# althonos/pyskani

Hardware: AMD Instinct MI355X
Metric: genome-pairs/sec (sketch+ANI) (higher is better)
Workload: dtype u64; 1 GPU; all-vs-all 10000 x 10000 synthetic ~5 Mb genomes on one GPU (100 families x 100; single-contig genomes, substitutions only), c=125 marker_c=1000 k=15; device-resident ASCII; hits=999867, genomes=10000, parallelism=references sharded over 1 GPU(s)

## Files before the change

include/pyskani_amd.h:

```cpp
#ifndef PYSKANI_AMD_H
#define PYSKANI_AMD_H
#include <stddef.h>
#include <stdint.h>
#ifdef __cplusplus
extern "C" {
#endif

typedef enum {
    PSK_OK = 0,
    PSK_EINVAL = 1,
    PSK_ENOMEM = 2,
    PSK_EHIP = 3,
    PSK_ENOMODEL = 4,
    PSK_EKEY = 5,
    PSK_ELIMIT = 6,
    PSK_ERCCL = 7
} psk_status;

typedef struct psk_ctx psk_ctx;
typedef struct psk_sketch psk_sketch;
typedef struct psk_db psk_db;
typedef struct psk_model psk_model;

typedef struct {
    int32_t c;
    int32_t marker_c;
    int32_t k;
} psk_params;

typedef struct {
    int32_t learned_ani;
    int32_t median;
    int32_t robust;
    int32_t faster_small;
    double cutoff;
    double min_aligned_frac;
    const psk_model* model;
} psk_query_opts;

typedef struct {
    float ani;
    float af_query;
    float af_ref;
    uint32_t ref_index;
    uint32_t n_chunks, n_intervals;
    uint64_t n_anchors, covered_query, covered_ref, sum_chain_anchors, sum_chunk_seeds;
    float ani_raw;
    float ani_std;
    uint32_t learned;
    uint32_t reserved;
} psk_hit;

typedef struct {
    float ani, af_query, af_ref;
    uint32_t ref_index;
    uint32_t query;
} psk_hit_min;

typedef struct { uint32_t kmer, pos, contig, canon; } psk_seed;

const char* psk_last_error(void);
const char* psk_version(void);
#define PSK_ABI_VERSION 7
int psk_abi_version(void);
void psk_free(void* p);

psk_status psk_ctx_create(int device, psk_ctx** out);
void psk_ctx_destroy(psk_ctx* ctx);
psk_status psk_ctx_synchronize(psk_ctx* ctx);
psk_status psk_ctx_set_timing(psk_ctx* ctx, int on);
psk_status psk_ctx_clock_probe(psk_ctx* ctx, double* mhz, double* ms);
psk_status psk_ctx_timing(psk_ctx* ctx, const char* kernel, double* total_ms, uint64_t* launches);
psk_status psk_ctx_work(psk_ctx* ctx, uint64_t* pairs, uint64_t* items, uint64_t* anchors, int reset);
psk_status psk_ctx_join_work(psk_ctx* ctx, uint64_t* lookups, uint64_t* visited, uint64_t* candidates, uint64_t* rows, int reset);
psk_status psk_ctx_small_query_stats(psk_ctx* ctx, uint64_t* taken, uint64_t* rerun, uint64_t* general);
psk_status psk_ctx_rerun_stats(psk_ctx* ctx, uint64_t* cap, uint64_t* wide, uint64_t* onepass, uint64_t* refit, int reset);
psk_status psk_ctx_tier_stats(psk_ctx* ctx, uint64_t* out, int n, int reset);
void psk_pack2bit_host(const uint8_t* src, uint64_t n, uint32_t* dst, int mode);
psk_status psk_device_alloc(psk_ctx* ctx, size_t bytes, void** dptr);
psk_status psk_device_free(psk_ctx* ctx, void* dptr);
psk_status psk_memcpy_h2d(psk_ctx* ctx, void* dst, const void* src, size_t bytes);

psk_status psk_sketch_host(psk_ctx* ctx, const psk_params* p, const uint8_t* const* contigs,
                           const uint64_t* lens, uint32_t n_contigs, int want_seeds,
                           psk_sketch** out);

psk_status psk_sketch_many_host(psk_ctx* ctx, const psk_params* p, const uint8_t* const* contigs, const uint64_t* lens,
                                const uint32_t* genome_first_contig, uint32_t n_genomes, int want_seeds,
                                psk_sketch** out);

psk_status psk_sketch_batch_device(psk_ctx* ctx, const psk_params* p, const uint8_t* d_bases,
                                   const uint64_t* contig_off, const uint64_t* contig_len,
                                   const uint32_t* genome_first_contig, uint32_t n_genomes,
                                   int want_seeds, psk_sketch** out);

void psk_sketch_free(psk_sketch* s);
void psk_sketch_free_many(psk_sketch* const* sketches, uint32_t n);
psk_status psk_sketch_info(const psk_sketch* s, psk_params* p, uint64_t* n_seeds,
                           uint64_t* n_markers, uint64_t* total_len, uint32_t* n_contigs);
psk_status psk_sketch_export(const psk_sketch* s, psk_seed* seeds, uint64_t* markers);

psk_status psk_sketch_contig_lens(const psk_sketch* s, uint32_t* lens);
psk_status psk_sketch_import(psk_ctx* ctx, const psk_params* p, const uint32_t* contig_lens, uint32_t n_contigs,
                             const psk_seed* seeds, uint64_t n_seeds, const uint64_t* markers, uint64_t n_markers,
                             int has_seeds, psk_sketch** out);

#define PSK_FEATURE_UNKNOWN (-3.402823466e+38F)
typedef struct {
    int32_t feature;
    float threshold;
    int32_t left, right;
    float value;
    int32_t missing;
    int32_t is_leaf;
    int32_t reserved;
} psk_tree_node;
typedef enum {
    PSK_F_ANI100 = 0,
    PSK_F_STD100 = 1,
    PSK_F_Q90_QUERY = 2, PSK_F_Q50_QUERY = 3, PSK_F_Q10_QUERY = 4,
    PSK_F_Q90_REF = 5, PSK_F_Q50_REF = 6, PSK_F_Q10_REF = 7,
    PSK_F_AVG_CHAIN_LEN = 8,
    PSK_F_AF_QUERY = 9, PSK_F_AF_REF = 10, PSK_F_N_CHUNKS = 11,
    PSK_F_TOTAL_LEN_QUERY = 12, PSK_F_TOTAL_LEN_REF = 13, PSK_F_N_CONTIGS_QUERY = 14, PSK_F_N_CONTIGS_REF = 15,
    PSK_F_COUNT = 16
} psk_feature;
psk_status psk_model_create(psk_ctx* ctx, const psk_tree_node* nodes, uint64_t n_nodes, const uint32_t* tree_first_node,
                            uint32_t n_trees, float bias, float shrinkage, const int32_t* features, uint32_t n_features,
                            psk_model** out);
psk_status psk_model_load_json(psk_ctx* ctx, const char* json, size_t len, psk_model** out);
psk_status psk_model_load_file(psk_ctx* ctx, const char* path, psk_model** out);
void psk_model_free(psk_model* m);
psk_status psk_model_info(const psk_model* m, uint32_t* n_trees, uint64_t* n_nodes, uint32_t* n_features);
psk_status psk_model_predict(const psk_model* m, const float* rows, uint32_t n_rows, float* out);

psk_status psk_sketch_pack_size(const psk_sketch* s, uint64_t* bytes);
psk_status psk_sketch_pack(const psk_sketch* s, void* d_dst, uint64_t capacity);
psk_status psk_sketch_unpack(psk_ctx* ctx, const void* d_src, uint64_t capacity, const uint64_t* offsets, uint32_t n, psk_sketch** out);
psk_status psk_sketch_pack_many(const psk_sketch* const* sketches, uint32_t n, void* d_dst, const uint64_t* offsets, uint64_t capacity);

typedef struct psk_comm psk_comm;
#define PSK_COMM_ID_BYTES 128
psk_status psk_comm_unique_id(void* id);
psk_status psk_comm_create(psk_ctx* ctx, int rank, int world, const void* id, psk_comm** out);
void psk_comm_destroy(psk_comm* comm);
psk_status psk_comm_info(const psk_comm* comm, int* rank, int* world, uint64_t* bytes_sent, uint64_t* collectives);
psk_status psk_gather_hits(psk_comm* comm, const psk_hit* local, uint64_t n_local, psk_hit** all, uint64_t* n_all, uint64_t* counts);
psk_status psk_gather_hits_min(psk_comm* comm, const psk_hit_min* local, uint64_t n_local, psk_hit_min** all, uint64_t* n_all, uint64_t* counts);
psk_status psk_gather_sketches(psk_comm* comm, const psk_sketch* const* mine, uint32_t n, psk_sketch*** all, uint32_t* counts);

psk_status psk_db_create(psk_ctx* ctx, const psk_params* p, psk_db** out);
void psk_db_destroy(psk_db* db);
psk_status psk_db_add(psk_db* db, const char* name, psk_sketch* s);
psk_status psk_db_add_batch(psk_db* db, const char* const* names, psk_sketch* const* sketches, uint32_t n);
uint32_t psk_db_size(const psk_db* db);
const char* psk_db_name(const psk_db* db, uint32_t index);
const psk_sketch* psk_db_sketch(const psk_db* db, uint32_t index);

psk_status psk_db_locality(psk_db* db, uint32_t* slot_of, uint32_t* n_groups, uint32_t* is_identity);

psk_status psk_screen(psk_db* db, const psk_sketch* query, double screen_val, int rescue_small,
                      uint8_t* pass, uint32_t* shared);

psk_status psk_chain(psk_ctx* ctx, const psk_sketch* const* refs, uint32_t n_refs,
                     const psk_sketch* query, const psk_query_opts* o, psk_hit* out);

psk_status psk_query(psk_db* db, const psk_sketch* query, const psk_query_opts* o,
                     psk_hit** hits, uint64_t* n_hits);

psk_status psk_query_host(psk_db* db, const uint8_t* const* contigs, const uint64_t* lens, uint32_t n_contigs, int seed,
                          const psk_query_opts* o, psk_hit** hits, uint64_t* n_hits);

psk_status psk_query_many(psk_db* db, const psk_sketch* const* queries, uint32_t n_queries,
                          const psk_query_opts* o, psk_hit** hits, uint64_t* offsets);
psk_status psk_query_many_min(psk_db* db, const psk_sketch* const* queries, uint32_t n_queries,
                              const psk_query_opts* opts, psk_hit_min** hits, uint64_t* offsets);

psk_status psk_query_many_tri(psk_db* db, const psk_sketch* const* queries, uint32_t n_queries, const int64_t* query_key, uint64_t ref_base,
                              const psk_query_opts* opts, psk_hit** hits, uint64_t* offsets);
psk_status psk_query_many_tri_min(psk_db* db, const psk_sketch* const* queries, uint32_t n_queries, const int64_t* query_key, uint64_t ref_base,
                                  const psk_query_opts* opts, psk_hit_min** hits, uint64_t* offsets);

typedef struct {
    double  min_ani;
    double  min_af;
    int32_t af_rule;
    int32_t linkage;
} psk_cluster_opts;
psk_status psk_cluster_records(psk_ctx* ctx, const psk_hit_min* recs, uint64_t n_recs, uint32_t n_genomes,
                               const uint64_t* priority , const psk_cluster_opts* opts,
                               uint32_t* rep_of, float* rep_ani , uint32_t* n_reps );
psk_status psk_ctx_cluster_stats(psk_ctx* ctx, uint64_t* edges, uint64_t* rounds, uint64_t* hook_passes);

#ifdef __cplusplus
}
#endif
#endif
```

pyskani_amd/_capi.py:

```python
import ctypes as C
import os

_HERE = os.path.dirname(os.path.abspath(__file__))
LIB_PATH = os.environ.get("PSK_LIB_PATH") or os.path.join(_HERE, "libpyskani_amd.so")

PSK_OK, PSK_EINVAL, PSK_ENOMEM, PSK_EHIP, PSK_ENOMODEL, PSK_EKEY, PSK_ELIMIT, PSK_ERCCL = range(8)
COMM_ID_BYTES = 128
ABI_VERSION = 7


class Params(C.Structure):
    _fields_ = [("c", C.c_int32), ("marker_c", C.c_int32), ("k", C.c_int32)]


class QueryOpts(C.Structure):
    _fields_ = [("learned_ani", C.c_int32), ("median", C.c_int32), ("robust", C.c_int32),
                ("faster_small", C.c_int32), ("cutoff", C.c_double), ("min_aligned_frac", C.c_double),
                ("model", C.c_void_p)]


class Hit(C.Structure):
    _fields_ = [("ani", C.c_float), ("af_query", C.c_float), ("af_ref", C.c_float),
                ("ref_index", C.c_uint32), ("n_chunks", C.c_uint32), ("n_intervals", C.c_uint32),
                ("n_anchors", C.c_uint64), ("covered_query", C.c_uint64), ("covered_ref", C.c_uint64),
                ("sum_chain_anchors", C.c_uint64), ("sum_chunk_seeds", C.c_uint64),
                ("ani_raw", C.c_float), ("ani_std", C.c_float), ("learned", C.c_uint32), ("reserved", C.c_uint32)]


class HitMin(C.Structure):
    _fields_ = [("ani", C.c_float), ("af_query", C.c_float), ("af_ref", C.c_float), ("ref_index", C.c_uint32), ("query", C.c_uint32)]


class ClusterOpts(C.Structure):
    _fields_ = [("min_ani", C.c_double), ("min_af", C.c_double), ("af_rule", C.c_int32), ("linkage", C.c_int32)]


class TreeNode(C.Structure):
    _fields_ = [("feature", C.c_int32), ("threshold", C.c_float), ("left", C.c_int32), ("right", C.c_int32),
                ("value", C.c_float), ("missing", C.c_int32), ("is_leaf", C.c_int32), ("reserved", C.c_int32)]


FEATURE_NAMES = ["ani100", "std100", "q90_query", "q50_query", "q10_query", "q90_ref", "q50_ref", "q10_ref", "avg_chain_len",
                 "af_query", "af_ref", "n_chunks", "total_len_query", "total_len_ref", "n_contigs_query", "n_contigs_ref"]
DEFAULT_FEATURES = FEATURE_NAMES[:9]


class Seed(C.Structure):
    _fields_ = [("kmer", C.c_uint32), ("pos", C.c_uint32), ("contig", C.c_uint32), ("canon", C.c_uint32)]


SYMBOLS = [
    "psk_last_error", "psk_version", "psk_abi_version", "psk_free", "psk_ctx_create", "psk_ctx_destroy",
    "psk_ctx_synchronize", "psk_pack2bit_host", "psk_ctx_small_query_stats", "psk_ctx_rerun_stats", "psk_ctx_tier_stats", "psk_ctx_set_timing", "psk_ctx_timing", "psk_db_add_batch", "psk_device_alloc", "psk_device_free", "psk_memcpy_h2d",
    "psk_sketch_host", "psk_sketch_many_host", "psk_sketch_batch_device", "psk_sketch_free", "psk_sketch_free_many", "psk_sketch_info",
    "psk_sketch_export", "psk_sketch_contig_lens", "psk_sketch_import", "psk_db_create", "psk_db_destroy", "psk_db_add", "psk_db_size",
    "psk_db_name", "psk_db_sketch", "psk_db_locality", "psk_screen", "psk_chain", "psk_query", "psk_query_host", "psk_query_many", "psk_query_many_min", "psk_query_many_tri", "psk_query_many_tri_min", "psk_cluster_records", "psk_ctx_cluster_stats", "psk_gather_hits_min",
    "psk_sketch_pack_size", "psk_sketch_pack", "psk_sketch_unpack", "psk_sketch_pack_many", "psk_ctx_clock_probe", "psk_ctx_work", "psk_ctx_join_work",
    "psk_comm_unique_id", "psk_comm_create", "psk_comm_destroy", "psk_comm_info", "psk_gather_hits", "psk_gather_sketches",
    "psk_model_create", "psk_model_load_json", "psk_model_load_file", "psk_model_free", "psk_model_info", "psk_model_predict",
]

_lib = None


def load():
    global _lib
    if _lib is not None:
        return _lib
    if not os.path.exists(LIB_PATH):
        raise ImportError(
            f"{LIB_PATH} not found: build it with `python -c 'import __graft_entry__ as g; g.build()'` "
            "or `make -C pyskani_amd/csrc`. pyskani_amd has no CPU fallback.")
    lib = C.CDLL(LIB_PATH)
    vp, u32, u64 = C.c_void_p, C.c_uint32, C.c_uint64
    lib.psk_abi_version.restype = C.c_int
    if lib.psk_abi_version() != ABI_VERSION:
        raise ImportError(f"{LIB_PATH} speaks C-ABI revision {lib.psk_abi_version()}, this binding {ABI_VERSION}: rebuild with `make -C pyskani_amd/csrc`")
    lib.psk_last_error.restype = C.c_char_p
    lib.psk_version.restype = C.c_char_p
    lib.psk_free.argtypes = [vp]
    lib.psk_ctx_create.argtypes = [C.c_int, C.POINTER(vp)]
    lib.psk_ctx_destroy.argtypes = [vp]
    lib.psk_ctx_destroy.restype = None
    lib.psk_ctx_synchronize.argtypes = [vp]
    lib.psk_ctx_small_query_stats.argtypes = [vp, C.POINTER(u64), C.POINTER(u64), C.POINTER(u64)]
    lib.psk_ctx_rerun_stats.argtypes = [vp, C.POINTER(u64), C.POINTER(u64), C.POINTER(u64), C.POINTER(u64), C.c_int]
    if hasattr(lib, "psk_ctx_tier_stats"):
        lib.psk_ctx_tier_stats.argtypes = [vp, C.POINTER(u64), C.c_int, C.c_int]
    lib.psk_pack2bit_host.argtypes = [vp, u64, vp, C.c_int]
    lib.psk_pack2bit_host.restype = None
    lib.psk_ctx_set_timing.argtypes = [vp, C.c_int]
    lib.psk_ctx_timing.argtypes = [vp, C.c_char_p, C.POINTER(C.c_double), C.POINTER(u64)]
    lib.psk_db_add_batch.argtypes = [vp, C.POINTER(C.c_char_p), C.POINTER(vp), u32]
    lib.psk_device_alloc.argtypes = [vp, C.c_size_t, C.POINTER(vp)]
    lib.psk_device_free.argtypes = [vp, vp]
    lib.psk_memcpy_h2d.argtypes = [vp, vp, vp, C.c_size_t]
    lib.psk_sketch_host.argtypes = [vp, C.POINTER(Params), C.POINTER(C.c_char_p), C.POINTER(u64), u32, C.c_int, C.POINTER(vp)]
    lib.psk_sketch_many_host.argtypes = [vp, C.POINTER(Params), C.POINTER(C.c_char_p), C.POINTER(u64), C.POINTER(u32), u32, C.c_int, C.POINTER(vp)]
    lib.psk_sketch_batch_device.argtypes = [vp, C.POINTER(Params), vp, C.POINTER(u64), C.POINTER(u64), C.POINTER(u32), u32, C.c_int, C.POINTER(vp)]
    lib.psk_sketch_free.argtypes = [vp]
    lib.psk_sketch_free.restype = None
    lib.psk_sketch_free_many.argtypes = [C.POINTER(vp), u32]
    lib.psk_sketch_free_many.restype = None
    lib.psk_sketch_info.argtypes = [vp, C.POINTER(Params), C.POINTER(u64), C.POINTER(u64), C.POINTER(u64), C.POINTER(u32)]
    lib.psk_sketch_export.argtypes = [vp, vp, vp]
    lib.psk_sketch_contig_lens.argtypes = [vp, vp]
    lib.psk_sketch_import.argtypes = [vp, C.POINTER(Params), vp, u32, vp, u64, vp, u64, C.c_int, C.POINTER(vp)]
    lib.psk_db_create.argtypes = [vp, C.POINTER(Params), C.POINTER(vp)]
    lib.psk_db_destroy.argtypes = [vp]
    lib.psk_db_destroy.restype = None
    lib.psk_db_add.argtypes = [vp, C.c_char_p, vp]
    lib.psk_db_size.argtypes = [vp]
    lib.psk_db_size.restype = u32
    lib.psk_db_name.argtypes = [vp, u32]
    lib.psk_db_name.restype = C.c_char_p
    lib.psk_db_sketch.argtypes = [vp, u32]
    lib.psk_db_sketch.restype = vp
    lib.psk_screen.argtypes = [vp, vp, C.c_double, C.c_int, vp, vp]
    lib.psk_db_locality.argtypes = [vp, C.POINTER(C.c_uint32), C.POINTER(C.c_uint32), C.POINTER(C.c_uint32)]
    lib.psk_chain.argtypes = [vp, C.POINTER(vp), u32, vp, C.POINTER(QueryOpts), C.POINTER(Hit)]
    lib.psk_query.argtypes = [vp, vp, C.POINTER(QueryOpts), C.POINTER(C.POINTER(Hit)), C.POINTER(u64)]
    lib.psk_query_host.argtypes = [vp, C.POINTER(C.c_char_p), C.POINTER(u64), u32, C.c_int, C.POINTER(QueryOpts), C.POINTER(C.POINTER(Hit)), C.POINTER(u64)]
    lib.psk_query_many.argtypes = [vp, C.POINTER(vp), u32, C.POINTER(QueryOpts), C.POINTER(C.POINTER(Hit)), C.POINTER(u64)]
    lib.psk_query_many_min.argtypes = [vp, C.POINTER(vp), u32, C.POINTER(QueryOpts), C.POINTER(C.POINTER(HitMin)), C.POINTER(u64)]
    lib.psk_query_many_tri.argtypes = [vp, C.POINTER(vp), u32, C.POINTER(C.c_int64), u64, C.POINTER(QueryOpts), C.POINTER(C.POINTER(Hit)), C.POINTER(u64)]
    lib.psk_query_many_tri_min.argtypes = [vp, C.POINTER(vp), u32, C.POINTER(C.c_int64), u64, C.POINTER(QueryOpts), C.POINTER(C.POINTER(HitMin)), C.POINTER(u64)]
    lib.psk_cluster_records.argtypes = [vp, vp, u64, u32, vp, C.POINTER(ClusterOpts), vp, vp, C.POINTER(u32)]
    lib.psk_ctx_cluster_stats.argtypes = [vp, C.POINTER(u64), C.POINTER(u64), C.POINTER(u64)]
    lib.psk_gather_hits_min.argtypes = [vp, vp, u64, C.POINTER(C.POINTER(HitMin)), C.POINTER(u64), C.POINTER(u64)]
    lib.psk_sketch_pack_size.argtypes = [vp, C.POINTER(u64)]
    lib.psk_sketch_pack.argtypes = [vp, vp, u64]
    lib.psk_sketch_unpack.argtypes = [vp, vp, u64, C.POINTER(u64), u32, C.POINTER(vp)]
    lib.psk_sketch_pack_many.argtypes = [C.POINTER(vp), u32, vp, C.POINTER(u64), u64]
    lib.psk_ctx_clock_probe.argtypes = [vp, C.POINTER(C.c_double), C.POINTER(C.c_double)]
    lib.psk_ctx_work.argtypes = [vp, C.POINTER(u64), C.POINTER(u64), C.POINTER(u64), C.c_int]
    lib.psk_ctx_join_work.argtypes = [vp, C.POINTER(u64), C.POINTER(u64), C.POINTER(u64), C.POINTER(u64), C.c_int]
    lib.psk_comm_unique_id.argtypes = [vp]
    lib.psk_comm_create.argtypes = [vp, C.c_int, C.c_int, vp, C.POINTER(vp)]
    lib.psk_comm_destroy.argtypes = [vp]
    lib.psk_comm_destroy.restype = None
    lib.psk_comm_info.argtypes = [vp, C.POINTER(C.c_int), C.POINTER(C.c_int), C.POINTER(u64), C.POINTER(u64)]
    lib.psk_gather_hits.argtypes = [vp, vp, u64, C.POINTER(C.POINTER(Hit)), C.POINTER(u64), C.POINTER(u64)]
    lib.psk_gather_sketches.argtypes = [vp, C.POINTER(vp), u32, C.POINTER(C.POINTER(vp)), C.POINTER(u32)]
    lib.psk_model_create.argtypes = [vp, C.POINTER(TreeNode), u64, C.POINTER(u32), u32, C.c_float, C.c_float, C.POINTER(C.c_int32), u32, C.POINTER(vp)]
    lib.psk_model_load_json.argtypes = [vp, C.c_char_p, C.c_size_t, C.POINTER(vp)]
    lib.psk_model_load_file.argtypes = [vp, C.c_char_p, C.POINTER(vp)]
    lib.psk_model_free.argtypes = [vp]
    lib.psk_model_free.restype = None
    lib.psk_model_info.argtypes = [vp, C.POINTER(u32), C.POINTER(u64), C.POINTER(u32)]
    lib.psk_model_predict.argtypes = [vp, vp, u32, vp]
    _lib = lib
    return lib


_EXC = {PSK_EINVAL: ValueError, PSK_ENOMEM: MemoryError, PSK_EHIP: RuntimeError,
        PSK_ENOMODEL: RuntimeError, PSK_EKEY: KeyError, PSK_ELIMIT: OverflowError, PSK_ERCCL: RuntimeError}


def check(status):
    if status != PSK_OK:
        msg = load().psk_last_error().decode("utf-8", "replace")
        raise _EXC.get(status, RuntimeError)(msg)


def hit_records(hits_p, lo, hi, dtype):
    import numpy as np
    n = max(0, hi - lo)
    out = np.empty(n, dtype)
    if n:
        C.memmove(out.ctypes.data, C.cast(hits_p, C.c_void_p).value + lo * dtype.itemsize, n * dtype.itemsize)
    return out
```

pyskani_amd/csrc/capi.hip:

```cpp
#include "common.h"
#include <cstdarg>
#include <algorithm>

static thread_local char g_err[512] = "";

void psk_set_error(const char* fmt, ...) {
    va_list ap;
    va_start(ap, fmt);
    vsnprintf(g_err, sizeof g_err, fmt, ap);
    va_end(ap);
}

#include <sys/mman.h>
#include <unordered_map>
namespace {
struct HitBlocks {
    std::mutex mu;
    std::unordered_map<void*, size_t> live;
    void* kept = nullptr; size_t kept_bytes = 0;
    const bool keep = !env_val("PSK_HIT_CACHE").off();
};
HitBlocks& hit_blocks() { static HitBlocks* hb = new HitBlocks(); return *hb; }
}
void* hit_block_alloc(size_t bytes) {
// ... 296 lines not shown
void psk_sketch_free_many(psk_sketch* const* sketches, uint32_t n) { if (sketches) for (uint32_t i = 0; i < n; i++) delete sketches[i]; }

psk_status psk_sketch_info(const psk_sketch* s, psk_params* p, uint64_t* n_seeds, uint64_t* n_markers, uint64_t* total_len, uint32_t* n_contigs) {
    if (!s) { psk_set_error("NULL sketch"); return PSK_EINVAL; }
    if (p) *p = s->params;
    if (n_seeds) *n_seeds = s->n_seeds;
    if (n_markers) *n_markers = s->n_markers;
    if (total_len) *total_len = s->total_len;
    if (n_contigs) *n_contigs = (uint32_t)s->contig_len.size();
    return PSK_OK;
}

psk_status psk_sketch_export(const psk_sketch* s, psk_seed* seeds, uint64_t* markers) {
    if (!s) { psk_set_error("NULL sketch"); return PSK_EINVAL; }
    PSK_LANE(lg, s->ctx);
    Lane* ctx = lg.lane;
    if (seeds && s->n_seeds) {
        size_t n = s->n_seeds;
        std::vector<uint32_t> kmer(n), pos(n), meta(n);
        PSK_HIP(hipMemcpyAsync(kmer.data(), s->store->seed_kmer + s->seed_off, 4 * n, hipMemcpyDeviceToHost, ctx->stream));
        PSK_HIP(hipMemcpyAsync(pos.data(), s->store->seed_pos + s->seed_off, 4 * n, hipMemcpyDeviceToHost, ctx->stream));
        PSK_HIP(hipMemcpyAsync(meta.data(), s->store->seed_meta + s->seed_off, 4 * n, hipMemcpyDeviceToHost, ctx->stream));
        PSK_HIP(hipStreamSynchronize(ctx->stream));
        for (size_t i = 0; i < n; i++) { seeds[i].kmer = kmer[i]; seeds[i].pos = pos[i]; seeds[i].contig = meta[i] >> 1; seeds[i].canon = meta[i] & 1; }
    }
    if (markers && s->n_markers) {
        PSK_HIP(hipMemcpyAsync(markers, s->store->markers + s->marker_off, 8 * (size_t)s->n_markers, hipMemcpyDeviceToHost, ctx->stream));
        PSK_HIP(hipStreamSynchronize(ctx->stream));
    }
    return PSK_OK;
}

psk_status psk_sketch_contig_lens(const psk_sketch* s, uint32_t* lens) {
    if (!s || (!lens && !s->contig_len.empty())) { psk_set_error("contig_lens: NULL argument"); return PSK_EINVAL; }
    for (size_t i = 0; i < s->contig_len.size(); i++) lens[i] = s->contig_len[i];
    return PSK_OK;
}

psk_status psk_sketch_import(psk_ctx* ctx, const psk_params* p, const uint32_t* contig_lens, uint32_t n_contigs,
                             const psk_seed* seeds, uint64_t n_seeds, const uint64_t* markers, uint64_t n_markers,
                             int has_seeds, psk_sketch** out) {
    if (!ctx || !p || !out || (n_contigs && !contig_lens) || (n_seeds && !seeds) || (n_markers && !markers)) { psk_set_error("sketch_import: NULL argument"); return PSK_EINVAL; }
    if (p->k < 1 || p->k > 16 || p->c < 1 || p->marker_c < 1) { psk_set_error("invalid sketch parameters"); return PSK_EINVAL; }
    if (n_seeds >= 0x7FFFFFF0ull || n_markers >= 0x7FFFFFF0ull) { psk_set_error("sketch too large to import"); return PSK_ELIMIT; }
    *out = nullptr;
    PSK_LANE(lg, ctx);
    Lane* lane = lg.lane;
    std::unique_ptr<psk_sketch> s(new psk_sketch());
    s->ctx = ctx; s->params = *p; s->has_seeds = has_seeds != 0;
    s->contig_len.assign(contig_lens, contig_lens + n_contigs);
    for (uint32_t i = 0; i < n_contigs; i++) s->total_len += contig_lens[i];
    s->contig_seed_start.assign(n_contigs + 1, 0);
    const size_t ns = (size_t)n_seeds;
    std::vector<uint32_t> kmer(ns), pos(ns), meta(ns), cstart(n_contigs + 1, 0);
    std::vector<uint64_t> pm(ns);
    for (size_t i = 0; i < ns; i++) {
        const psk_seed& sd = seeds[i];
        if (sd.contig >= n_contigs || sd.pos >= contig_lens[sd.contig] || sd.canon > 1 ||
            (i && (sd.contig < seeds[i - 1].contig || (sd.contig == seeds[i - 1].contig && sd.pos <= seeds[i - 1].pos)))) {
            psk_set_error("sketch_import: seed %zu is out of range or out of (contig,pos) order", i);
            return PSK_EINVAL;
        }
        kmer[i] = sd.kmer; pos[i] = sd.pos; meta[i] = (sd.contig << 1) | sd.canon; pm[i] = ((uint64_t)sd.pos << 32) | meta[i];
        cstart[sd.contig + 1]++;
    }
    for (uint32_t c = 0; c < n_contigs; c++) cstart[c + 1] += cstart[c];
    s->contig_seed_start = cstart;
    for (uint64_t i = 1; i < n_markers; i++) if (markers[i] <= markers[i - 1]) { psk_set_error("sketch_import: markers must be sorted and distinct"); return PSK_EINVAL; }
    auto store = std::make_shared<SketchStore>();
    store->ctx = ctx;
    auto al = [](size_t x) { return (x + 255) & ~(size_t)255; };
    size_t b_kmer = 0, b_pos = al(b_kmer + 4 * ns), b_meta = al(b_pos + 4 * ns), b_pm = al(b_meta + 4 * ns), b_cs = al(b_pm + 8 * ns), b_end = al(b_cs + 4 * (size_t)(n_contigs + 1));
    PSK_TRY(ctx->pool_alloc(b_end, &store->base, &store->bytes));
    char* sb = (char*)store->base;
    store->seed_kmer = (uint32_t*)(sb + b_kmer); store->seed_pos = (uint32_t*)(sb + b_pos); store->seed_meta = (uint32_t*)(sb + b_meta);
    store->seed_pm = (uint64_t*)(sb + b_pm); store->contig_seed_start = (uint32_t*)(sb + b_cs);
    PSK_TRY(ctx->pool_alloc(8 * ((size_t)n_markers + 1), &store->mbase, &store->mbytes));
    store->markers = (uint64_t*)store->mbase;
    hipStream_t st = lane->stream;
    if (ns) {
        PSK_HIP(hipMemcpyAsync(store->seed_kmer, kmer.data(), 4 * ns, hipMemcpyHostToDevice, st));
        PSK_HIP(hipMemcpyAsync(store->seed_pos, pos.data(), 4 * ns, hipMemcpyHostToDevice, st));
        PSK_HIP(hipMemcpyAsync(store->seed_meta, meta.data(), 4 * ns, hipMemcpyHostToDevice, st));
        PSK_HIP(hipMemcpyAsync(store->seed_pm, pm.data(), 8 * ns, hipMemcpyHostToDevice, st));
    }
    PSK_HIP(hipMemcpyAsync(store->contig_seed_start, cstart.data(), 4 * (size_t)(n_contigs + 1), hipMemcpyHostToDevice, st));
    if (n_markers) PSK_HIP(hipMemcpyAsync(store->markers, markers, 8 * (size_t)n_markers, hipMemcpyHostToDevice, st));
    PSK_HIP(hipStreamSynchronize(st));
    s->store = store;
    s->seed_off = 0; s->n_seeds = n_seeds; s->marker_off = 0; s->n_markers = n_markers; s->contig_off = 0;
    *out = s.release();
    return PSK_OK;
}

psk_status psk_db_create(psk_ctx* ctx, const psk_params* p, psk_db** out) {
    if (!ctx || !p || !out) { psk_set_error("db_create: NULL argument"); return PSK_EINVAL; }
    if (p->k < 1 || p->k > 16 || p->c < 1 || p->marker_c < 1) { psk_set_error("invalid sketch parameters (c=%d marker_c=%d k=%d)", p->c, p->marker_c, p->k); return PSK_EINVAL; }
    psk_db* db = new psk_db();
    db->ctx = ctx; db->params = *p;
    *out = db;
    return PSK_OK;
}

void psk_db_destroy(psk_db* db) {
    if (!db) return;
    (void)hipSetDevice(db->ctx->device);
    for (psk_sketch* s : db->refs) delete s;
    db->d_marker_ptr.release(); db->d_marker_n.release();
    db->inv_key.release(); db->inv_ref.release(); db->inv_tmp.release(); db->inv_bucket.release();
    db->d_refdesc.release(); db->d_canon.release(); db->d_refdesc_slot.release(); db->d_ref_of.release(); db->d_slot_of.release();
    db->gsi_key.release(); db->gsi_val.release(); db->gsi_bucket.release();
    db->bsi_key.release(); db->bsi_val.release(); db->bsi_bucket.release(); db->bsi_base.release();
    delete db;
}

psk_status psk_db_add(psk_db* db, const char* name, psk_sketch* s) {
    if (!db || !name || !s) { delete s; psk_set_error("db_add: NULL argument"); return PSK_EINVAL; }
    if (s->ctx != db->ctx) { delete s; psk_set_error("db_add: sketch belongs to another context"); return PSK_EINVAL; }
    std::unique_lock<std::shared_mutex> lk(db->rw);
    db->refs.push_back(s);
    db->names.emplace_back(name);
    db->note_added((uint32_t)db->refs.size() - 1);
    db->stale();
    return PSK_OK;
}

psk_status psk_db_add_batch(psk_db* db, const char* const* names, psk_sketch* const* sketches, uint32_t n) {
    if (!db || (n && (!names || !sketches))) { psk_set_error("db_add_batch: NULL argument"); return PSK_EINVAL; }
    std::unique_lock<std::shared_mutex> lk(db->rw);
    for (uint32_t i = 0; i < n; i++)
        if (!sketches[i] || !names[i] || sketches[i]->ctx != db->ctx) { psk_set_error("db_add_batch: bad entry %u", i); return PSK_EINVAL; }
    for (uint32_t i = 0; i < n; i++) {
        db->refs.push_back(sketches[i]);
        db->names.emplace_back(names[i]);
        db->note_added((uint32_t)db->refs.size() - 1);
    }
    db->stale();
    return PSK_OK;
}

uint32_t psk_db_size(const psk_db* db) { if (!db) return 0; std::shared_lock<std::shared_mutex> lk(db->rw); return (uint32_t)db->refs.size(); }
const char* psk_db_name(const psk_db* db, uint32_t i) { if (!db) return nullptr; std::shared_lock<std::shared_mutex> lk(db->rw); return i < db->names.size() ? db->names[i].c_str() : nullptr; }
const psk_sketch* psk_db_sketch(const psk_db* db, uint32_t i) { if (!db) return nullptr; std::shared_lock<std::shared_mutex> lk(db->rw); return i < db->refs.size() ? db->refs[i] : nullptr; }

psk_status psk_db_locality(psk_db* db, uint32_t* slot_of, uint32_t* n_groups, uint32_t* is_identity) {
    if (!db) { psk_set_error("db_locality: NULL database"); return PSK_EINVAL; }
    PSK_LANE(lg, db->ctx);
    std::unique_lock<std::shared_mutex> lk(db->rw);
    PSK_TRY(ensure_locality(lg.lane, db, n_groups != nullptr));
    const uint32_t n = (uint32_t)db->refs.size();
    if (slot_of) for (uint32_t r = 0; r < n; r++) slot_of[r] = db->loc_identity ? r : db->slot_of[r];
    if (n_groups) *n_groups = db->loc_groups;
    if (is_identity) *is_identity = db->loc_identity ? 1u : 0u;
    return PSK_OK;
}

psk_status psk_screen(psk_db* db, const psk_sketch* q, double screen_val, int rescue_small, uint8_t* pass, uint32_t* shared) {
    if (!db || !q || !pass) { psk_set_error("screen: NULL argument"); return PSK_EINVAL; }
    PSK_LANE(lg, db->ctx);
    return screen_impl(lg.lane, db, q, screen_val, rescue_small, pass, shared);
}

psk_status psk_chain(psk_ctx* ctx, const psk_sketch* const* refs, uint32_t n_refs, const psk_sketch* q, const psk_query_opts* o, psk_hit* out) {
    if (!ctx) { psk_set_error("NULL ctx"); return PSK_EINVAL; }
    PSK_LANE(lg, ctx);
    return chain_impl(lg.lane, refs, n_refs, q, o, out);
}

static psk_status hits_out(HitList& all, psk_hit** hits) {
    if (!all.p) { all.p = (psk_hit*)malloc(sizeof(psk_hit)); if (!all.p) { psk_set_error("out of host memory"); return PSK_ENOMEM; } }
    *hits = all.release();
    return PSK_OK;
}

psk_status psk_query(psk_db* db, const psk_sketch* q, const psk_query_opts* o, psk_hit** hits, uint64_t* n_hits) {
    if (!db || !q || !o || !hits || !n_hits) { psk_set_error("query: NULL argument"); return PSK_EINVAL; }
    *hits = nullptr; *n_hits = 0;
    PSK_LANE(lg, db->ctx);
    HitList all;
    uint64_t offs[2];
    PSK_TRY(query_many_impl(lg.lane, db, &q, 1, o, all, offs));
    const uint64_t nh = all.n;
    PSK_TRY(hits_out(all, hits));
    *n_hits = nh;
    return PSK_OK;
}

psk_status psk_query_host(psk_db* db, const uint8_t* const* contigs, const uint64_t* lens, uint32_t n_contigs, int want_seeds,
                          const psk_query_opts* o, psk_hit** hits, uint64_t* n_hits) {
    if (!db || !o || !hits || !n_hits || (n_contigs && (!contigs || !lens))) { psk_set_error("query_host: NULL argument"); return PSK_EINVAL; }
    *hits = nullptr; *n_hits = 0;
    HitList all;
    if (want_seeds) {
        PSK_LANE(lg, db->ctx);
        bool done = false;
        PSK_TRY(query_host_small(lg.lane, db, contigs, lens, n_contigs, o, all, &done));
        if (!done) db->ctx->sq_general++;
        if (done) {
            const uint64_t nh = all.n;
            PSK_TRY(hits_out(all, hits));
            *n_hits = nh;
            return PSK_OK;
        }
        all.n = 0;
    }
    psk_sketch* q = nullptr;
    PSK_TRY(psk_sketch_host(db->ctx, &db->params, contigs, lens, n_contigs, want_seeds, &q));
    const psk_status rc = psk_query(db, q, o, hits, n_hits);
    delete q;
    return rc;
}

psk_status psk_query_many(psk_db* db, const psk_sketch* const* queries, uint32_t n_queries, const psk_query_opts* o,
                          psk_hit** hits, uint64_t* offsets) {
    if (!db || (!queries && n_queries) || !o || !hits || !offsets) { psk_set_error("query_many: NULL argument"); return PSK_EINVAL; }
    *hits = nullptr;
    offsets[0] = 0;
    PSK_LANE(lg, db->ctx);
    HitList all;
    PSK_TRY(query_many_impl(lg.lane, db, queries, n_queries, o, all, offsets));
    return hits_out(all, hits);
}

psk_status psk_query_many_min(psk_db* db, const psk_sketch* const* queries, uint32_t n_queries, const psk_query_opts* o,
                              psk_hit_min** hits, uint64_t* offsets) {
    if (!db || (!queries && n_queries) || !o || !hits || !offsets) { psk_set_error("query_many_min: NULL argument"); return PSK_EINVAL; }
    *hits = nullptr;
    offsets[0] = 0;
    PSK_LANE(lg, db->ctx);
    HitListMin all;
    PSK_TRY(query_many_min_impl(lg.lane, db, queries, n_queries, o, all, offsets));
    if (!all.p) { all.p = (psk_hit_min*)malloc(sizeof(psk_hit_min)); if (!all.p) { psk_set_error("out of host memory"); return PSK_ENOMEM; } }
    *hits = all.release();
    return PSK_OK;
}

static psk_status tri_args(const psk_db* db, const void* queries, uint32_t n_queries, const int64_t* query_key, uint64_t ref_base, const void* o, const void* hits, const void* offsets, const char* who) {
    if (!db || (!queries && n_queries) || !o || !hits || !offsets) { psk_set_error("%s: NULL argument", who); return PSK_EINVAL; }
    if (!query_key && n_queries) { psk_set_error("%s: NULL query_key", who); return PSK_EINVAL; }
    if (ref_base > (1ull << 63) || ref_base + psk_db_size(db) > (1ull << 63)) { psk_set_error("%s: ref_base %llu + the database's size exceeds 2^63 (keys are signed 64-bit)", who, (unsigned long long)ref_base); return PSK_ELIMIT; }
    return PSK_OK;
}

psk_status psk_query_many_tri(psk_db* db, const psk_sketch* const* queries, uint32_t n_queries, const int64_t* query_key, uint64_t ref_base,
                              const psk_query_opts* o, psk_hit** hits, uint64_t* offsets) {
    PSK_TRY(tri_args(db, queries, n_queries, query_key, ref_base, o, hits, offsets, "query_many_tri"));
    *hits = nullptr;
    offsets[0] = 0;
    PSK_LANE(lg, db->ctx);
    HitList all;
    PSK_TRY(query_many_impl(lg.lane, db, queries, n_queries, o, all, offsets, n_queries ? query_key : nullptr, ref_base));
    return hits_out(all, hits);
}

psk_status psk_query_many_tri_min(psk_db* db, const psk_sketch* const* queries, uint32_t n_queries, const int64_t* query_key, uint64_t ref_base,
                                  const psk_query_opts* o, psk_hit_min** hits, uint64_t* offsets) {
    PSK_TRY(tri_args(db, queries, n_queries, query_key, ref_base, o, hits, offsets, "query_many_tri_min"));
    *hits = nullptr;
    offsets[0] = 0;
    PSK_LANE(lg, db->ctx);
    HitListMin all;
    PSK_TRY(query_many_min_impl(lg.lane, db, queries, n_queries, o, all, offsets, n_queries ? query_key : nullptr, ref_base));
    if (!all.p) { all.p = (psk_hit_min*)malloc(sizeof(psk_hit_min)); if (!all.p) { psk_set_error("out of host memory"); return PSK_ENOMEM; } }
    *hits = all.release();
    return PSK_OK;
}

}


#include <condition_variable>
#include <functional>
#include <thread>
#include <atomic>
#include <map>
namespace {
struct ParallelFor {
    std::vector<std::thread> th; std::mutex mu; std::condition_variable cv, cv_done;
    std::function<void(int)> fn; int n = 0, next = 0, active = 0; uint64_t gen = 0; bool stop = false;
    explicit ParallelFor(int workers) {
        for (int i = 0; i < workers; i++) th.emplace_back([this] {
            uint64_t seen = 0;
            for (;;) {
                std::unique_lock<std::mutex> lk(mu);
                cv.wait(lk, [&] { return stop || (gen != seen && next < n); });
                if (stop) return;
                seen = gen;
                while (next < n) { int i = next++; active++; lk.unlock(); fn(i); lk.lock(); active--; }
                if (active == 0) cv_done.notify_all();
            }
        });
    }
    void run(int count, std::function<void(int)> f) {
        std::unique_lock<std::mutex> lk(mu);
        fn = std::move(f); n = count; next = 0; gen++;
        cv.notify_all();
        while (next < n) { int i = next++; active++; lk.unlock(); fn(i); lk.lock(); active--; }
        cv_done.wait(lk, [&] { return active == 0 && next >= n; });
    }
    ~ParallelFor() { { std::lock_guard<std::mutex> lk(mu); stop = true; } cv.notify_all(); for (auto& t : th) t.join(); }
};
constexpr size_t INGEST_SLOT = 32u << 20;
constexpr int INGEST_SLOTS = 4;
struct IngestRes {
    hipStream_t copy = nullptr;
    void* pinned[INGEST_SLOTS] = {nullptr}; hipEvent_t slot_free[INGEST_SLOTS] = {nullptr};
// ... 175 lines not shown
```

pyskani_amd/csrc/chain.hip:

```cpp
#include "chain_stages.h"
#include "query_parts.h"
#include <hipcub/hipcub.hpp>
#include <cmath>
#include <algorithm>
#include <unordered_map>


SketchDesc make_desc(const psk_sketch* s, bool unindexed_ok) {
    SketchDesc d{};
    const bool ix = s->idx != nullptr;
    d.key = ix ? s->idx->km32 + s->idx_off : nullptr; d.pms = ix ? s->idx->pms + s->idx_off : nullptr;
    d.perm = ix ? s->idx->perm + s->idx_off : nullptr; d.bucket = ix ? s->idx->bucket + s->idx_boff : nullptr;
    d.bshift = ix ? s->idx_bshift : 0; d.n = (ix || (unindexed_ok && s->store)) ? (uint32_t)s->n_seeds : 0;
    d.pos = s->store ? s->store->seed_pos + s->seed_off : nullptr; d.meta = s->store ? s->store->seed_meta + s->seed_off : nullptr;
    d.kmer = s->store ? s->store->seed_kmer + s->seed_off : nullptr;
    d.seed_pos_base = s->store ? s->store->seed_pos : nullptr;
    d.contig_start = s->store ? s->store->contig_seed_start + s->contig_off : nullptr;
    d.total_len = s->total_len; d.n_contigs = (uint32_t)s->contig_len.size();
    uint64_t rows = 0;
    if (d.n) for (uint32_t len : s->contig_len) rows += (uint64_t)len / (FRAGMENT_LENGTH + 1) + 1;
    d.rows = (uint32_t)std::min<uint64_t>(rows, 0xFFFFFFFFu);
    s->len_quantiles(d.lenq);
    d.tab = (ix && s->ptab) ? (const ProbeLine*)s->ptab->base + s->ptab_off : nullptr; d.tab_lines = (ix && s->ptab) ? s->ptab_lines : 0;
    return d;
// ... 24 lines not shown
    const uint8_t* __restrict__ row = pass + (size_t)B.q * n_refs;
    const int lane = threadIdx.x & 63, wave = threadIdx.x >> 6;
    uint32_t running = 0;
    for (uint32_t base = 0; base < n_refs && running < B.rank_hi; base += 256) {
        const uint32_t r = base + threadIdx.x;
        const bool f = r < n_refs && row[r];
        const unsigned long long bal = __ballot(f);
        if (lane == 0) s_w[wave] = (uint32_t)__popcll(bal);
        __syncthreads();
        uint32_t before = 0;
        for (int w = 0; w < wave; w++) before += s_w[w];
        const uint32_t tot = s_w[0] + s_w[1] + s_w[2] + s_w[3];
        const uint32_t rank = running + before + (uint32_t)__popcll(bal & ((1ull << lane) - 1));
        if (f && rank >= B.rank_lo && rank < B.rank_hi) {
            const uint32_t j = rank - B.rank_lo, slot = B.pair_off + j;
            pairs[slot] = combine_desc(Q, rd[r]);
            sbase[slot] = B.item_off + j * Q.n; cbase[slot] = B.row_off + j * Q.rows;
            pair_qr[slot] = make_uint2(B.q, r);
        }
        running += tot;
        __syncthreads();
    }
    if (blockIdx.x == gridDim.x - 1 && threadIdx.x == 0) { sbase[n_pairs] = n_items; cbase[n_pairs] = n_rows; }
}

__global__ __launch_bounds__(256) void pass_canon_kernel(uint8_t* __restrict__ pass, uint32_t n_refs, const uint32_t* __restrict__ canon) {
    uint8_t* row = pass + (size_t)blockIdx.x * n_refs;
    for (uint32_t r = threadIdx.x; r < n_refs; r += blockDim.x) if (row[r] && canon[r] != r) { row[canon[r]] = 1; row[r] = 0; }
}
__global__ __launch_bounds__(256) void pass_triangle_kernel(uint8_t* __restrict__ pass, uint32_t n_refs, const long long* __restrict__ key, unsigned long long ref_base) {
    const long long k = key[blockIdx.x];
    if (k < 0 || (unsigned long long)k < ref_base) return;
    const unsigned long long d = (unsigned long long)k - ref_base;
    const uint32_t len = d >= n_refs ? n_refs : (uint32_t)d + 1u;
    uint8_t* row = pass + (size_t)blockIdx.x * n_refs;
    const uint32_t to16 = (16u - (uint32_t)((uintptr_t)row & 15u)) & 15u, head = to16 < len ? to16 : len;
    const uint32_t n16 = (len - head) >> 4, tail = head + (n16 << 4);
    if (threadIdx.x < head) row[threadIdx.x] = 0;
    uint4* mid = (uint4*)(row + head);
    for (uint32_t i = threadIdx.x; i < n16; i += blockDim.x) mid[i] = make_uint4(0, 0, 0, 0);
    if (threadIdx.x < len - tail) row[tail + threadIdx.x] = 0;
}
static_assert((1 << BSI_BLOG) == 256, "pass_count_kernel: one sweep of its 256 threads = one block of references");
__global__ __launch_bounds__(256) void pass_count_kernel(const uint8_t* __restrict__ pass, uint32_t n_refs, uint32_t* __restrict__ row_count, uint8_t* __restrict__ col_flag, uint32_t* __restrict__ row_blocks) {
    __shared__ uint32_t s_c[4], s_any;
    const uint8_t* row = pass + (size_t)blockIdx.x * n_refs;
    uint32_t c = 0, blocks = 0;
    if (threadIdx.x == 0) s_any = 0;
    __syncthreads();
    for (uint32_t r0 = 0; r0 < n_refs; r0 += 256) {
        const uint32_t r = r0 + threadIdx.x;
        const bool f = r < n_refs && row[r];
        if (f) { c++; col_flag[r] = 1; s_any = 1; }
        __syncthreads();
        blocks += s_any;
        __syncthreads();
        if (threadIdx.x == 0) s_any = 0;
        __syncthreads();
    }
#pragma unroll
    for (int o = 32; o > 0; o >>= 1) c += __shfl_xor(c, o);
    if ((threadIdx.x & 63) == 0) s_c[threadIdx.x >> 6] = c;
    __syncthreads();
    if (threadIdx.x == 0) { row_count[blockIdx.x] = s_c[0] + s_c[1] + s_c[2] + s_c[3]; row_blocks[blockIdx.x] = blocks; }
}

__global__ __launch_bounds__(256) void gsi_room_kernel(const uint32_t* __restrict__ sbase, uint32_t n_pairs, uint32_t* __restrict__ pstart) {
    const uint32_t p = blockIdx.x * blockDim.x + threadIdx.x;
    if (p <= n_pairs) { const uint32_t a = sbase[p]; pstart[p] = a + (a >> 3) + 8u * p; }
}
__global__ void gsi_total_kernel(const unsigned long long* __restrict__ poff, uint32_t n_pairs, unsigned long long* __restrict__ total64) { *total64 = poff[n_pairs]; }

struct HitPasses { __host__ __device__ bool operator()(const psk_hit& h) const { return h.ani > 0.1f; } };

__global__ __launch_bounds__(256) void work_rows_kernel(const ChunkOut* __restrict__ cout, const uint32_t* __restrict__ n_chunks, const uint32_t* __restrict__ cbase,
                                                        const uint32_t* __restrict__ row_pair, uint32_t n_rows, unsigned long long* __restrict__ out) {
    __shared__ unsigned long long s_c[4], s_l[4];
    unsigned long long c = 0, live = 0;
    for (uint32_t r = blockIdx.x * blockDim.x + threadIdx.x; r < n_rows; r += gridDim.x * blockDim.x) {
        const uint32_t p = row_pair[r];
        if (r - cbase[p] < n_chunks[p]) { c += cout[r].n_cand; live++; }
    }
#pragma unroll
    for (int o = 32; o > 0; o >>= 1) { c += __shfl_xor(c, o); live += __shfl_xor(live, o); }
    if ((threadIdx.x & 63) == 0) { s_c[threadIdx.x >> 6] = c; s_l[threadIdx.x >> 6] = live; }
    __syncthreads();
    if (threadIdx.x == 0) {
        c = s_c[0] + s_c[1] + s_c[2] + s_c[3]; live = s_l[0] + s_l[1] + s_l[2] + s_l[3];
        if (live) { atomicAdd(&out[0], c); atomicAdd(&out[1], live); }
    }
}

psk_status chain_layout(Lane* ctx, size_t n_pairs, size_t n_items, size_t n_rows, size_t n_bq, ChainBufs* L) {
    const size_t gi = (n_items + 255) / 256, gi_sum = std::max(gi, (n_pairs + 3) / 4);
    size_t o_pairs = 0, o_sbase = al256(o_pairs + sizeof(PairDesc) * n_pairs), o_cbase = al256(o_sbase + 4 * (n_pairs + 1)),
           o_pstart = al256(o_cbase + 4 * (n_pairs + 1)), o_lb = al256(o_pstart + 4 * (n_pairs + 1)),
           o_aoff = al256(o_lb + 8 * (n_items + 1)), o_nch = al256(o_aoff + 4 * (n_items + 1)),
           o_chunks = al256(o_nch + 4 * n_pairs), o_rq0 = al256(o_chunks + sizeof(uint2) * n_rows), o_cout = al256(o_rq0 + sizeof(uint2) * n_rows),
           o_misc = al256(o_cout + sizeof(ChunkOut) * n_rows), o_hits = o_misc + 256, o_sel = al256(o_hits + sizeof(psk_hit) * n_pairs),
           o_ovf = al256(o_sel + sizeof(psk_hit) * n_pairs), o_bsum = al256(o_ovf + 4 * n_rows),
           o_qr = al256(o_bsum + 8 * (gi_sum + 1)), o_bq = al256(o_qr + 8 * n_pairs), o_bp = al256(o_bq + sizeof(BatchQ) * (n_bq + 1)),
           o_rp = al256(o_bp + 4 * (gi + 1)), o_live = al256(o_rp + 4 * (n_rows + 1)), o_big = al256(o_live + 4 * (n_pairs + 1)),
           o_huge = al256(o_big + 4 * (n_pairs + 1)), o_end = o_huge + 4 * (n_pairs + 1);
    PSK_TRY(ctx->q_b.reserve(o_end));
    char* B = (char*)ctx->q_b.p;
    L->pairs = (PairDesc*)(B + o_pairs); L->sbase = (uint32_t*)(B + o_sbase); L->cbase = (uint32_t*)(B + o_cbase); L->pstart = (uint32_t*)(B + o_pstart);
    L->lbcnt = (uint2*)(B + o_lb); L->aoff = (uint32_t*)(B + o_aoff); L->nch = (uint32_t*)(B + o_nch); L->chunks = (uint2*)(B + o_chunks); L->row_q0 = (uint2*)(B + o_rq0);
    L->cout = (ChunkOut*)(B + o_cout); L->hits = (psk_hit*)(B + o_hits); L->hits_sel = (psk_hit*)(B + o_sel); L->misc = (uint32_t*)(B + o_misc);
    L->ovf = (uint32_t*)(B + o_ovf); L->bsum = (unsigned long long*)(B + o_bsum); L->pair_qr = (uint2*)(B + o_qr); L->bq = (BatchQ*)(B + o_bq);
    L->blk_pair = (uint32_t*)(B + o_bp); L->row_pair = (uint32_t*)(B + o_rp); L->live = (uint32_t*)(B + o_live); L->big_list = (uint32_t*)(B + o_big); L->huge_list = (uint32_t*)(B + o_huge);
    L->gi = (uint32_t)gi; L->gi_sum = (uint32_t)gi_sum;
    L->total = (unsigned long long*)(L->misc + 16);
    return PSK_OK;
}

psk_status chain_run(Lane* ctx, const ChainBufs& L, uint32_t n_pairs, size_t n_items, size_t n_rows, const psk_params& prm,
                     const psk_query_opts* o, const SketchDesc* d_qd, const SketchDesc* d_rd, uint64_t cap, bool wide, const Switches& sw, bool probe_ok) {
    hipStream_t st = ctx->stream;
    const int force_serial = sw.chain_serial.get() != nullptr;
    const uint32_t gi = L.gi;
    hipLaunchKernelGGL(pair_table_kernel, dim3((uint32_t)(((size_t)gi + n_rows + 255) / 256)), dim3(256), 0, st, L.sbase, L.cbase, n_pairs, gi, (uint32_t)n_items, (uint32_t)n_rows, L.blk_pair, L.row_pair,
                       L.misc, L.lbcnt + n_items);
    ctx->t_begin(K_ANCHOR);
    if (wide) hipLaunchKernelGGL(anchor_count_kernel, dim3(gi), dim3(256), 0, st, L.pairs, L.sbase, n_pairs, (uint32_t)n_items, L.lbcnt, L.bsum, L.blk_pair);
    const uint32_t gi4 = (gi + JT - 1) / JT;
    uint32_t n_sum = gi;
    const int jp_force = sw.join_pairs.force();
    const bool gsi_join = !wide && (L.g_key || L.b_key) && L.d_pass && L.n_bq;
    const bool join_pairs = !wide && (gsi_join || (jp_force >= 0 ? jp_force == 1 : (n_pairs >= 16384 && n_items / n_pairs < 2048)));
    const bool gsl = gsi_join && L.gsi_slice;
    const bool gsi_one = gsi_join && !gsl && L.gsi_onepass && cap >= n_items + n_items / 8 + 8 * ((size_t)n_pairs + 1);
    bool probe_local = false;
    GsiJoinArgs GA{};
    GslArgs GL{};
    const uint32_t gsi_nw = (L.g_key && !L.gsi_slice) ? std::max(4u, (L.n_refs + 63u) / 64u) : 4u;
    const size_t gsi_lds_row = 8 * (size_t)gsi_nw + 4 * (size_t)((gsi_nw + 1u) & ~1u), gsi_lds_count = gsi_lds_row + 4 * (size_t)L.p_cap, gsi_lds_emit = gsi_lds_row + 4 * (size_t)L.p_cap * 9;
    if (gsi_join) {
        GA.bq = L.bq; GA.pass = L.d_pass; GA.n_refs = L.n_refs; GA.qd = d_qd; GA.g_key = L.g_key; GA.g_val = L.g_val; GA.g_bucket = L.g_bucket; GA.g_shift = L.g_shift;
        GA.b_key = L.b_key; GA.b_val = L.b_val; GA.b_bucket = L.b_bucket; GA.b_shift = L.b_shift; GA.b_nb1 = L.b_nb1; GA.b_blocks = L.b_blocks; GA.b_max = L.b_max;
        GA.pair_cnt = L.big_list; GA.pstart = L.pstart; GA.cap = (uint32_t)cap; GA.err = L.misc; GA.p_cap = L.p_cap; GA.nw_lds = gsi_nw;
        const uint32_t t_blocks = gsl ? L.g_blocks : L.b_blocks;
        const unsigned long long* t_base = gsl ? L.g_base : L.b_base;
        const uint32_t bcap = std::max(1u, std::min<uint32_t>(t_blocks, std::min<uint32_t>(GSI_PMAX, std::max(1u, L.p_cap))));
        uint32_t* d_btab = nullptr; uint32_t* d_bcnt = nullptr;
        if (t_blocks) {
            const size_t o_bc = al256(4 * (size_t)L.n_bq * bcap * GSL_BT_WORDS);
            PSK_TRY(ctx->q_k.reserve(o_bc + 4 * (size_t)L.n_bq + 256));
            d_btab = (uint32_t*)ctx->q_k.p; d_bcnt = (uint32_t*)((char*)ctx->q_k.p + o_bc);
            PSK_TRY(gsl_blocks_launch(L.bq, L.n_bq, L.d_pass, L.n_refs, t_blocks, t_base, d_btab, d_bcnt, bcap, st));
        }
        GA.blk_tab = d_btab; GA.blk_cnt = d_bcnt; GA.blk_cap = bcap;
        if (gsl) {
            GL.bq = L.bq; GL.n_entries = L.n_bq; GL.tab = L.gsl_tab; GL.n_tab = L.gsl_n_tab; GL.ebase = L.gsl_ebase; GL.pass = L.d_pass; GL.n_refs = L.n_refs; GL.qd = d_qd;
            GL.g_key = L.g_key; GL.g_val = L.g_val; GL.g_bucket = L.g_bucket; GL.g_shift = L.g_shift; GL.g_nb1 = L.g_nb1; GL.g_blocks = L.g_blocks; GL.g_base = L.g_base; GL.blk_tab = d_btab; GL.blk_cnt = d_bcnt; GL.blk_cap = bcap; GL.cnt = L.gsl_cnt; GL.rec = L.gsl_rec; GL.bm = L.gsl_bm; GL.un = L.gsl_un; GL.n_slices = L.gsl_n_slices;
            GL.pair_cnt = L.big_list; GL.pstart = L.pstart; GL.cap = (uint32_t)cap; GL.err = L.misc; GL.p_cap = L.p_cap; GL.chunks = L.chunks; GL.n_chunks = L.nch; GL.row_q0 = L.row_q0;
            PSK_HIP(hipMemsetAsync(L.big_list, 0, 4 * ((size_t)n_pairs + 1), st));
            PSK_TRY(gsl_count_launch(GL, st));
        }
        else if (!gsi_one) hipLaunchKernelGGL(gsi_join_kernel<false>, dim3(L.n_bq), dim3(64), gsi_lds_count, st, GA);
        probe_local = true;
    }
    else if (join_pairs) {
        size_t ts = 0;
        uint32_t* keys_in = L.big_list;
        uint32_t* vals_in = L.live;
        uint32_t* keys_out = (uint32_t*)L.hits_sel;
        uint32_t* order = keys_out + n_pairs;
        hipLaunchKernelGGL(pair_ref_keys_kernel, dim3((n_pairs + 255) / 256), dim3(256), 0, st, L.pair_qr, n_pairs, keys_in, vals_in);
        PSK_HIP(hipcub::DeviceRadixSort::SortPairs(nullptr, ts, keys_in, keys_out, vals_in, order, (int)n_pairs, 0, 32, st));
        PSK_TRY(ctx->q_g.reserve(ts + 256));
        PSK_HIP(hipcub::DeviceRadixSort::SortPairs(ctx->q_g.p, ts, keys_in, keys_out, vals_in, order, (int)n_pairs, 0, 32, st));
        const uint32_t nb = (n_pairs + 3) / 4;
        probe_local = probe_ok;
        if (probe_ok) hipLaunchKernelGGL(anchor_join_probe_kernel, dim3(nb), dim3(256), 0, st, L.pairs, L.sbase, order, n_pairs, L.lbcnt, L.bsum, L.misc + 5, L.aoff, L.big_list);
        else hipLaunchKernelGGL(anchor_join_pairs_kernel, dim3(nb), dim3(256), 0, st, L.pairs, L.sbase, order, n_pairs, L.lbcnt, L.bsum, L.misc + 5);
        n_sum = nb;
    }
    const int ep_force = sw.emit_pairs.force();
    const bool emit_pairs = !wide && !join_pairs && n_items >= 2 * ((size_t)n_pairs + 1) &&
                            (ep_force >= 0 ? ep_force == 1 : (n_pairs >= 1024 && n_items / n_pairs >= 1024 && n_items / n_pairs <= (1u << 17)));
    uint32_t* pair_cnt = L.live;
    if (emit_pairs) PSK_HIP(hipMemsetAsync(pair_cnt, 0, 4 * ((size_t)n_pairs + 1), st));
    const int xg_env = (int)sw.xcd_group.num(-1);
    const uint32_t xcd_group = xg_env >= 0 ? (uint32_t)xg_env : (n_pairs >= 64 ? (uint32_t)std::min<size_t>(4096, std::max<size_t>(1, 4 * (n_items / n_pairs) / (JT * 256))) : 0u);
    if (!wide && !join_pairs) { hipLaunchKernelGGL(anchor_join4_kernel, dim3(gi4), dim3(256), 0, st, L.pairs, L.sbase, n_pairs, (uint32_t)n_items, gi, L.lbcnt, L.bsum, L.misc + 5, L.blk_pair, emit_pairs ? pair_cnt : (uint32_t*)nullptr, xcd_group); n_sum = gi4; }
    ctx->t_end();
    size_t tmp = 0, tmp2 = 0;
    hipcub::TransformInputIterator<uint32_t, CountOf, const uint2*> cnt_it(L.lbcnt, CountOf());
    hipcub::TransformInputIterator<uint32_t, PackedCount, const uint2*> pcnt_it(L.lbcnt, PackedCount());
    PSK_HIP(hipcub::DeviceScan::ExclusiveSum(nullptr, tmp, cnt_it, L.aoff, (int)(n_items + 1), st));
    PSK_HIP(hipcub::DeviceReduce::Sum(nullptr, tmp2, L.bsum, L.total, (int)L.gi_sum, st));
    size_t tmp3 = 0;
    PSK_HIP(hipcub::DeviceSelect::If(nullptr, tmp3, L.hits, L.hits_sel, L.misc + 12, (int)n_pairs, HitPasses(), st));
    PSK_TRY(ctx->q_c.reserve(std::max(tmp, std::max(tmp2, tmp3))));
    unsigned long long* poff = (unsigned long long*)L.aoff;
    hipcub::TransformInputIterator<unsigned long long, Widen, const uint32_t*> pc_it(pair_cnt, Widen());
    if (gsi_one) {
        hipLaunchKernelGGL(gsi_room_kernel, dim3((n_pairs + 1 + 255) / 256), dim3(256), 0, st, (const uint32_t*)L.sbase, n_pairs, L.pstart);
        PSK_HIP(hipMemsetAsync(L.total, 0, 8, st));
    }
    else if (emit_pairs) {
        size_t tmp4 = 0;
        PSK_HIP(hipcub::DeviceScan::ExclusiveSum(nullptr, tmp4, pc_it, poff, (int)(n_pairs + 1), st));
        PSK_TRY(ctx->q_c.reserve(std::max(tmp4, std::max(tmp, std::max(tmp2, tmp3)))));
        PSK_HIP(hipcub::DeviceScan::ExclusiveSum(ctx->q_c.p, tmp4, pc_it, poff, (int)(n_pairs + 1), st));
        hipLaunchKernelGGL(pair_start64_kernel, dim3((n_pairs + 1 + 255) / 256), dim3(256), 0, st, poff, n_pairs, L.pstart, (uint32_t)cap, (const uint32_t*)(L.misc + 5));
    }
    else if (probe_local) {
        hipcub::TransformInputIterator<unsigned long long, Widen, const uint32_t*> pl_it(L.big_list, Widen());
        size_t tmp5 = 0;
        PSK_HIP(hipcub::DeviceScan::ExclusiveSum(nullptr, tmp5, pl_it, (unsigned long long*)nullptr, (int)(n_pairs + 1), st));
        const size_t o_poff = al256(tmp5 + 256);
        PSK_TRY(ctx->q_g.reserve(o_poff + 8 * ((size_t)n_pairs + 2) + 256));
        unsigned long long* pl_off64 = (unsigned long long*)((char*)ctx->q_g.p + o_poff);
        PSK_HIP(hipMemsetAsync(L.big_list + n_pairs, 0, 4, st));
        PSK_HIP(hipcub::DeviceScan::ExclusiveSum(ctx->q_g.p, tmp5, pl_it, pl_off64, (int)(n_pairs + 1), st));
        hipLaunchKernelGGL(pair_start64_kernel, dim3((n_pairs + 1 + 255) / 256), dim3(256), 0, st, (const unsigned long long*)pl_off64, n_pairs, L.pstart, (uint32_t)cap, (const uint32_t*)(L.misc + 5));
        if (gsi_join) hipLaunchKernelGGL(gsi_total_kernel, dim3(1), dim3(1), 0, st, (const unsigned long long*)pl_off64, n_pairs, L.total);
    }
    else if (wide) PSK_HIP(hipcub::DeviceScan::ExclusiveSum(ctx->q_c.p, tmp, cnt_it, L.aoff, (int)(n_items + 1), st));
    else PSK_HIP(hipcub::DeviceScan::ExclusiveSum(ctx->q_c.p, tmp, pcnt_it, L.aoff, (int)(n_items + 1), st));
    const bool small_sum = !gsi_join && n_sum <= 16384;
    if (!small_sum && !gsi_join) PSK_HIP(hipcub::DeviceReduce::Sum(ctx->q_c.p, tmp2, L.bsum, L.total, (int)n_sum, st));
    if ((!emit_pairs && !probe_local) || small_sum)
        hipLaunchKernelGGL(pair_start_kernel, dim3((emit_pairs || probe_local) ? 1u : (n_pairs + 1 + 255) / 256), dim3(256), 0, st, (emit_pairs || probe_local) ? (const uint32_t*)nullptr : L.aoff, L.sbase, n_pairs, L.pstart, (uint32_t)cap,
                           L.bsum, small_sum ? n_sum : 0u, L.total, (const uint32_t*)(L.misc + 5));
    hipLaunchKernelGGL(pair_guard_kernel, dim3((n_pairs + 1 + 255) / 256), dim3(256), 0, st, (const uint32_t*)(L.misc + 5), (const unsigned long long*)L.total, (unsigned long long)cap, L.pstart, n_pairs);
    const size_t na = ((size_t)cap + 64 + 63) & ~(size_t)63;
    PSK_TRY(ctx->q_d.reserve(4 * na * CHAIN_ANCHOR_WORDS));
    PSK_TRY(ctx->q_e.reserve(na * (8 + 4 * 7 + 1) + 512 + 4 * 2 * BIG_GMAX * (BIG_GROUPS + 64) + 4 * BIG_GROUPS));
    uint32_t* D = (uint32_t*)ctx->q_d.p;
    uint32_t* E4 = (uint32_t*)ctx->q_e.p;
    uint4* anc = (uint4*)D;
    uint32_t* a_nxt = D + 4 * na;
    ChainArgs A{};
    A.anc = anc;
    A.row_q0 = gsl ? L.row_q0 : nullptr;
    A.sc_ptr = D + 5 * na;
    A.sc_f = (int32_t*)E4; A.sc_root = E4 + na; A.sc_depth = E4 + 2 * na; A.sc_best = E4 + 3 * na;
    uint32_t* CAND = D + 6 * na;
    A.c_score.p = (int32_t*)CAND; A.c_q0.p = CAND + 1; A.c_q1.p = CAND + 2; A.c_r0.p = CAND + 3; A.c_r1.p = CAND + 4; A.c_n.p = CAND + 5; A.c_rc.p = CAND + 6; A.c_state.p = CAND + 7;
    A.chunks = L.chunks; A.n_chunks = L.nch; A.cbase = L.cbase; A.n_pairs = n_pairs; A.n_rows = (uint32_t)n_rows;
    A.row_pair = L.row_pair;
    A.pairs = L.pairs;
    A.out = L.cout; A.two_c = 2u * (uint32_t)prm.c; A.force_serial = force_serial; A.stats = L.misc + 1;
    A.band = std::max(1, std::min(MAX_CHAIN_BAND, BP_CHAIN_BAND / (int)prm.c));
    A.cap = (uint32_t)cap;
    const bool use_hops = gsi_join ? false : sw.chunk_hops.get() ? !sw.chunk_hops.off() : ((n_pairs < 1024 && n_items / n_pairs > 4096) || n_items / n_pairs > (1u << 20));
    const bool emit_heads = emit_pairs && !use_hops && !sw.emit_heads.off();
    const int hi_force = sw.hops_items.force();
    const bool hops_items = use_hops && !gsl && !emit_pairs && !join_pairs && n_items <= 0x7FFFFFFFull && (hi_force >= 0 ? hi_force == 1 : n_items / n_pairs > (1u << 20));
    ctx->t_begin(K_ANCHOR_EMIT);
    if (hops_items) {
        const size_t o_scr = al256(4 * (size_t)n_pairs * HOP_SLICES + 256);
        PSK_TRY(ctx->q_g.reserve(o_scr + sizeof(uint2) * n_rows + 256));
        uint32_t* slice_cnt = (uint32_t*)ctx->q_g.p;
        uint2* scratch_rows = (uint2*)((char*)ctx->q_g.p + o_scr);
        hipStream_t sd = nullptr;
        PSK_TRY(ctx->side_lane(&sd));
        PSK_HIP(hipEventRecord(ctx->side_fork, st));
        PSK_HIP(hipStreamWaitEvent(sd, ctx->side_fork, 0));
        hipLaunchKernelGGL(chunk_hops_items_kernel, dim3(n_pairs, HOP_SLICES), dim3(64), 0, sd, L.pstart, (const uint32_t*)L.aoff, L.pairs, L.sbase, L.cbase, n_pairs, slice_cnt, scratch_rows, L.misc);
        hipLaunchKernelGGL(chunk_hops_sliced_kernel, dim3(n_pairs, HOP_SLICES), dim3(64), 0, sd, L.pstart, a_nxt, anc, L.pairs, L.cbase, n_pairs, slice_cnt, 1, scratch_rows, L.chunks, L.nch, L.misc);
        PSK_HIP(hipEventRecord(ctx->side_join, sd));
    }
    if (gsl) { GL.anc = (uint2*)anc; PSK_TRY(gsl_heads_launch(GL, st)); PSK_TRY(gsl_emit_launch(GL, st)); }
    else if (gsi_join) { GA.anc = anc; GA.chunks = L.chunks; GA.n_chunks = L.nch; GA.onepass = gsi_one ? 1 : 0; GA.total = L.total; if (gsi_one) GA.pair_cnt = L.aoff;
                    hipLaunchKernelGGL(gsi_join_kernel<true>, dim3(L.n_bq), dim3(64), gsi_lds_emit, st, GA); }
    else if (wide) hipLaunchKernelGGL(anchor_emit_kernel, dim3(gi), dim3(256), 0, st, L.pairs, L.sbase, n_pairs, (uint32_t)n_items, L.lbcnt, L.aoff, anc, (uint32_t)cap, L.misc, L.blk_pair);
    else if (emit_pairs) hipLaunchKernelGGL(anchor_emit_pairs_kernel, dim3(n_pairs), dim3(EP_T), 0, st, L.pairs, L.sbase, n_pairs, L.lbcnt, poff, anc, (uint32_t)cap, L.misc,
                                            L.cbase, emit_heads ? L.chunks : (uint2*)nullptr, L.nch);
    else {
        const int ex_force = sw.emit_expand.force();
        const bool expand = ex_force >= 0 ? ex_force == 1 : n_items / n_pairs > (1u << 20);
        if (expand) hipLaunchKernelGGL(anchor_emit_expand_kernel, dim3(gi), dim3(256), 0, st, L.pairs, L.sbase, n_pairs, (uint32_t)n_items, L.lbcnt, L.aoff, anc, (uint32_t)cap, L.misc, L.blk_pair);
        else hipLaunchKernelGGL(anchor_emit_packed4_kernel, dim3(gi4), dim3(256), 0, st, L.pairs, L.sbase, n_pairs, (uint32_t)n_items, gi, L.lbcnt, L.aoff, anc, (uint32_t)cap, L.misc, L.blk_pair,
                                probe_local ? (const uint32_t*)L.pstart : (const uint32_t*)nullptr);
    }
    if (hops_items) PSK_HIP(hipStreamWaitEvent(st, ctx->side_join, 0));
    else if (use_hops) {
        if (n_items / n_pairs > (1u << 20)) {
            uint32_t* coarse = E4;
            hipLaunchKernelGGL(anchor_next_kernel<1>, dim3((uint32_t)((cap / 64 + 1 + 255) / 256)), dim3(256), 0, st, anc, L.pstart, n_pairs, (const uint32_t*)nullptr, coarse);
            hipLaunchKernelGGL(anchor_next_kernel<2>, dim3((uint32_t)((cap + 255) / 256)), dim3(256), 0, st, anc, L.pstart, n_pairs, (const uint32_t*)coarse, a_nxt);
        } else
        hipLaunchKernelGGL(anchor_next_kernel<0>, dim3((uint32_t)((cap + 255) / 256)), dim3(256), 0, st, anc, L.pstart, n_pairs, (const uint32_t*)nullptr, a_nxt);
        if (n_items / n_pairs > (1u << 20)) {
            const size_t o_scr = al256(4 * (size_t)n_pairs * HOP_SLICES + 256);
            PSK_TRY(ctx->q_g.reserve(o_scr + sizeof(uint2) * n_rows + 256));
            uint32_t* slice_cnt = (uint32_t*)ctx->q_g.p;
            uint2* scratch_rows = (uint2*)((char*)ctx->q_g.p + o_scr);
            for (int pass = 0; pass < 2; pass++)
                hipLaunchKernelGGL(chunk_hops_sliced_kernel, dim3(n_pairs, HOP_SLICES), dim3(64), 0, st, L.pstart, a_nxt, anc, L.pairs, L.cbase, n_pairs, slice_cnt, pass, scratch_rows, L.chunks, L.nch, L.misc);
        } else
        hipLaunchKernelGGL(chunk_hops_kernel, dim3(n_pairs), dim3(64), 0, st, L.pstart, a_nxt, L.cbase, n_pairs, L.chunks, L.nch, L.misc);
    } else if (!emit_heads && !gsi_join)
        hipLaunchKernelGGL(chunk_heads_kernel, dim3(n_pairs), dim3(64), 0, st, L.pstart, anc, L.cbase, n_pairs, L.chunks, L.nch, L.misc);
    ctx->t_end();
    ctx->t_begin(K_CHAIN_CHUNK);
    auto order_rows = [&]() -> psk_status {
        if (n_rows < 4096) return PSK_OK;
        size_t ts = 0;
        PSK_HIP(hipcub::DeviceRadixSort::SortPairsDescending(nullptr, ts, (const uint32_t*)nullptr, (uint32_t*)nullptr, (const uint32_t*)nullptr, (uint32_t*)nullptr, (int)n_rows, 0, 8, st));
        const size_t ob = al256(4 * n_rows);
        PSK_TRY(ctx->q_g.reserve(4 * ob + ts + 256));
        uint32_t* k_in = (uint32_t*)ctx->q_g.p; uint32_t* v_in = (uint32_t*)((char*)ctx->q_g.p + ob); uint32_t* k_out = (uint32_t*)((char*)ctx->q_g.p + 2 * ob); uint32_t* v_out = (uint32_t*)((char*)ctx->q_g.p + 3 * ob);
        hipLaunchKernelGGL(row_len_kernel, dim3((uint32_t)((n_rows + 255) / 256)), dim3(256), 0, st, L.chunks, L.nch, L.cbase, L.row_pair, (uint32_t)n_rows, k_in, v_in);
// ... 278 lines not shown
```

pyskani_amd/csrc/common.h:

```cpp
#pragma once
#include <hip/hip_runtime.h>
#include <cstdint>
#include <cstdio>
#include <cstdlib>
#include <cstring>
#include <ctime>
#include <sys/mman.h>
#include <algorithm>
#include <atomic>
#include <memory>
#include <mutex>
#include <shared_mutex>
#include <condition_variable>
#include <deque>
#include <string>
#include <unordered_map>
#include <vector>
#include "../../include/pyskani_amd.h"

struct EnvVal {
    const char* text;
    bool off() const { return text && text[0] == '0'; }
    int force() const { return text ? text[0] == '1' : -1; }
    double num(double dflt) const { return text ? atof(text) : dflt; }
// ... 272 lines not shown
    void* base = nullptr;
    size_t bytes = 0;
    uint64_t* key = nullptr;
    uint32_t* perm = nullptr;
    uint64_t* pms = nullptr;
    uint32_t* km32 = nullptr;
    uint32_t* bucket = nullptr;
    hipStream_t built_on = nullptr; hipEvent_t ready = nullptr;
    ~IndexStore();
};

inline IndexStore::~IndexStore() {
    if (ready) { (void)hipEventSynchronize(ready); (void)hipEventDestroy(ready); }
    if (ctx) ctx->pool_release(base, bytes); else if (base) (void)hipFree(base);
}

constexpr uint32_t PROBE_SLOTS = 5;
constexpr uint32_t PROBE_EMPTY = 0xFFFFFFFFu;
struct ProbeLine { uint32_t k[PROBE_SLOTS]; uint32_t pad; uint2 v[PROBE_SLOTS]; };
static_assert(sizeof(ProbeLine) == 64, "one probe line = one 64-byte cache line");
struct ProbeStore {
    psk_ctx* ctx = nullptr;
    void* base = nullptr;
    size_t bytes = 0;
    ~ProbeStore() { if (ctx) ctx->pool_release(base, bytes); else if (base) (void)hipFree(base); }
};

struct SketchStore {
    psk_ctx* ctx = nullptr;
    void* base = nullptr;
    size_t bytes = 0, mbytes = 0;
    uint32_t* seed_kmer = nullptr;
    uint32_t* seed_pos = nullptr;
    uint32_t* seed_meta = nullptr;
    uint64_t* seed_pm = nullptr;
    uint64_t* markers = nullptr;
    uint32_t* contig_seed_start = nullptr;
    void* mbase = nullptr;
    ~SketchStore() {
        if (ctx) { ctx->pool_release(base, bytes); ctx->pool_release(mbase, mbytes); }
        else { if (base) (void)hipFree(base); if (mbase) (void)hipFree(mbase); }
    }
};

struct SketchDesc {
    const uint32_t* key; const uint64_t* pms; const uint32_t* perm; const uint32_t* bucket;
    const uint32_t* pos; const uint32_t* meta; const uint32_t* seed_pos_base; const uint32_t* contig_start;
    const uint32_t* kmer;
    uint64_t total_len;
    uint32_t n;
    uint32_t bshift, rows;
    uint32_t n_contigs;
    float lenq[3];
    uint32_t tab_lines;
    const ProbeLine* tab;
};

struct SmallVecU32 {
    uint32_t inl[4]; uint32_t* p = inl; uint32_t n = 0, cap = 4;
    SmallVecU32() = default;
    SmallVecU32(const SmallVecU32&) = delete; SmallVecU32& operator=(const SmallVecU32&) = delete;
    ~SmallVecU32() { if (p != inl) delete[] p; }
    void grow(size_t c) {
        if (c <= cap) return;
        const size_t nc = c > 2 * (size_t)cap ? c : 2 * (size_t)cap;
        uint32_t* q = new uint32_t[nc];
        memcpy(q, p, 4 * (size_t)n);
        if (p != inl) delete[] p;
        p = q; cap = (uint32_t)nc;
    }
    size_t size() const { return n; }
    bool empty() const { return n == 0; }
    uint32_t& operator[](size_t i) { return p[i]; }
    const uint32_t& operator[](size_t i) const { return p[i]; }
    const uint32_t* begin() const { return p; }
    const uint32_t* end() const { return p + n; }
    void push_back(uint32_t v) { grow((size_t)n + 1); p[n++] = v; }
    void resize(size_t c) { grow(c); for (size_t i = n; i < c; i++) p[i] = 0; n = (uint32_t)c; }
    void assign(size_t c, uint32_t v) { grow(c); for (size_t i = 0; i < c; i++) p[i] = v; n = (uint32_t)c; }
    template <class It> void assign(It a, It b) { const size_t c = (size_t)(b - a); grow(c); for (size_t i = 0; i < c; i++) p[i] = (uint32_t)a[i]; n = (uint32_t)c; }
    SmallVecU32& operator=(const std::vector<uint32_t>& v) { assign(v.begin(), v.end()); return *this; }
};

struct psk_sketch {
    psk_ctx* ctx = nullptr;
    psk_params params{};
    std::shared_ptr<SketchStore> store;
    uint64_t seed_off = 0, n_seeds = 0;
    uint64_t marker_off = 0, n_markers = 0;
    uint64_t contig_off = 0;
    SmallVecU32 contig_len;
    SmallVecU32 contig_seed_start;
    uint64_t total_len = 0;
    bool has_seeds = true;
    void len_quantiles(float out[3]) const {
        out[0] = out[1] = out[2] = 0.f;
        if (contig_len.empty()) return;
        if (contig_len.size() == 1) { out[0] = out[1] = out[2] = (float)contig_len[0]; return; }
        std::vector<uint32_t> v(contig_len.begin(), contig_len.end());
        std::sort(v.begin(), v.end());
        const size_t n = v.size();
        out[0] = (float)v[std::min(n - 1, n * 9 / 10)]; out[1] = (float)v[std::min(n - 1, n / 2)]; out[2] = (float)v[std::min(n - 1, n / 10)];
    }
    mutable uint64_t visit = 0;
    mutable std::shared_ptr<IndexStore> idx;
    mutable uint64_t idx_off = 0;
    mutable uint64_t idx_boff = 0;
    mutable uint32_t idx_bshift = 0;
    mutable std::shared_ptr<ProbeStore> ptab;
    mutable uint64_t ptab_off = 0;
    mutable uint32_t ptab_lines = 0;
};

struct psk_db {
    psk_ctx* ctx = nullptr;
    mutable std::shared_mutex rw;
    psk_params params{};
    std::vector<psk_sketch*> refs;
    std::deque<std::string> names;
    std::vector<uint32_t> name_slot;
    std::vector<uint32_t> canon;
    bool has_dups = false, canon_dirty = false;
    static uint32_t name_hash(const std::string& s) { uint32_t h = 2166136261u; for (unsigned char c : s) h = (h ^ c) * 16777619u; return h; }
    void note_added(uint32_t i) {
        canon_dirty = true;
        if (name_slot.size() < 2 * (size_t)(i + 1) + 2) {
            size_t cap = 64; while (cap < 4 * (size_t)(i + 1)) cap <<= 1;
            std::vector<uint32_t> grown(cap, 0);
            for (uint32_t v : name_slot) if (v) { size_t k = name_hash(names[v - 1]) & (cap - 1); while (grown[k]) k = (k + 1) & (cap - 1); grown[k] = v; }
            name_slot.swap(grown);
        }
        const size_t mask = name_slot.size() - 1;
        size_t k = name_hash(names[i]) & mask;
        while (name_slot[k] && names[name_slot[k] - 1] != names[i]) k = (k + 1) & mask;
        if (name_slot[k]) { has_dups = true; const uint32_t prev = name_slot[k] - 1; for (uint32_t j = 0; j < i; j++) if (canon[j] == prev) canon[j] = i; }
        name_slot[k] = i + 1;
        canon.push_back(i);
    }
    bool tables_dirty = true;
    PoolScratch d_marker_ptr, d_marker_n;
    bool inv_dirty = true;
    PoolScratch inv_key, inv_ref, inv_tmp, inv_bucket;
    uint64_t inv_n = 0; int inv_bits = 0;
    bool desc_dirty = true;
    uint64_t desc_indexed = 0; uint32_t desc_n = 0;
    PoolScratch d_refdesc, d_canon;
    std::vector<SketchDesc> h_refdesc, h_refdesc_slot;
    int gsi_state = 0;
    PoolScratch gsi_key, gsi_val, gsi_bucket;
    uint64_t gsi_n = 0; int gsi_shift = 0;
    int bsi_state = 0;
    PoolScratch bsi_key, bsi_val, bsi_bucket, bsi_base;
    uint64_t bsi_n = 0; int bsi_shift = 0; uint32_t bsi_nb1 = 0, bsi_blocks = 0;
    std::atomic<int> small_state{0};
    int loc_state = 0;
    bool loc_identity = true, loc_groups_known = false;
    uint32_t loc_groups = 0;
    std::vector<uint32_t> ref_of, slot_of;
    PoolScratch d_ref_of, d_slot_of, d_refdesc_slot;
    void stale() {
        tables_dirty = true; inv_dirty = true; desc_dirty = true; small_state = 0; gsi_key.release(); gsi_val.release(); gsi_bucket.release(); gsi_state = 0;
        bsi_key.release(); bsi_val.release(); bsi_bucket.release(); bsi_base.release(); bsi_state = 0;
        loc_state = 0;
    }
};

psk_status ensure_locality(Lane* ctx, psk_db* db, bool want_groups = false);

struct ModelNode { int32_t feature; float threshold; int32_t left, right; float value; int32_t missing, is_leaf, menu; };
struct ModelDev { const ModelNode* nodes; const uint32_t* first; uint32_t n_trees; uint32_t n_features; float bias, shrinkage; };
struct psk_model {
    psk_ctx* ctx = nullptr;
    void* base = nullptr;
    ModelDev dev{};
    uint64_t n_nodes = 0;
    std::vector<int32_t> features;
    ~psk_model() { if (base) (void)hipFree(base); }
};
void learned_apply_launch(const psk_model* m, psk_hit* d_hits, const uint2* pair_qr, const SketchDesc* qd, const SketchDesc* rd,
                          uint32_t n_pairs, hipStream_t st);

struct ContigDesc {
    uint64_t byte_off;
    uint32_t len;
    uint32_t first_tile;
    uint32_t genome;
    uint32_t contig_index;
    uint32_t pad0, pad1;
};

struct SketchConsts {
    uint64_t thr, thr_marker;
    uint32_t kmask;
    int k, d, rshift;
    int delta;
};


constexpr int BSI_BLOG = 8;
constexpr uint32_t GSI_CONTIG_BITS = 15;
constexpr uint32_t SQ_MAX_TILES = 64, SQ_MAX_DESC = 64;
constexpr uint32_t SQ_SEEDS = 3072;
constexpr uint32_t SQ_MARKERS = 2048;
constexpr uint32_t SQ_ROWS = 64;
constexpr uint32_t SQ_CANDS = 256;
constexpr uint32_t SQ_HITS_FIRST = 256;
constexpr uint32_t SQ_F_SEEDS = 1u, SQ_F_MARKERS = 2u, SQ_F_PAIR = 4u;
struct SmallQHead {
    uint32_t n_seeds, n_markers_raw, n_markers, n_short;
    uint32_t flags, n_hits;
    unsigned long long n_anchors;
    uint32_t coff[SQ_MAX_DESC + 1];
    uint32_t done;
    uint32_t pad1[128 - 9 - (SQ_MAX_DESC + 1)];
};
static_assert(sizeof(SmallQHead) == 512, "the status block is 512 bytes, the hits follow it");
struct SmallQSketch {
    const uint8_t* d_bases; const ContigDesc* d_desc; const uint32_t* d_tci; const uint4* d_tinfo; const uint32_t* d_cft;
    uint32_t n_desc, n_tiles;
    uint32_t *d_packed; uint64_t* d_mask; uint32_t *d_cnt, *d_toff, *d_tmc;
    uint32_t *seed_kmer, *seed_pos, *seed_meta; uint64_t* seed_pm; uint64_t* mstage;
    SmallQHead* head;
};
psk_status small_query_sketch_enqueue(Lane* ctx, const psk_params* p, const SmallQSketch& A, hipStream_t st);

__device__ __forceinline__ uint64_t mm_hash64(uint64_t key) {
    key = ~(key + (key << 21));
    key = key ^ key >> 24;
    key = (key + (key << 3)) + (key << 8);
    key = key ^ key >> 14;
    key = (key + (key << 2)) + (key << 4);
    key = key ^ key >> 28;
    key = key + (key << 31);
    return key;
}

__device__ __forceinline__ uint64_t mm_hash64_u32(uint32_t key) {
    const uint64_t P = (uint64_t)key * 0x200001u;
    uint32_t lo = (uint32_t)P, hi = (uint32_t)(P >> 32);
    lo ^= __builtin_amdgcn_alignbit(hi, lo, 24);
    hi ^= 0xFFFFFF00u;
    uint64_t r = (uint64_t)lo * 265u;
    hi = hi * 265u + (uint32_t)(r >> 32);
    uint64_t x = ((uint64_t)hi << 32) | (uint32_t)r;
    x ^= x >> 14;
    lo = (uint32_t)x; hi = (uint32_t)(x >> 32);
    r = (uint64_t)lo * 21u;
    hi = hi * 21u + (uint32_t)(r >> 32);
    x = ((uint64_t)hi << 32) | (uint32_t)r;
    x ^= x >> 28;
    lo = (uint32_t)x; hi = (uint32_t)(x >> 32);
    r = (uint64_t)lo * 0x80000001u;
    hi = (hi << 31) + (uint32_t)(r >> 32) + hi;
    return ((uint64_t)hi << 32) | (uint32_t)r;
}

psk_status sketch_batch_impl(Lane* ctx, const psk_params* p, const uint8_t* d_bases,
                             const uint64_t* contig_off, const uint64_t* contig_len,
                             const uint32_t* genome_first_contig, uint32_t n_genomes,
                             int want_seeds, psk_sketch** out, const uint32_t* d_packed_in = nullptr);
extern "C" void psk_pack2bit_host(const uint8_t* src, uint64_t n, uint32_t* dst, int mode);
psk_status ensure_index(Lane* ctx, const psk_sketch* const* refs, uint32_t n, bool lazy = false);
psk_status ensure_probe(Lane* ctx, const psk_sketch* const* refs, uint32_t n);
__device__ __forceinline__ uint32_t probe_line(uint32_t km, uint32_t lines) { return __umulhi(km * 2654435761u, lines); }
psk_status screen_impl(Lane* ctx, psk_db* db, const psk_sketch* query, double screen_val, int rescue_small,
                       uint8_t* pass, uint32_t* shared);
psk_status chain_pairs_impl(Lane* ctx, const psk_sketch* const* refs, const psk_sketch* const* queries, uint32_t n,
                            const psk_query_opts* o, psk_hit* out);
void* hit_block_alloc(size_t bytes);
bool hit_block_free(void* p);
void hit_block_trim();
template <class H>
struct HitListT {
    H* p = nullptr; size_t n = 0, cap = 0;
    HitListT() = default;
    HitListT(const HitListT&) = delete; HitListT& operator=(const HitListT&) = delete;
    ~HitListT() { drop(p); }
    static void drop(void* q) { if (q && !hit_block_free(q)) free(q); }
    bool reserve(size_t want) {
        if (want <= cap) return true;
        if (n && want < 2 * cap) want = 2 * cap;
        const size_t bytes = sizeof(H) * want;
        H* q = (H*)(bytes >= ((size_t)8 << 20) ? hit_block_alloc(bytes) : malloc(bytes));
        if (!q) return false;
        if (n) memcpy(q, p, sizeof(H) * n);
        drop(p);
        p = q; cap = want;
        return true;
    }
    bool reserve_for(size_t k) { return n + k <= cap || reserve(std::max<size_t>(n + k, cap + cap / 2 + 64)); }
    bool append(const H* src, size_t k) {
        if (n + k > cap && !reserve(std::max<size_t>(n + k, cap + cap / 2 + 64))) return false;
        if (k) memcpy(p + n, src, sizeof(H) * k);
        n += k;
        return true;
    }
    H* release() { H* q = p; p = nullptr; n = cap = 0; return q; }
};
using HitList = HitListT<psk_hit>;
using HitListMin = HitListT<psk_hit_min>;
psk_status query_many_impl(Lane* ctx, psk_db* db, const psk_sketch* const* queries, uint32_t n_queries, const psk_query_opts* o,
                           HitList& all, uint64_t* offsets, const int64_t* keys = nullptr, uint64_t ref_base = 0);
psk_status query_many_min_impl(Lane* ctx, psk_db* db, const psk_sketch* const* queries, uint32_t n_queries, const psk_query_opts* o,
                               HitListMin& all, uint64_t* offsets, const int64_t* keys = nullptr, uint64_t ref_base = 0);
psk_status chain_impl(Lane* ctx, const psk_sketch* const* refs, uint32_t n_refs,
                      const psk_sketch* query, const psk_query_opts* o, psk_hit* out);
constexpr uint32_t SQ_MAX_REFS = 24 * 1024;
psk_status query_host_small(Lane* ctx, psk_db* db, const uint8_t* const* contigs, const uint64_t* lens, uint32_t n_contigs, const psk_query_opts* o,
                            HitList& all, bool* done);
psk_status small_query_prepare(Lane* ctx, psk_db* db, std::shared_lock<std::shared_mutex>& sh, bool* ok);
```

pyskani_amd/csrc/query_many.hip:

```cpp
#include "chain_stages.h"
#include "query_parts.h"
#include <hipcub/hipcub.hpp>
#include <algorithm>
#include <deque>
#include <thread>

constexpr uint32_t PF_SLOTS = 8192;
constexpr uint32_t PF_MAX_FILL = 4096;
constexpr int PF_T = 512;
constexpr uint32_t PF_EMPTY = 0xFFFFFFFFu;

__global__ __launch_bounds__(256) void pref_gather_kernel(const SketchDesc* __restrict__ qd, const uint32_t* __restrict__ rq, const uint32_t* __restrict__ eoff,
                                                          const uint32_t* __restrict__ qn, uint32_t n_resc, uint32_t* __restrict__ e_key, uint32_t* __restrict__ e_qid) {
    const uint32_t j = blockIdx.x;
    if (j >= n_resc) return;
    const uint32_t* __restrict__ km = qd[rq[j]].kmer;
    const uint32_t o = eoff[j], nn = qn[j];
    for (uint32_t i = threadIdx.x; i < nn; i += blockDim.x) { e_key[o + i] = km[i]; e_qid[o + i] = j; }
}

__global__ __launch_bounds__(PF_T) void pref_count_kernel(const uint32_t* __restrict__ e_key, const uint32_t* __restrict__ e_qid, uint32_t n_entries,
                                                         uint32_t slice_shift, const SketchDesc* __restrict__ rd, uint32_t n_refs, uint32_t refs_per_chunk,
                                                         uint32_t* __restrict__ cnt, uint32_t* __restrict__ overflow) {
    __shared__ uint32_t t_key[PF_SLOTS];
// ... 375 lines not shown
                if (db->bsi_state == 0) PSK_TRY(exclusive([&]() -> psk_status { return build_bsi(ctx, db); }));
                round_gsi = round_slice = round_bsi = db->bsi_state == 1;
            }
        }
        if (round_gsi) {
            round_probe = !round_slice;
            if (db->desc_dirty || db->desc_n != n) PSK_TRY(exclusive([&]() -> psk_status { return refresh_ref_descs(ctx, db); }));
        } else {
        {
            bool refs_stale = db->desc_dirty || db->desc_n != n;
            refs_stale = refs_stale || index_stamp(db) != db->desc_indexed;
            for (size_t i = 0; i < n_need_refs && !refs_stale; i++) refs_stale = !need[i]->idx && need[i]->n_seeds && need[i]->store;
            if (refs_stale)
                PSK_TRY(exclusive([&]() -> psk_status {
                    PSK_TRY(ensure_index(ctx, need.data(), (uint32_t)need.size()));
                    return refresh_ref_descs(ctx, db);
                }));
            else if (need.size() > n_need_refs) PSK_TRY(ensure_index(ctx, need.data() + n_need_refs, (uint32_t)(need.size() - n_need_refs)));
        }
        if (want_small) {
            round_probe = true;
            bool missing = false;
            for (size_t i = 0; i < n_need_refs; i++) {
                if (need[i]->n_seeds < 64 || need[i]->n_seeds > (1u << 22)) { round_probe = false; break; }
                missing = missing || !need[i]->ptab;
            }
            if (round_probe && missing)
                PSK_TRY(exclusive([&]() -> psk_status {
                    PSK_TRY(ensure_probe(ctx, need.data(), (uint32_t)n_need_refs));
                    return refresh_ref_descs(ctx, db);
                }));
        }
        }
        if (!(round_gsi && h_qd_gsi_round == (int64_t)b && h_qd.size() == m)) {
            h_qd.resize(m);
            for (uint32_t i = 0; i < m; i++) h_qd[i] = make_desc(queries[b + i], round_gsi);
        }
        PSK_TRY(ctx->q_h.reserve(sizeof(SketchDesc) * (size_t)m + 256));
        SketchDesc* d_qd = (SketchDesc*)ctx->q_h.p;
        PSK_HIP(hipMemcpyAsync(d_qd, h_qd.data(), sizeof(SketchDesc) * (size_t)m, hipMemcpyHostToDevice, st));
        const int items_env = sw.batch_items_log2.get() ? std::min(31, std::max(16, (int)sw.batch_items_log2.num(0))) : 0;
        int items_log2 = items_env ? items_env : 29;
        if (!items_env) for (uint32_t i = 0; i < m; i++) if (h_qd[i].n > (1u << 20)) { items_log2 = 27; break; }
        if (!items_env && items_log2 == 27) {
            size_t free_b = 0, total_b = 0;
            const size_t need = (size_t)212 << 30;
            if (hipMemGetInfo(&free_b, &total_b) == hipSuccess && free_b + ctx->q_d.cap + ctx->q_e.cap <= need && total_b > need) {
                psk_trim_idle_lanes(ctx->dev, ctx);
                if (lane2) { Scratch* big[] = {&lane2->lane->q_b, &lane2->lane->q_c, &lane2->lane->q_d, &lane2->lane->q_e, &lane2->lane->q_g, &lane2->lane->q_j, &lane2->lane->q_k, &lane2->lane->q_sel}; (void)hipStreamSynchronize(lane2->lane->stream); for (Scratch* s : big) s->release(); }
                (void)hipMemGetInfo(&free_b, &total_b);
            }
            if (free_b + ctx->q_d.cap + ctx->q_e.cap > need) items_log2 = 28;
        }
        const int pairs_env = sw.batch_pairs_log2.get() ? std::min(24, std::max(10, (int)sw.batch_pairs_log2.num(0))) : 0;
        if (!items_env && items_log2 == 29 && round_probe) items_log2 = 30;
        if (!items_env && items_log2 == 29 && round_slice) items_log2 = 30;
        uint64_t max_items = 1ull << items_log2, max_pairs = 1ull << (pairs_env ? pairs_env : (round_probe ? 22 : 21)), max_rows = 1ull << 26;
        {
            if (round_gsi && !round_slice && !sw.gsi_onepass.off() && !items_env && max_items == (1ull << 30)) max_items = 3ull << 28;
        }
        uint32_t qi = 0, rank = 0;
        std::vector<uint64_t> q_hits(m, 0);
        const size_t half_pairs = (size_t)std::min<uint64_t>(round_pairs, max_pairs);
        const size_t half_bytes = al256(sizeof(psk_hit) * half_pairs + 512);
        void* hpin2 = nullptr;
        PSK_TRY(ctx->pinned(2 * half_bytes, &hpin2));
        {
            size_t want = all.n + (size_t)std::min<uint64_t>(round_pairs, 1ull << 26);
            if (want > all.cap) {
                if (b == 0 && n_queries > m) want = std::max(want, (size_t)std::min<double>((double)round_pairs * ((double)n_queries / (double)m) * 1.05, (double)(1ull << 27)));
                if (b > 0 && all.n) want = std::max(want, (size_t)((double)all.n * ((double)n_queries / (double)b) * 1.1) + 4096);
            }
            if (round_pairs > 4096 && !all.reserve(want)) { psk_set_error("out of host memory"); return PSK_ENOMEM; }
        }
        int parity = 0;
        const H* pend_hits = nullptr; uint32_t pend_n = 0;
        bool pend_copy = false;
        hipStream_t cst = nullptr;
        struct CopyDrain { bool& pend; hipStream_t& s; ~CopyDrain() { if (pend && s) (void)hipStreamSynchronize(s); } } copy_drain{pend_copy, cst};
        const size_t sel_half = al256(sizeof(H) * half_pairs + 256);
        auto consume = [&]() -> psk_status {
            if (!pend_n) return PSK_OK;
            if (pend_copy) { PSK_HIP(hipStreamSynchronize(cst)); pend_copy = false; }
            const size_t old = all.n;
            if (!all.reserve_for(pend_n)) { psk_set_error("out of host memory"); return PSK_ENOMEM; }
            auto move = [&](size_t lo, size_t hi, bool shared) {
                memcpy(all.p + old + lo, pend_hits + lo, sizeof(H) * (hi - lo));
                for (size_t i = lo; i < hi; i++) {
                    H& h = all.p[old + i];
                    if (loc) h.ref_index = db->ref_of[h.ref_index];
                    const uint32_t lq = HitRec<H>::local_query(h);
                    if (shared) __atomic_fetch_add(&q_hits[lq], 1u, __ATOMIC_RELAXED); else q_hits[lq]++;
                    HitRec<H>::finish(h, b + lq);
                }
            };
            static const unsigned move_threads = [] { const EnvVal e = env_val("PSK_HIT_THREADS"); const unsigned hw = std::max(1u, std::thread::hardware_concurrency());
                                                      return e.text ? (unsigned)std::max(1, (int)e.num(0)) : std::min(8u, std::max(1u, hw / 8)); }();
            const unsigned nt = (size_t)pend_n * sizeof(H) >= ((size_t)16 << 20) ? move_threads : 1u;
            if (nt <= 1) move(0, pend_n, false);
            else {
                std::vector<std::thread> th;
                const size_t per = ((size_t)pend_n + nt - 1) / nt;
                size_t started = per;
                try {
                    th.reserve(nt);
                    for (unsigned t = 1; t < nt; t++) {
                        const size_t lo = std::min<size_t>(pend_n, t * per), hi = std::min<size_t>(pend_n, lo + per);
                        if (hi > lo) { th.emplace_back(move, lo, hi, true); started = hi; }
                    }
                } catch (...) {}
                move(0, std::min<size_t>(pend_n, per), true);
                if (started < pend_n) move(std::max(started, std::min<size_t>(pend_n, per)), pend_n, true);
                for (std::thread& t : th) t.join();
            }
            all.n += pend_n;
            pend_n = 0;
            return PSK_OK;
        };
        {
            const int pipe_env = (int)sw.pipeline.num(-1);
            const bool pipe_want = round_slice && pipe_env != 0 && (pipe_env == 1 || round_items >= (4ull << 29));
            if (pipe_want && !lane2) {
                lane2.reset(new (std::nothrow) LaneGuard(ctx->dev, true));
                if (lane2 && !lane2->lane) lane2.reset();
            }
            if (pipe_want && lane2) {
                if (!items_env) max_items = 1ull << 29;
                struct PipeJob {
                    uint32_t q0 = 0, r0 = 0, q1 = 0, r1 = 0;
                    std::vector<BatchQ> bqs; std::vector<uint2> tab, ebase; std::vector<uint32_t> qn;
                    uint64_t pairs = 0, items = 0, rows = 0, rows_pair_max = 0;
                    psk_status rc = PSK_OK; bool refit = false; char err[512] = "";
                    std::vector<H> hits; uint64_t anchors = 0, cands = 0, wrows = 0, visited = 0, lookups = 0; uint32_t misc[16] = {};
                };
                PipeJob job[2];
                std::thread th[2];
                bool live[2] = {false, false};
                Lane* lanes[2] = {ctx, lane2->lane};
                PSK_HIP(hipStreamSynchronize(st));
                const SketchDesc* d_rd = ref_descs();
                auto exec = [&](Lane* ln, PipeJob* Jp) {
                    PipeJob& J = *Jp;
                    (void)hipSetDevice(ln->device);
                    J.refit = false; J.hits.clear();
                    try {
                    J.rc = [&]() -> psk_status {
                        hipStream_t s2 = ln->stream;
                        const uint32_t n_pairs = (uint32_t)J.pairs;
                        ChainBufs L;
                        psk_status lrc = chain_layout(ln, n_pairs, (size_t)J.items, (size_t)J.rows, J.bqs.size(), &L);
                        if (lrc == PSK_ENOMEM) { J.refit = true; ctx->dev->rr_refit++; return PSK_OK; }
                        PSK_TRY(lrc);
                        L.rows_pair_max = (uint32_t)std::min<uint64_t>(J.rows_pair_max, 0xFFFFFFFFu);
                        L.g_key = (const uint32_t*)db->bsi_key.p; L.g_val = (const unsigned long long*)db->bsi_val.p; L.g_bucket = (const uint32_t*)db->bsi_bucket.p; L.g_shift = db->bsi_shift; L.g_nb1 = db->bsi_nb1; L.g_blocks = db->bsi_blocks; L.g_base = (const unsigned long long*)db->bsi_base.p;
                        L.d_pass = d_pass; L.n_refs = n; L.n_bq = (uint32_t)J.bqs.size();
                        uint32_t pm = 1; for (const BatchQ& e : J.bqs) pm = std::max(pm, e.rank_hi - e.rank_lo);
                        L.p_cap = (pm + 15u) & ~15u;
                        L.gsi_onepass = false;
                        J.qn.resize(J.bqs.size());
                        for (size_t e = 0; e < J.bqs.size(); e++) J.qn[e] = h_qd[J.bqs[e].q].n;
                        uint64_t n_rec = 0, n_sl = 0;
                        gsl_make_tab(J.bqs.data(), J.bqs.size(), J.qn.data(), J.tab, J.ebase, &n_rec, &n_sl);
                        if (n_rec >= 0x7FFFFF00ull) { psk_set_error("internal: %llu (pair, slice) records in one batch", (unsigned long long)n_rec); return PSK_ELIMIT; }
                        const size_t o_tab = 0, o_eb = al256(o_tab + 8 * J.tab.size()), o_cnt = al256(o_eb + 8 * J.ebase.size()), o_rec = al256(o_cnt + 4 * (size_t)n_rec),
                                     o_bm = al256(o_rec + 16 * (size_t)n_rec), o_un = al256(o_bm + 4 * (size_t)GSL_WORDS * (size_t)n_rec), o_endj = o_un + 4 * (size_t)GSL_WORDS * (size_t)n_sl;
                        lrc = ln->q_j.reserve(o_endj + 256);
                        if (lrc == PSK_ENOMEM) { J.refit = true; ctx->dev->rr_refit++; return PSK_OK; }
                        PSK_TRY(lrc);
                        char* Jb = (char*)ln->q_j.p;
                        PSK_HIP(hipMemcpyAsync(Jb + o_tab, J.tab.data(), 8 * J.tab.size(), hipMemcpyHostToDevice, s2));
                        PSK_HIP(hipMemcpyAsync(Jb + o_eb, J.ebase.data(), 8 * J.ebase.size(), hipMemcpyHostToDevice, s2));
                        L.gsi_slice = true; L.gsl_tab = (const uint2*)(Jb + o_tab); L.gsl_n_tab = (uint32_t)J.tab.size(); L.gsl_ebase = (const uint2*)(Jb + o_eb); L.gsl_un = (uint32_t*)(Jb + o_un); L.gsl_n_slices = (uint32_t)n_sl;
                        L.gsl_cnt = (uint32_t*)(Jb + o_cnt); L.gsl_rec = (uint4*)(Jb + o_rec); L.gsl_bm = (uint32_t*)(Jb + o_bm);
                        PSK_HIP(hipMemcpyAsync(L.bq, J.bqs.data(), sizeof(BatchQ) * J.bqs.size(), hipMemcpyHostToDevice, s2));
                        hipLaunchKernelGGL(pair_build_rows_kernel, dim3((uint32_t)J.bqs.size()), dim3(256), 0, s2, L.bq, d_pass, n, d_qd, d_rd, L.pairs, L.sbase, L.cbase, L.pair_qr, n_pairs, (uint32_t)J.items, (uint32_t)J.rows);
                        const bool host_filter = n_pairs <= 4096;
                        H* d_sel = nullptr;
                        if (!host_filter) { lrc = ln->q_sel.reserve(al256(sizeof(H) * (size_t)n_pairs + 256)); if (lrc == PSK_ENOMEM) { J.refit = true; ctx->dev->rr_refit++; return PSK_OK; } PSK_TRY(lrc); d_sel = (H*)ln->q_sel.p; }
                        void* hp = nullptr;
                        PSK_TRY(ln->pinned(al256(sizeof(psk_hit) * (size_t)n_pairs + 512), &hp));
                        ChainTail* T = (ChainTail*)hp; H* h_sel = (H*)((char*)hp + 256);
                        uint64_t cap = anchor_cap_for(ln, (size_t)J.items, false, false);
                        cap = std::min<uint64_t>(cap, std::max<uint64_t>(ln->q_d.cap / (4 * CHAIN_ANCHOR_WORDS) > 128 ? ln->q_d.cap / (4 * CHAIN_ANCHOR_WORDS) - 128 : 0, (uint64_t)J.items / 4 * 3 + 65536));
                        bool wide = sw.join_wide();
                        for (int attempt = 0;; attempt++) {
                            psk_status rrc = chain_run(ln, L, n_pairs, (size_t)J.items, (size_t)J.rows, db->params, o, d_qd, d_rd, cap, wide, sw, false);
                            if (rrc == PSK_ENOMEM) { (void)hipStreamSynchronize(s2); J.refit = true; ctx->dev->rr_refit++; return PSK_OK; }
                            PSK_TRY(rrc);
                            if (!host_filter) {
                                size_t tmp3 = 0;
                                hipcub::TransformInputIterator<H, ToRec<H>, const psk_hit*> rec_it(L.hits, ToRec<H>());
                                PSK_HIP(hipcub::DeviceSelect::If(nullptr, tmp3, rec_it, d_sel, L.misc + 12, (int)n_pairs, RecPasses<H>(), s2));
                                PSK_TRY(ln->q_c.reserve(tmp3));
                                PSK_HIP(hipcub::DeviceSelect::If(ln->q_c.p, tmp3, rec_it, d_sel, L.misc + 12, (int)n_pairs, RecPasses<H>(), s2));
                                PSK_HIP(hipMemcpyAsync(T, L.misc, sizeof(ChainTail), hipMemcpyDeviceToHost, s2));
                            } else PSK_HIP(hipMemcpyAsync(T, L.misc, 256 + sizeof(psk_hit) * (size_t)n_pairs, hipMemcpyDeviceToHost, s2));
                            PSK_HIP(hipStreamSynchronize(s2));
                            bool retry, was_wide = wide;
                            psk_status rc = chain_check(*T, n_pairs, &cap, &wide, &retry);
                            count_rerun(ctx->dev, was_wide, wide, retry);
                            if ((rc == PSK_ELIMIT && n_pairs > 1) || wide != was_wide) { J.refit = true; ctx->dev->rr_refit++; return PSK_OK; }
                            PSK_TRY(rc);
                            if (!retry) break;
                            if (attempt >= 3) { psk_set_error("internal: anchor capacity did not converge"); return PSK_EHIP; }
                        }
                        uint32_t n_sel = T->misc[12];
                        if (host_filter) {
                            const psk_hit* raw = (const psk_hit*)((char*)hp + 256);
                            for (uint32_t i = 0; i < n_pairs; i++) { const psk_hit r = raw[i]; if (r.ani > 0.1f) J.hits.push_back(HitRec<H>::from_raw(r)); }
                        } else if (n_sel) {
                            PSK_HIP(hipMemcpyAsync(h_sel, d_sel, sizeof(H) * (size_t)n_sel, hipMemcpyDeviceToHost, s2));
                            PSK_HIP(hipStreamSynchronize(s2));
                            J.hits.assign(h_sel, h_sel + n_sel);
                        }
                        J.anchors = T->total64; J.cands = T->cands; J.wrows = T->rows; J.visited = T->visited; memcpy(J.misc, T->misc, sizeof J.misc);
                        J.lookups = 0; for (const BatchQ& e : J.bqs) J.lookups += h_qd[e.q].n;
                        return PSK_OK;
                    }();
                    } catch (...) { psk_set_error("out of host memory"); J.rc = PSK_ENOMEM; }
                    if (J.rc != PSK_OK) snprintf(J.err, sizeof J.err, "%s", psk_last_error());
                    if (J.rc != PSK_OK || J.refit) (void)hipStreamSynchronize(ln->stream);
                    ln->huge_release();
                };
                bool refit = false;
                struct JoinAll { std::thread* t; ~JoinAll() { for (int i = 0; i < 2; i++) if (t[i].joinable()) t[i].join(); } } join_all{th};
                auto reap = [&](int sl) -> psk_status {
                    if (th[sl].joinable()) th[sl].join();
                    live[sl] = false;
                    PipeJob& J = job[sl];
                    if (J.rc != PSK_OK) { psk_set_error("%s", J.err); return J.rc; }
                    if (J.refit) { if (!refit) { refit = true; qi = J.q0; rank = J.r0; } return PSK_OK; }
                    if (refit) return PSK_OK;
                    const size_t nh = J.hits.size();
                    if (nh) {
                        if (!all.reserve_for(nh)) { psk_set_error("out of host memory"); return PSK_ENOMEM; }
                        memcpy(all.p + all.n, J.hits.data(), sizeof(H) * nh);
                        for (size_t i = 0; i < nh; i++) { H& h = all.p[all.n + i]; if (loc) h.ref_index = db->ref_of[h.ref_index]; const uint32_t lq = HitRec<H>::local_query(h); q_hits[lq]++; HitRec<H>::finish(h, b + lq); }
                        all.n += nh;
                    }
                    ctx->dev->w_pairs += J.pairs; ctx->dev->w_items += J.items; ctx->dev->w_anchors += J.anchors; ctx->dev->w_cands += J.cands; ctx->dev->w_rows += J.wrows; count_tier_pairs(ctx->dev, J.misc);
                    ctx->dev->w_lookups += J.lookups; ctx->dev->w_visited += J.visited;
                    return PSK_OK;
                };
                uint32_t k = 0;
                for (;;) {
                    while (qi < m && rank >= h_cnt[qi]) { qi++; rank = 0; }
                    if (qi >= m || refit) break;
                    const int sl = (int)(k & 1u);
                    if (live[sl]) { PSK_TRY(reap(sl)); if (refit) break; }
                    PipeJob& J = job[sl];
                    J.bqs.clear(); J.pairs = J.items = J.rows = J.rows_pair_max = 0;
                    J.q0 = qi; J.r0 = rank;
                    uint32_t pq = qi, pr = rank;
                    while (pq < m) {
                        const uint32_t left = h_cnt[pq] - pr;
                        if (left == 0) { pq++; pr = 0; continue; }
                        const uint64_t qn = h_qd[pq].n, qrows = h_qd[pq].rows;
                        uint64_t take = std::min<uint64_t>(left, max_pairs - J.pairs);
                        take = std::min<uint64_t>(take, GSI_PMAX);
                        if (qn) take = std::min<uint64_t>(take, (max_items - J.items) / qn);
                        if (qrows) take = std::min<uint64_t>(take, (max_rows - J.rows) / qrows);
                        if (take == 0) { if (J.pairs == 0) take = 1; else break; }
                        J.bqs.push_back(BatchQ{pq, pr, pr + (uint32_t)take, (uint32_t)J.pairs, (uint32_t)J.items, (uint32_t)J.rows});
                        J.rows_pair_max = std::max<uint64_t>(J.rows_pair_max, qrows);
                        J.pairs += take; J.items += take * qn; J.rows += take * qrows;
                        pr += (uint32_t)take;
                        if (J.pairs >= max_pairs || J.items >= max_items || J.rows >= max_rows) break;
                    }
                    J.q1 = pq; J.r1 = pr;
                    if (J.items >= 0xFFFFFF00ull || J.rows >= 0xFFFFFF00ull) { psk_set_error("a single pair exceeds the per-launch limits (%llu query seeds)", (unsigned long long)J.items); return PSK_ELIMIT; }
                    qi = pq; rank = pr;
                    if (J.items == 0 || J.rows == 0) continue;
                    try { th[sl] = std::thread(exec, lanes[sl], &J); }
                    catch (...) { exec(lanes[sl], &J); }
                    live[sl] = true;
                    k++;
                }
                for (int i = 0; i < 2; i++) { const int sl = (int)((k + (uint32_t)i) & 1u); if (live[sl]) PSK_TRY(reap(sl)); }
                if (refit) max_items = std::max<uint64_t>(1, max_items / 4);
            }
        }
        while (qi < m) {
            if (rank >= h_cnt[qi]) { qi++; rank = 0; continue; }
            bqs.clear();
            uint64_t pairs = 0, items = 0, rows = 0, rows_pair_max = 0;
            uint32_t pq = qi, pr = rank;
            while (pq < m) {
                const uint32_t left = h_cnt[pq] - pr;
                if (left == 0) { pq++; pr = 0; continue; }
                const uint64_t qn = h_qd[pq].n, qrows = h_qd[pq].rows;
                uint64_t take = std::min<uint64_t>(left, max_pairs - pairs);
                if (round_gsi) take = std::min<uint64_t>(take, GSI_PMAX);
                if (qn) take = std::min<uint64_t>(take, (max_items - items) / qn);
                if (qrows) take = std::min<uint64_t>(take, (max_rows - rows) / qrows);
                if (take == 0) { if (pairs == 0) take = 1; else break; }
                bqs.push_back(BatchQ{pq, pr, pr + (uint32_t)take, (uint32_t)pairs, (uint32_t)items, (uint32_t)rows});
                rows_pair_max = std::max<uint64_t>(rows_pair_max, qrows);
                pairs += take; items += take * qn; rows += take * qrows;
                pr += (uint32_t)take;
                if (pairs >= max_pairs || items >= max_items || rows >= max_rows) break;
            }
            const uint32_t n_pairs = (uint32_t)pairs;
            if (items >= 0xFFFFFF00ull || rows >= 0xFFFFFF00ull) { psk_set_error("a single pair exceeds the per-launch limits (%llu query seeds)", (unsigned long long)items); return PSK_ELIMIT; }
            uint32_t n_sel = 0;
            H* h_sel = nullptr;
            if (items == 0 || rows == 0) {
            } else {
                ChainBufs L;
                psk_status lrc = chain_layout(ctx, n_pairs, (size_t)items, (size_t)rows, bqs.size(), &L);
                L.rows_pair_max = (uint32_t)std::min<uint64_t>(rows_pair_max, 0xFFFFFFFFu);
                if (round_gsi) {
                    if (round_slice) { L.g_key = (const uint32_t*)db->bsi_key.p; L.g_val = (const unsigned long long*)db->bsi_val.p; L.g_bucket = (const uint32_t*)db->bsi_bucket.p; L.g_shift = db->bsi_shift; L.g_nb1 = db->bsi_nb1; L.g_blocks = db->bsi_blocks; L.g_base = (const unsigned long long*)db->bsi_base.p; }
                    else {
                        if (db->gsi_state == 1) { L.g_key = (const uint32_t*)db->gsi_key.p; L.g_val = (const unsigned long long*)db->gsi_val.p; L.g_bucket = (const uint32_t*)db->gsi_bucket.p; L.g_shift = db->gsi_shift; }
                        if (round_bsi) { L.b_key = (const uint32_t*)db->bsi_key.p; L.b_val = (const unsigned long long*)db->bsi_val.p; L.b_bucket = (const uint32_t*)db->bsi_bucket.p; L.b_shift = db->bsi_shift; L.b_nb1 = db->bsi_nb1; L.b_blocks = db->bsi_blocks; L.b_base = (const unsigned long long*)db->bsi_base.p; L.b_max = (uint32_t)std::max(1.0, max_blocks_join); }
                    }
                    L.d_pass = d_pass; L.n_refs = n; L.n_bq = (uint32_t)bqs.size();
                    uint32_t pm = 1; for (const BatchQ& e : bqs) pm = std::max(pm, e.rank_hi - e.rank_lo);
                    L.p_cap = round_slice ? (pm + 15u) & ~15u : (pm + 63u) & ~63u;
                    L.gsi_onepass = !sw.gsi_onepass.off() && !round_slice;
                    if (round_slice && lrc == PSK_OK) {
                        gsl_qn.resize(bqs.size());
                        for (size_t e = 0; e < bqs.size(); e++) gsl_qn[e] = h_qd[bqs[e].q].n;
                        uint64_t n_rec = 0, n_sl = 0;
                        gsl_make_tab(bqs.data(), bqs.size(), gsl_qn.data(), gsl_tab, gsl_ebase, &n_rec, &n_sl);
                        if (n_rec >= 0x7FFFFF00ull) { psk_set_error("internal: %llu (pair, slice) records in one batch", (unsigned long long)n_rec); return PSK_ELIMIT; }
                        const size_t o_tab = 0, o_eb = al256(o_tab + 8 * gsl_tab.size()), o_cnt = al256(o_eb + 8 * gsl_ebase.size()), o_rec = al256(o_cnt + 4 * (size_t)n_rec),
                                     o_bm = al256(o_rec + 16 * (size_t)n_rec), o_un = al256(o_bm + 4 * (size_t)GSL_WORDS * (size_t)n_rec), o_endj = o_un + 4 * (size_t)GSL_WORDS * (size_t)n_sl;
                        lrc = ctx->q_j.reserve(o_endj + 256);
                        if (lrc == PSK_OK) {
                            char* J = (char*)ctx->q_j.p;
                            PSK_HIP(hipMemcpyAsync(J + o_tab, gsl_tab.data(), 8 * gsl_tab.size(), hipMemcpyHostToDevice, st));
                            PSK_HIP(hipMemcpyAsync(J + o_eb, gsl_ebase.data(), 8 * gsl_ebase.size(), hipMemcpyHostToDevice, st));
                            L.gsi_slice = true; L.gsl_tab = (const uint2*)(J + o_tab); L.gsl_n_tab = (uint32_t)gsl_tab.size(); L.gsl_ebase = (const uint2*)(J + o_eb); L.gsl_un = (uint32_t*)(J + o_un); L.gsl_n_slices = (uint32_t)n_sl;
                            L.gsl_cnt = (uint32_t*)(J + o_cnt); L.gsl_rec = (uint4*)(J + o_rec); L.gsl_bm = (uint32_t*)(J + o_bm);
                        }
                    }
                }
                if (lrc == PSK_ENOMEM && n_pairs > 1 && max_items > (1ull << 22)) { max_items >>= 2; continue; }
                PSK_TRY(lrc);
                PSK_HIP(hipMemcpyAsync(L.bq, bqs.data(), sizeof(BatchQ) * bqs.size(), hipMemcpyHostToDevice, st));
                hipLaunchKernelGGL(pair_build_rows_kernel, dim3((uint32_t)bqs.size()), dim3(256), 0, st, L.bq, d_pass, n, d_qd, ref_descs(),
                                   L.pairs, L.sbase, L.cbase, L.pair_qr, n_pairs, (uint32_t)items, (uint32_t)rows);
                const bool host_filter = n_pairs <= 4096;
                H* d_sel = nullptr;
                if (!host_filter) {
                    PSK_TRY(ctx->copy_lane(&cst));
                    PSK_TRY(ctx->q_sel.reserve(2 * sel_half));
                    d_sel = (H*)((char*)ctx->q_sel.p + (parity ? sel_half : 0));
                }
                if (sizeof(psk_hit) * (size_t)n_pairs + 512 > half_bytes) { psk_set_error("internal: batch larger than its staging half"); return PSK_EHIP; }
                hpin = (char*)hpin2 + (parity ? half_bytes : 0);
                ChainTail* T = (ChainTail*)hpin; h_sel = (H*)((char*)hpin + 256);
                uint64_t cap = anchor_cap_for(ctx, (size_t)items, round_probe, items / n_pairs > (1u << 20));
                if (round_slice) cap = std::min<uint64_t>(cap, std::max<uint64_t>(ctx->q_d.cap / (4 * CHAIN_ANCHOR_WORDS) > 128 ? ctx->q_d.cap / (4 * CHAIN_ANCHOR_WORDS) - 128 : 0, (uint64_t)items / 4 * 3 + 65536));
                if (L.gsi_onepass) cap = std::min<uint64_t>(std::max<uint64_t>(cap, items + items / 8 + 8 * ((uint64_t)n_pairs + 1) + 64), 0x7FFFFF00ull);
                bool too_big = false, wide = sw.join_wide();
                static const bool trace_batch = getenv("PSK_TRACE_BATCH") != nullptr;
                for (int attempt = 0;; attempt++) {
                    struct timespec tb0{}, tb1{}, tb2{};
                    if (trace_batch) clock_gettime(CLOCK_MONOTONIC, &tb0);
                    psk_status rrc = chain_run(ctx, L, n_pairs, (size_t)items, (size_t)rows, db->params, o, d_qd, ref_descs(), cap, wide, sw, round_probe && !round_gsi);
                    if (trace_batch) clock_gettime(CLOCK_MONOTONIC, &tb1);
                    if (rrc == PSK_ENOMEM && n_pairs > 1 && max_items > (1ull << 22)) { (void)hipStreamSynchronize(st); ctx->huge_release(); too_big = true; break; }
                    PSK_TRY(rrc);
                    if (!host_filter) {
                        size_t tmp3 = 0;
                        hipcub::TransformInputIterator<H, ToRec<H>, const psk_hit*> rec_it(L.hits, ToRec<H>());
                        PSK_HIP(hipcub::DeviceSelect::If(nullptr, tmp3, rec_it, d_sel, L.misc + 12, (int)n_pairs, RecPasses<H>(), st));
                        PSK_TRY(ctx->q_c.reserve(tmp3));
                        PSK_HIP(hipcub::DeviceSelect::If(ctx->q_c.p, tmp3, rec_it, d_sel, L.misc + 12, (int)n_pairs, RecPasses<H>(), st));
                    }
                    if (host_filter) PSK_HIP(hipMemcpyAsync(T, L.misc, 256 + sizeof(psk_hit) * (size_t)n_pairs, hipMemcpyDeviceToHost, st));
                    else PSK_HIP(hipMemcpyAsync(T, L.misc, sizeof(ChainTail), hipMemcpyDeviceToHost, st));
                    PSK_TRY(consume());
                    PSK_HIP(hipStreamSynchronize(st));
                    if (trace_batch) {
                        clock_gettime(CLOCK_MONOTONIC, &tb2);
                        static struct timespec last{};
                        const double gap = last.tv_sec ? (tb0.tv_sec - last.tv_sec) * 1e3 + (tb0.tv_nsec - last.tv_nsec) / 1e6 : 0.0;
                        fprintf(stderr, "[psk batch] pairs %u items %llu attempt %d: since last %.1f ms, launch %.1f ms, wait %.1f ms; anchors %llu of %llu, status %x, wide %u -> %u\n", n_pairs, (unsigned long long)items, attempt, gap,
                                (tb1.tv_sec - tb0.tv_sec) * 1e3 + (tb1.tv_nsec - tb0.tv_nsec) / 1e6, (tb2.tv_sec - tb1.tv_sec) * 1e3 + (tb2.tv_nsec - tb1.tv_nsec) / 1e6,
                                (unsigned long long)T->total64, (unsigned long long)cap, T->misc[0], wide ? 1u : 0u, T->misc[5]);
                        last = tb2;
                    }
                    ctx->huge_release();
                    bool retry; const bool was_wide = wide;
                    psk_status rc = chain_check(*T, n_pairs, &cap, &wide, &retry);
                    count_rerun(ctx->dev, was_wide, wide, retry);
                    if (rc == PSK_ELIMIT && n_pairs > 1) { too_big = true; break; }
                    PSK_TRY(rc);
                    if (!retry && L.gsi_onepass && (T->misc[0] & 4u)) { L.gsi_onepass = false; retry = true; ctx->dev->rr_onepass++; }
                    if (!retry) {
                        ctx->dev->w_pairs += n_pairs; ctx->dev->w_items += items; ctx->dev->w_anchors += T->total64; ctx->dev->w_cands += T->cands; ctx->dev->w_rows += T->rows; count_tier_pairs(ctx->dev, T->misc);
                        if (round_gsi) { uint64_t lk = 0; for (const BatchQ& e : bqs) lk += h_qd[e.q].n; ctx->dev->w_lookups += lk; ctx->dev->w_visited += T->visited; }
                        break;
                    }
                    if (attempt >= 3) { psk_set_error("internal: anchor capacity did not converge"); return PSK_EHIP; }
                }
                if (too_big) { max_items = std::max<uint64_t>(1, items / 4); max_pairs = std::max<uint64_t>(1, pairs / 4); continue; }
                n_sel = T->misc[12];
                if (n_pairs <= 4096) {
                    const psk_hit* raw = (const psk_hit*)((char*)hpin + 256);
                    uint32_t w = 0;
                    for (uint32_t i = 0; i < n_pairs; i++) { const psk_hit r = raw[i]; if (r.ani > 0.1f) h_sel[w++] = HitRec<H>::from_raw(r); }
                    n_sel = w;
                }
                else if (n_sel) {
                    PSK_HIP(hipMemcpyAsync(h_sel, d_sel, sizeof(H) * (size_t)n_sel, hipMemcpyDeviceToHost, cst));
                    pend_copy = true;
                }
            }
            if (n_sel) { pend_hits = h_sel; pend_n = n_sel; parity ^= 1; }
            qi = pq; rank = pr;
        }
        PSK_TRY(consume());
        for (uint32_t i = 0; i < m; i++) offsets[b + i + 1] = offsets[b + i] + q_hits[i];
        if (loc)
            for (uint32_t i = 0; i < m; i++) {
                H* h0 = all.p + all0 + offsets[b + i]; H* h1 = all.p + all0 + offsets[b + i + 1];
                auto by_ref = [](const H& x, const H& y) { return x.ref_index < y.ref_index; };
                if (!std::is_sorted(h0, h1, by_ref)) std::sort(h0, h1, by_ref);
            }
    }
    return PSK_OK;
}
psk_status query_many_impl(Lane* ctx, psk_db* db, const psk_sketch* const* queries, uint32_t n_queries, const psk_query_opts* o, HitList& all, uint64_t* offsets, const int64_t* keys, uint64_t ref_base) {
    return query_many_t<psk_hit>(ctx, db, queries, n_queries, o, all, offsets, keys, ref_base);
}
psk_status query_many_min_impl(Lane* ctx, psk_db* db, const psk_sketch* const* queries, uint32_t n_queries, const psk_query_opts* o, HitListMin& all, uint64_t* offsets, const int64_t* keys, uint64_t ref_base) {
    return query_many_t<psk_hit_min>(ctx, db, queries, n_queries, o, all, offsets, keys, ref_base);
}
```

pyskani_amd/csrc/query_parts.h:

```cpp
#pragma once
#include "chain_stages.h"
#include <deque>
#include <vector>
#include <cstring>

static inline size_t al256(size_t x) { return (x + 255) & ~(size_t)255; }

struct SwitchVal {
    char text[24]; bool set;
    const char* get() const { return set ? text : nullptr; }
    bool off() const { return EnvVal{get()}.off(); }
    int force() const { return EnvVal{get()}.force(); }
    double num(double dflt) const { return EnvVal{get()}.num(dflt); }
};
#define PSK_SWITCHES(X) \
    X(chain_serial, "PSK_CHAIN_SERIAL") \
    X(join_pairs, "PSK_JOIN_PAIRS") \
    X(emit_pairs, "PSK_EMIT_PAIRS") \
    X(xcd_group, "PSK_XCD_GROUP") \
    X(chunk_hops, "PSK_CHUNK_HOPS") \
    X(emit_heads, "PSK_EMIT_HEADS") \
    X(hops_items, "PSK_HOPS_ITEMS") \
    X(emit_expand, "PSK_EMIT_EXPAND") \
    X(chain_lane, "PSK_CHAIN_LANE") \
    X(lane_xtrees, "PSK_LANE_XTREES") \
    X(chain_quad_deep, "PSK_CHAIN_QUAD_DEEP") \
    X(chain_wave_reg, "PSK_CHAIN_WAVE_REG") \
    X(select_tiny, "PSK_SELECT_TINY") \
    X(big_solo, "PSK_BIG_SOLO") \
    X(huge_slots, "PSK_HUGE_SLOTS") \
    X(huge_min_seeds, "PSK_HUGE_MIN_SEEDS") \
    X(reduce_small, "PSK_REDUCE_SMALL") \
    X(reduce_wave, "PSK_REDUCE_WAVE") \
    X(reduce_tiny, "PSK_REDUCE_TINY") \
    X(join, "PSK_JOIN") \
    X(round_queries, "PSK_ROUND_QUERIES") \
    X(screen, "PSK_SCREEN") \
    X(prefilter, "PSK_PREFILTER") \
    X(gsi_join, "PSK_GSI_JOIN") \
    X(gsl_max_blocks, "PSK_GSL_MAX_BLOCKS") \
    X(probe, "PSK_PROBE") \
    X(gsi_slice, "PSK_GSI_SLICE") \
    X(bsi_small, "PSK_BSI_SMALL") \
    X(batch_items_log2, "PSK_BATCH_ITEMS_LOG2") \
    X(batch_pairs_log2, "PSK_BATCH_PAIRS_LOG2") \
    X(gsi_onepass, "PSK_GSI_ONEPASS") \
    X(pipeline, "PSK_PIPELINE") \
    X(screen_global, "PSK_SCREEN_GLOBAL") \
    X(screen_wave, "PSK_SCREEN_WAVE") \
    X(locality, "PSK_LOCALITY")
struct Switches {
#define X(field, name) SwitchVal field;
    PSK_SWITCHES(X)
#undef X
    static Switches read();
    bool join_wide() const { const char* e = join.get(); return e && !strcmp(e, "wide"); }
};

struct ScreenStaging { std::deque<std::vector<MarkerSet>> hq; std::deque<std::vector<uint32_t>> qoff; };
psk_status upload_marker_table(Lane* ctx, psk_db* db);
psk_status build_inverted(Lane* ctx, psk_db* db);
psk_status screen_many_device(Lane* ctx, psk_db* db, const psk_sketch* const* queries, uint32_t nq, double screen_val, int rescue_small, uint8_t* d_pass, ScreenStaging& keep, const Switches& sw);

SketchDesc make_desc(const psk_sketch* s, bool unindexed_ok = false);
__global__ __launch_bounds__(256) void pair_build_rows_kernel(const BatchQ* __restrict__ bq, const uint8_t* __restrict__ pass, uint32_t n_refs,
                                                              const SketchDesc* __restrict__ qd, const SketchDesc* __restrict__ rd,
                                                              PairDesc* __restrict__ pairs, uint32_t* __restrict__ sbase, uint32_t* __restrict__ cbase,
                                                              uint2* __restrict__ pair_qr, uint32_t n_pairs, uint32_t n_items, uint32_t n_rows);
__global__ __launch_bounds__(256) void pass_canon_kernel(uint8_t* __restrict__ pass, uint32_t n_refs, const uint32_t* __restrict__ canon);
__global__ __launch_bounds__(256) void pass_triangle_kernel(uint8_t* __restrict__ pass, uint32_t n_refs, const long long* __restrict__ key, unsigned long long ref_base);
__global__ __launch_bounds__(256) void pass_count_kernel(const uint8_t* __restrict__ pass, uint32_t n_refs, uint32_t* __restrict__ row_count, uint8_t* __restrict__ col_flag, uint32_t* __restrict__ row_blocks);
constexpr size_t CHAIN_ANCHOR_WORDS = 14;
struct ChainBufs {
    PairDesc* pairs; uint32_t *sbase, *cbase, *pstart; uint2* lbcnt; uint32_t* aoff; uint32_t* nch; uint2* chunks; ChunkOut* cout;
    uint2* row_q0;
    psk_hit* hits; psk_hit* hits_sel; uint32_t* misc; uint32_t* ovf; unsigned long long* bsum; uint2* pair_qr; BatchQ* bq;
    uint32_t *blk_pair, *row_pair, *live, *big_list, *huge_list;
    uint32_t gi, gi_sum;
    unsigned long long* total;
    uint32_t rows_pair_max = 0xFFFFFFFFu;
    const uint32_t* g_key = nullptr; const unsigned long long* g_val = nullptr; const uint32_t* g_bucket = nullptr; int g_shift = 0;
    uint32_t g_nb1 = 0, g_blocks = 0; const unsigned long long* g_base = nullptr;
    const uint32_t* b_key = nullptr; const unsigned long long* b_val = nullptr; const uint32_t* b_bucket = nullptr; int b_shift = 0; uint32_t b_nb1 = 0, b_blocks = 0, b_max = 0; const unsigned long long* b_base = nullptr;
    const uint8_t* d_pass = nullptr; uint32_t n_refs = 0, n_bq = 0, p_cap = 0;
    bool gsi_slice = false; const uint2* gsl_tab = nullptr; uint32_t gsl_n_tab = 0; const uint2* gsl_ebase = nullptr; uint32_t *gsl_cnt = nullptr, *gsl_bm = nullptr, *gsl_un = nullptr, gsl_n_slices = 0; uint4* gsl_rec = nullptr;
    bool gsi_onepass = false;
};
psk_status chain_layout(Lane* ctx, size_t n_pairs, size_t n_items, size_t n_rows, size_t n_bq, ChainBufs* L);
psk_status chain_run(Lane* ctx, const ChainBufs& L, uint32_t n_pairs, size_t n_items, size_t n_rows, const psk_params& prm,
                     const psk_query_opts* o, const SketchDesc* d_qd, const SketchDesc* d_rd, uint64_t cap, bool wide, const Switches& sw, bool probe_ok = false);
uint64_t anchor_cap_for(Lane* ctx, size_t n_items, bool sparse = false, bool gb_scale = false);
struct ChainTail { uint32_t misc[16]; unsigned long long total64, visited, cands, rows; };
psk_status chain_check(const ChainTail& T, uint32_t n_pairs, uint64_t* cap, bool* wide, bool* retry);
static inline void count_rerun(psk_ctx* dev, bool was_wide, bool wide, bool retry) { if (wide && !was_wide) dev->rr_wide++; else if (retry) dev->rr_cap++; }
static inline void count_tier_pairs(psk_ctx* dev, const uint32_t* misc) { dev->tier[TIER_PAIRS_LIVE] += misc[9]; dev->tier[TIER_PAIRS_REST] += misc[13]; dev->tier[TIER_PAIRS_MID] += misc[14]; dev->tier[TIER_PAIRS_BIG] += misc[10]; }
struct HostPair { const psk_sketch* r; const psk_sketch* q; };
psk_status chain_batch(Lane* ctx, const HostPair* hp, uint32_t n_pairs, const psk_query_opts* o, psk_hit* out, const Switches& sw);

uint64_t index_stamp(const psk_db* db);
psk_status refresh_ref_descs(Lane* ctx, psk_db* db);

static inline uint32_t ref_at(const psk_db* db, uint32_t slot) { return db->loc_identity ? slot : db->ref_of[slot]; }
static inline uint32_t slot_at(const psk_db* db, uint32_t ref) { return db->loc_identity ? ref : db->slot_of[ref]; }
void pass_to_slots_launch(const uint8_t* in, uint8_t* out, uint32_t n_queries, uint32_t n_refs, const uint32_t* ref_of, hipStream_t st);

psk_status build_gsi(Lane* ctx, psk_db* db);
psk_status build_bsi(Lane* ctx, psk_db* db);
```

pyskani_amd/csrc/seed_index.hip:

```cpp
#include "query_parts.h"
#include <hipcub/hipcub.hpp>
#include <algorithm>

struct GsiSeg { const uint32_t* kmer; const uint64_t* pm; uint32_t n, off; };
__global__ __launch_bounds__(256) void gsi_gather_kernel(const GsiSeg* __restrict__ segs, uint32_t* __restrict__ key, unsigned long long* __restrict__ val) {
    const GsiSeg sg = segs[blockIdx.y];
    const unsigned long long ref = (unsigned long long)blockIdx.y << 48;
    for (uint32_t i = blockIdx.x * blockDim.x + threadIdx.x; i < sg.n; i += gridDim.x * blockDim.x) {
        const unsigned long long pm = sg.pm[i];
        const uint32_t meta = (uint32_t)pm;
        key[sg.off + i] = sg.kmer[i];
        val[sg.off + i] = ref | ((unsigned long long)(meta >> 1) << 33) | ((pm >> 32) << 1) | (meta & 1u);
    }
}
__global__ __launch_bounds__(256) void gsi_bucket_kernel(const uint32_t* __restrict__ key, uint32_t n, int shift, uint32_t nb, uint32_t* __restrict__ bucket) {
    const uint32_t i = blockIdx.x * 256u + threadIdx.x;
    if (i >= n) return;
    const uint32_t b = key[i] >> shift;
    const uint32_t from = i ? (key[i - 1] >> shift) + 1u : 0u;
    for (uint32_t x = from; x <= b; x++) bucket[x] = i;
    if (i == n - 1) for (uint32_t x = b + 1; x <= nb; x++) bucket[x] = n;
}
psk_status build_gsi(Lane* ctx, psk_db* db) {
    if (db->gsi_state) return PSK_OK;
    static const bool off = env_val("PSK_GSI").off();
    hipStream_t st = ctx->stream;
    const uint32_t n = (uint32_t)db->refs.size();
    db->gsi_state = 2;
    if (off || n == 0 || n > 65536u || db->params.k > 16) return PSK_OK;
    { const psk_status lrc = ensure_locality(ctx, db); if (lrc != PSK_OK) { db->gsi_state = 0; return lrc; } }
    std::vector<GsiSeg> segs(n);
    uint64_t N = 0; uint32_t maxn = 0;
    for (uint32_t i = 0; i < n; i++) {
        const psk_sketch* r = db->refs[ref_at(db, i)];
        if (!r->has_seeds || r->contig_len.size() > (1u << GSI_CONTIG_BITS) || r->params.k != db->params.k || r->params.c != db->params.c) return PSK_OK;
        const uint32_t ns = r->store ? (uint32_t)r->n_seeds : 0u;
        segs[i] = GsiSeg{ns ? r->store->seed_kmer + r->seed_off : nullptr, ns ? r->store->seed_pm + r->seed_off : nullptr, ns, (uint32_t)N};
        N += ns; maxn = std::max(maxn, ns);
        if (N >= 0x7FFFFF00ull) return PSK_OK;
    }
    if (N == 0) return PSK_OK;
    const int kbits = 2 * db->params.k;
    int bits = 4; while (bits < 26 && (8ull << bits) < N) bits++;
    if (bits > kbits) bits = kbits;
    const uint32_t nb = 1u << bits;
    size_t ts = 0;
    PSK_HIP(hipcub::DeviceRadixSort::SortPairs(nullptr, ts, (const uint32_t*)nullptr, (uint32_t*)nullptr, (const unsigned long long*)nullptr, (unsigned long long*)nullptr, (int)N, 0, kbits, st));
    PoolScratch tmp;
    const size_t o_k = 0, o_v = al256(4 * (size_t)N), o_t = al256(o_v + 8 * (size_t)N), o_s = al256(o_t + ts), o_end = o_s + sizeof(GsiSeg) * (size_t)n;
    psk_status rc = tmp.reserve(ctx->dev, o_end + 256);
    if (rc == PSK_OK) rc = db->gsi_key.reserve(ctx->dev, 4 * (size_t)N + 256);
    if (rc == PSK_OK) rc = db->gsi_val.reserve(ctx->dev, 8 * (size_t)N + 256);
    if (rc == PSK_OK) rc = db->gsi_bucket.reserve(ctx->dev, 4 * ((size_t)nb + 2));
    if (rc != PSK_OK) { db->gsi_key.release(); db->gsi_val.release(); db->gsi_bucket.release(); return rc == PSK_ENOMEM ? PSK_OK : rc; }
    char* T = (char*)tmp.p;
    auto fail = [&](hipError_t e, const char* what) -> psk_status {
        (void)hipStreamSynchronize(st);
        db->gsi_key.release(); db->gsi_val.release(); db->gsi_bucket.release();
        psk_set_error("%s: %s", what, hipGetErrorString(e));
        return PSK_OK;
    };
    hipError_t e = hipMemcpyAsync(T + o_s, segs.data(), sizeof(GsiSeg) * (size_t)n, hipMemcpyHostToDevice, st);
    if (e != hipSuccess) return fail(e, "gsi: upload");
    hipLaunchKernelGGL(gsi_gather_kernel, dim3(std::max(1u, std::min(64u, (maxn + 4095u) / 4096u)), n), dim3(256), 0, st, (const GsiSeg*)(T + o_s), (uint32_t*)(T + o_k), (unsigned long long*)(T + o_v));
    e = hipcub::DeviceRadixSort::SortPairs(T + o_t, ts, (const uint32_t*)(T + o_k), (uint32_t*)db->gsi_key.p, (const unsigned long long*)(T + o_v), (unsigned long long*)db->gsi_val.p, (int)N, 0, kbits, st);
    if (e != hipSuccess) return fail(e, "gsi: sort");
    hipLaunchKernelGGL(gsi_bucket_kernel, dim3((uint32_t)((N + 255) / 256)), dim3(256), 0, st, (const uint32_t*)db->gsi_key.p, (uint32_t)N, kbits - bits, nb, (uint32_t*)db->gsi_bucket.p);
    e = hipStreamSynchronize(st);
    if (e != hipSuccess) return fail(e, "gsi: build");
    db->gsi_n = N; db->gsi_shift = kbits - bits;
    db->gsi_state = 1;
    return PSK_OK;
}

__global__ __launch_bounds__(256) void bsi_bucket_kernel(const uint32_t* __restrict__ key, uint32_t n, int shift, uint32_t nb, uint32_t* __restrict__ bucket, uint32_t base) {
    const uint32_t i = blockIdx.x * 256u + threadIdx.x;
    if (n == 0) { for (uint32_t x = i; x <= nb; x += gridDim.x * 256u) bucket[x] = base; return; }
    if (i >= n) return;
    const uint32_t b = key[i] >> shift;
    const uint32_t from = i ? (key[i - 1] >> shift) + 1u : 0u;
    for (uint32_t x = from; x <= b; x++) bucket[x] = base + i;
    if (i == n - 1) for (uint32_t x = b + 1; x <= nb; x++) bucket[x] = base + n;
}
psk_status build_bsi(Lane* ctx, psk_db* db) {
    if (db->bsi_state) return PSK_OK;
    static const bool off = env_val("PSK_GSI").off();
    hipStream_t st = ctx->stream;
    const uint32_t n = (uint32_t)db->refs.size();
    db->bsi_state = 2;
    if (off || n == 0 || db->params.k > 16) return PSK_OK;
    { const psk_status lrc = ensure_locality(ctx, db); if (lrc != PSK_OK) { db->bsi_state = 0; return lrc; } }
    const uint32_t n_blocks = (n + (1u << BSI_BLOG) - 1) >> BSI_BLOG;
    std::vector<GsiSeg> segs(n);
    std::vector<uint64_t> base(n_blocks + 1, 0);
    uint64_t N = 0, max_block = 0; uint32_t maxn = 0;
    for (uint32_t b = 0; b < n_blocks; b++) {
        const uint32_t r0 = b << BSI_BLOG, r1 = std::min<uint32_t>(n, (b + 1) << BSI_BLOG);
        uint64_t in_block = 0;
        for (uint32_t i = r0; i < r1; i++) {
            const psk_sketch* r = db->refs[ref_at(db, i)];
            if (!r->has_seeds || r->contig_len.size() > (1u << GSI_CONTIG_BITS) || r->params.k != db->params.k || r->params.c != db->params.c) return PSK_OK;
            const uint32_t ns = r->store ? (uint32_t)r->n_seeds : 0u;
            if (in_block + ns >= 0x7FFFFF00ull) return PSK_OK;
            segs[i] = GsiSeg{ns ? r->store->seed_kmer + r->seed_off : nullptr, ns ? r->store->seed_pm + r->seed_off : nullptr, ns, (uint32_t)in_block};
            in_block += ns; maxn = std::max(maxn, ns);
        }
        base[b] = N; N += in_block; max_block = std::max(max_block, in_block);
    }
    base[n_blocks] = N;
    if (N == 0) return PSK_OK;
    const int kbits = 2 * db->params.k;
    int bits = 4; while (bits < 24 && (8ull << bits) < max_block) bits++;
    if (bits > kbits) bits = kbits;
    const uint32_t nb = 1u << bits;
    size_t ts = 0;
    PSK_HIP(hipcub::DeviceRadixSort::SortPairs(nullptr, ts, (const uint32_t*)nullptr, (uint32_t*)nullptr, (const unsigned long long*)nullptr, (unsigned long long*)nullptr, (int)max_block, 0, kbits, st));
    PoolScratch tmp;
    const size_t o_k = 0, o_v = al256(4 * (size_t)max_block), o_t = al256(o_v + 8 * (size_t)max_block), o_s = al256(o_t + ts), o_end = o_s + sizeof(GsiSeg) * (size_t)n;
    psk_status rc = tmp.reserve(ctx->dev, o_end + 256);
    if (rc == PSK_OK) rc = db->bsi_key.reserve(ctx->dev, 4 * (size_t)N + 256);
    if (rc == PSK_OK) rc = db->bsi_val.reserve(ctx->dev, 8 * (size_t)N + 256);
    if (rc == PSK_OK) rc = db->bsi_bucket.reserve(ctx->dev, 4 * ((size_t)n_blocks * (nb + 1) + 2));
    if (rc == PSK_OK) rc = db->bsi_base.reserve(ctx->dev, 8 * ((size_t)n_blocks + 1) + 256);
    auto drop = [&]() { db->bsi_key.release(); db->bsi_val.release(); db->bsi_bucket.release(); db->bsi_base.release(); };
    if (rc != PSK_OK) { drop(); if (rc == PSK_ENOMEM) return PSK_OK; return rc; }
    char* T = (char*)tmp.p;
    auto fail = [&](hipError_t e, const char* what) -> psk_status {
        (void)hipStreamSynchronize(st);
        drop();
        psk_set_error("%s: %s", what, hipGetErrorString(e));
        return PSK_OK;
    };
    hipError_t e = hipMemcpyAsync(T + o_s, segs.data(), sizeof(GsiSeg) * (size_t)n, hipMemcpyHostToDevice, st);
    if (e == hipSuccess) e = hipMemcpyAsync(db->bsi_base.p, base.data(), 8 * ((size_t)n_blocks + 1), hipMemcpyHostToDevice, st);
    if (e != hipSuccess) return fail(e, "bsi: upload");
    for (uint32_t b = 0; b < n_blocks; b++) {
        const uint32_t r0 = b << BSI_BLOG, r1 = std::min<uint32_t>(n, (b + 1) << BSI_BLOG);
        const size_t o = (size_t)base[b]; const uint32_t cnt = (uint32_t)(base[b + 1] - base[b]);
        if (cnt) {
            hipLaunchKernelGGL(gsi_gather_kernel, dim3(std::max(1u, std::min(64u, (maxn + 4095u) / 4096u)), r1 - r0), dim3(256), 0, st, (const GsiSeg*)(T + o_s) + r0, (uint32_t*)(T + o_k), (unsigned long long*)(T + o_v));
            size_t ts_b = ts;
            e = hipcub::DeviceRadixSort::SortPairs(T + o_t, ts_b, (const uint32_t*)(T + o_k), (uint32_t*)db->bsi_key.p + o, (const unsigned long long*)(T + o_v), (unsigned long long*)db->bsi_val.p + o, (int)cnt, 0, kbits, st);
            if (e != hipSuccess) return fail(e, "bsi: sort");
        }
        hipLaunchKernelGGL(bsi_bucket_kernel, dim3(std::max(1u, (cnt + 255u) / 256u)), dim3(256), 0, st, (const uint32_t*)db->bsi_key.p + o, cnt, kbits - bits, nb, (uint32_t*)db->bsi_bucket.p + (size_t)b * (nb + 1), 0u);
    }
    e = hipStreamSynchronize(st);
    if (e != hipSuccess) return fail(e, "bsi: build");
    db->bsi_n = N; db->bsi_shift = kbits - bits; db->bsi_nb1 = nb + 1; db->bsi_blocks = n_blocks;
    db->bsi_state = 1;
    return PSK_OK;
}

psk_status small_query_prepare(Lane* ctx, psk_db* db, std::shared_lock<std::shared_mutex>& sh, bool* ok) {
    *ok = false;
    const int state = db->small_state.load(std::memory_order_acquire);
    if (state == 1) { *ok = true; return PSK_OK; }
    if (state == 2) return PSK_OK;
    const uint32_t n = (uint32_t)db->refs.size();
    if (n == 0 || n > SQ_MAX_REFS) return PSK_OK;
    for (const psk_sketch* r : db->refs)
        if (!r->has_seeds || !r->store || r->params.k != db->params.k || r->params.c != db->params.c) { db->small_state = 2; return PSK_OK; }
    sh.unlock();
    psk_status rc = PSK_OK;
    {
        std::unique_lock<std::shared_mutex> ex(db->rw);
        if (db->refs.size() == n && db->small_state.load() == 0) {
            auto build = [&]() -> psk_status {
                PSK_TRY(upload_marker_table(ctx, db));
                PSK_TRY(build_inverted(ctx, db));
                if (db->has_dups && db->canon_dirty) {
                    PSK_TRY(db->d_canon.reserve(ctx->dev, 4 * (size_t)n));
                    PSK_HIP(hipMemcpyAsync(db->d_canon.p, db->canon.data(), 4 * (size_t)n, hipMemcpyHostToDevice, ctx->stream));
                    db->canon_dirty = false;
                }
                std::vector<const psk_sketch*> all_refs(db->refs.begin(), db->refs.end());
                PSK_TRY(ensure_index(ctx, all_refs.data(), (uint32_t)all_refs.size()));
                PSK_TRY(refresh_ref_descs(ctx, db));
                PSK_HIP(hipStreamSynchronize(ctx->stream));
                PSK_TRY(build_gsi(ctx, db));
                return PSK_OK;
            };
            rc = build();
            if (rc == PSK_OK) db->small_state.store(1, std::memory_order_release);
        }
    }
    sh.lock();
    PSK_TRY(rc);
    *ok = db->small_state.load(std::memory_order_acquire) == 1 && db->refs.size() == n;
    return PSK_OK;
}
```

pyskani_amd/csrc/slice_join.h:

```cpp
#pragma once
#include "common.h"

struct BatchQ { uint32_t q, rank_lo, rank_hi, pair_off, item_off, row_off; };
constexpr uint32_t GSI_PMAX = 256;

#ifndef GSL_SEEDS_N
#define GSL_SEEDS_N 256
#endif
constexpr uint32_t GSL_SEEDS = GSL_SEEDS_N;
constexpr uint32_t GSL_WORDS = GSL_SEEDS / 32;
constexpr uint32_t GSL_BT_WORDS = 12;
struct GslArgs {
    const BatchQ* bq; uint32_t n_entries;
    const uint2* tab; uint32_t n_tab;
    const uint2* ebase;
    uint32_t* un; uint32_t n_slices;
    const uint8_t* pass; uint32_t n_refs; const SketchDesc* qd;
    const uint32_t* g_key; const unsigned long long* g_val; const uint32_t* g_bucket; int g_shift;
    const unsigned long long* g_base;
    uint32_t g_nb1, g_blocks;
    uint32_t* blk_tab; uint32_t* blk_cnt; uint32_t blk_cap;
    uint32_t* cnt;
    uint4* rec;
    uint32_t* bm;
    uint32_t* pair_cnt;
    const uint32_t* pstart; uint2* anc; uint32_t cap; uint32_t* err;
    uint32_t p_cap;
    uint2* chunks; uint32_t* n_chunks;
    uint2* row_q0;
};

void gsl_make_tab(const BatchQ* bq, size_t n_entries, const uint32_t* q_seeds , std::vector<uint2>& tab, std::vector<uint2>& ebase, uint64_t* n_records, uint64_t* n_slices);
psk_status gsl_blocks_launch(const BatchQ* bq, uint32_t n_entries, const uint8_t* pass, uint32_t n_refs, uint32_t g_blocks, const unsigned long long* g_base,
                             uint32_t* blk_tab, uint32_t* blk_cnt, uint32_t blk_cap, hipStream_t st);
psk_status gsl_count_launch(const GslArgs& A, hipStream_t st);
psk_status gsl_heads_launch(const GslArgs& A, hipStream_t st);
psk_status gsl_emit_launch(const GslArgs& A, hipStream_t st);
```

pyskani_amd/csrc/slice_join.hip:

```cpp
#include "slice_join.h"
#include "chain_dev.h"

void gsl_make_tab(const BatchQ* bq, size_t n_entries, const uint32_t* q_seeds, std::vector<uint2>& tab, std::vector<uint2>& ebase, uint64_t* n_records, uint64_t* n_slices) {
    tab.clear(); ebase.resize(n_entries);
    uint64_t rec = 0, nsl_all = 0; uint32_t max_sl = 0;
    for (size_t e = 0; e < n_entries; e++) {
        const uint32_t nsl = (q_seeds[e] + GSL_SEEDS - 1) / GSL_SEEDS;
        ebase[e] = make_uint2((uint32_t)rec, (uint32_t)nsl_all);
        rec += (uint64_t)nsl * (bq[e].rank_hi - bq[e].rank_lo);
        nsl_all += nsl;
        max_sl = std::max(max_sl, nsl);
    }
    *n_records = rec; *n_slices = nsl_all;
    (void)max_sl;
    for (size_t e = 0; e < n_entries; e++) for (uint32_t sl = 0; sl < (q_seeds[e] + GSL_SEEDS - 1) / GSL_SEEDS; sl++) tab.push_back(make_uint2((uint32_t)e, sl));
}

#ifndef GSL_LINE_N
#define GSL_LINE_N 4
#endif
constexpr uint32_t GSL_LW = GSL_LINE_N, GSL_LM = GSL_LW - 1u, GSL_LS = GSL_LW == 8 ? 3u : GSL_LW == 4 ? 2u : 1u;
static_assert(GSL_LW == 8 || GSL_LW == 4 || GSL_LW == 2, "a staged line holds eight, four or two anchors");
static size_t gsl_walk_lds(const GslArgs& A, bool emit) {
    const size_t nw = (A.n_refs + 63) / 64;
    (void)nw;
    return (emit ? (8 * GSL_LW + 8 + 8) * (size_t)A.p_cap + 8 * 64 : 0) + 64 + 4 * (size_t)A.p_cap + (emit ? 0 : 4 * (size_t)GSL_WORDS * (A.p_cap + 1));
}

template <bool EMIT>
__global__ __launch_bounds__(64) void gsl_walk_kernel(GslArgs A) {
    extern __shared__ uint4 s_gsl[];
    const int lane = threadIdx.x;
    const uint2 te = A.tab[blockIdx.x];
    if (te.x == 0xFFFFFFFFu) return;
    if (EMIT && (A.err[5] || *(const unsigned long long*)(A.err + 16) > A.cap)) return;
    const BatchQ B = A.bq[te.x];
    const SketchDesc Q = A.qd[B.q];
    const uint32_t sb = te.y * GSL_SEEDS;
    if (sb >= Q.n) return;
    const uint32_t se = Q.n - sb > GSL_SEEDS ? sb + GSL_SEEDS : Q.n;
    const uint32_t P = B.rank_hi - B.rank_lo, pc = A.p_cap;
    const uint2 eb = A.ebase[te.x];
    const uint32_t rec0 = eb.x + te.y * P;
    uint2* s_line = (uint2*)s_gsl;
    unsigned long long* s_lim = (unsigned long long*)(s_line + (EMIT ? GSL_LW * pc : 0u));
    uint2* s_cs = (uint2*)(s_lim + (EMIT ? pc : 0u));
    uint2* s_fl = s_cs + (EMIT ? pc : 0u);
    uint2* s_bp = s_fl + (EMIT ? 64u : 0u);
    uint32_t* s_cur = (uint32_t*)(s_bp + 8u);
    uint32_t* s_rows = s_cur;
    uint32_t* s_bm = s_cur + pc;
    {
        if (EMIT) for (uint32_t j = lane; j < P; j += 64) { const uint4 v = A.rec[rec0 + j]; s_cs[j] = make_uint2(v.x, v.x); s_rows[j] = v.y; s_lim[j] = ((unsigned long long)v.w << 32) | v.z; }
        else {
            for (uint32_t j = lane; j < P; j += 64) s_cur[j] = 0;
            for (uint32_t x = lane; x < GSL_WORDS * (pc + 1u); x += 64) s_bm[x] = 0;
        }
    }
    uint32_t unw = 0;
    if (EMIT && lane < (int)GSL_WORDS) unw = A.un[(size_t)(eb.y + te.y) * GSL_WORDS + lane];
    lds_wave_sync();
    constexpr uint32_t GSL_AHEAD = 4;
    unsigned long long visited = 0;
    const uint32_t n_blk = A.blk_cnt[te.x];
    const uint32_t* __restrict__ brow = A.blk_tab + (size_t)te.x * A.blk_cap * GSL_BT_WORDS;
#pragma unroll 1
    for (uint32_t bi = 0; bi < n_blk; bi++, brow += GSL_BT_WORDS) {
    {
    const uint32_t blk = brow[8];
    const unsigned long long x_base = ((unsigned long long)brow[11] << 32) | brow[10];
    const uint32_t* __restrict__ x_key = A.g_key + x_base; const unsigned long long* __restrict__ x_val = A.g_val + x_base;
    {
        lds_wave_sync();
        if (lane < 8) {
            uint32_t run = brow[9];
#pragma unroll
            for (int u = 0; u < 7; u++) { const uint32_t w = brow[u]; if (u < lane) run += (uint32_t)__popc(w); }
            s_bp[lane] = make_uint2(brow[lane], run);
        }
        lds_wave_sync();
    }
    const uint32_t* __restrict__ bkt = A.g_bucket + (size_t)blk * A.g_nb1;
    uint32_t km1 = sb + (uint32_t)lane < se ? Q.kmer[sb + lane] : 0u, km2 = sb + 64u + (uint32_t)lane < se ? Q.kmer[sb + 64u + lane] : 0u;
    uint32_t lo1 = 0, hi1 = 0;
    if (sb + (uint32_t)lane < se) { const uint32_t b = km1 >> A.g_shift; lo1 = bkt[b]; hi1 = bkt[b + 1]; }
    for (uint32_t c0 = sb; c0 < se; c0 += 64) {
        const uint32_t i = c0 + (uint32_t)lane;
        const uint32_t km = km1, lo = lo1, hi = hi1;
        km1 = km2; lo1 = 0; hi1 = 0;
        if (i + 64u < se) { const uint32_t b = km1 >> A.g_shift; lo1 = bkt[b]; hi1 = bkt[b + 1]; }
        km2 = i + 128u < se ? Q.kmer[i + 128u] : 0u;
        uint32_t qp = 0, qm = 0;
        if (EMIT && i < se) { qp = Q.pos[i]; qm = Q.meta[i]; }
        const uint32_t nst = (hi - lo + 63u) >> 6;
        if (!EMIT) visited += hi - lo;
        uint32_t pre = nst;
#pragma unroll
        for (int o = 1; o < 64; o <<= 1) { const uint32_t y = __shfl_up(pre, o); if (lane >= o) pre += y; }
        const uint32_t T = (uint32_t)__builtin_amdgcn_readlane((int)pre, 63);
        pre -= nst;
        uint32_t ns[GSL_AHEAD], nx[GSL_AHEAD], nh[GSL_AHEAD], nk[GSL_AHEAD]; unsigned long long nv[GSL_AHEAD];
#define GSL_FETCH(t, u) do { \
            ns[u] = 0; nx[u] = 0; nh[u] = 0; nk[u] = 0xFFFFFFFFu; nv[u] = 0ull; \
            if ((t) < T) { \
                const unsigned long long own = __ballot(nst != 0 && pre <= (t)); \
                ns[u] = 63u - (uint32_t)__clzll((long long)own); \
                nx[u] = (uint32_t)__builtin_amdgcn_readlane((int)lo, (int)ns[u]) + 64u * ((t) - (uint32_t)__builtin_amdgcn_readlane((int)pre, (int)ns[u])); \
                nh[u] = (uint32_t)__builtin_amdgcn_readlane((int)hi, (int)ns[u]); \
                if (nx[u] + (uint32_t)lane < nh[u]) { nk[u] = x_key[nx[u] + lane]; nv[u] = x_val[nx[u] + lane]; } \
            } } while (0)
#pragma unroll
        for (uint32_t u = 0; u < GSL_AHEAD; u++) GSL_FETCH(u, u);
        for (uint32_t t0 = 0; t0 < T; t0 += GSL_AHEAD) {
            uint32_t cs[GSL_AHEAD], cx[GSL_AHEAD], ch[GSL_AHEAD], ck[GSL_AHEAD]; unsigned long long cv[GSL_AHEAD];
#pragma unroll
            for (uint32_t u = 0; u < GSL_AHEAD; u++) { cs[u] = ns[u]; cx[u] = nx[u]; ch[u] = nh[u]; ck[u] = nk[u]; cv[u] = nv[u]; }
#pragma unroll
            for (uint32_t u = 0; u < GSL_AHEAD; u++) GSL_FETCH(t0 + GSL_AHEAD + u, u);
            uint32_t slots[GSL_AHEAD]; uint2 bps[GSL_AHEAD];
#pragma unroll
            for (uint32_t u = 0; u < GSL_AHEAD; u++) bps[u] = s_bp[(uint32_t)(cv[u] >> 53) & 7u];
#pragma unroll
            for (uint32_t u = 0; u < GSL_AHEAD; u++) {
                const uint32_t skm = (uint32_t)__builtin_amdgcn_readlane((int)km, (int)cs[u]);
                const uint32_t b = (uint32_t)(cv[u] >> 48) & 31u, rk = bps[u].y + (uint32_t)__popc(bps[u].x & ~(~0u << b)) - B.rank_lo;
                const bool ok = cx[u] + (uint32_t)lane < ch[u] && ck[u] == skm && ((bps[u].x >> b) & 1u) && rk < P;
                slots[u] = ok ? rk : 0xFFFFFFFFu;
            }
#pragma unroll
            for (uint32_t u = 0; u < GSL_AHEAD; u++) {
                if (t0 + u >= T) break;
                const uint32_t s = cs[u]; const unsigned long long v = cv[u];
                const uint32_t slot = slots[u];
                const bool valid = slot != 0xFFFFFFFFu;
                if (!__any(valid)) continue;
                const uint32_t jl = c0 - sb + s;
                if (!EMIT) {
                    if (valid) { atomicAdd(&s_cur[slot], 1u); atomicOr(&s_bm[(jl >> 5) * (pc + 1u) + slot], 1u << (jl & 31u)); }
                    continue;
                }
                const uint32_t sqp = (uint32_t)__builtin_amdgcn_readlane((int)qp, (int)s), sqm = (uint32_t)__builtin_amdgcn_readlane((int)qm, (int)s);
                const uint32_t rmeta = (uint32_t)((((v >> 33) & ((1ull << GSI_CONTIG_BITS) - 1ull)) << 1) | (v & 1ull));
                const uint32_t prev = (uint32_t)__builtin_amdgcn_update_dpp(-1, (int)slot, 0x138 , 0xf, 0xf, false);
                const bool same = valid && prev == slot;
                const bool dup = __ballot(same) != 0;
                const uint2 cs = s_cs[valid ? slot : 0u];
                const unsigned long long lim = s_lim[valid ? slot : 0u];
                const uint32_t base = cs.x;
                bool opens = false;
                if (((uint32_t)__builtin_amdgcn_readlane((int)unw, (int)(jl >> 5)) >> (jl & 31u)) & 1u) {
                    const unsigned long long key1 = (((unsigned long long)(sqm >> 1) << 32) | sqp) + 1ull;
                    opens = valid && key1 > lim;
                    if (opens && !same) {
                        const uint32_t row = s_rows[slot], idxc = base < A.cap ? base : A.cap;
                        if (row < Q.rows) {
                            const size_t ri = (size_t)B.row_off + (size_t)slot * Q.rows + row;
                            uint2* r = A.chunks + ri;
                            r->x = idxc;
                            if (row > 0) r[-1].y = idxc;
                            A.row_q0[ri] = make_uint2(sqp, sqm >> 1);
                        } else atomicOr(A.err, 1u);
                        s_rows[slot] = row + 1u; s_lim[slot] = key1 + FRAGMENT_LENGTH;
                    }
                }
                const uint32_t q_rel = opens ? 0u : sqp - (uint32_t)(lim - 1ull - FRAGMENT_LENGTH);
                const uint2 av = pk_anchor(q_rel, (uint32_t)(v >> 1), (rmeta & ~1u) | ((rmeta ^ sqm) & 1u));
                if (!dup) {
                    const uint32_t t3 = base & GSL_LM;
                    if (valid) { s_cs[slot].x = base + 1u; s_line[t3 * pc + slot] = av; }
                    const bool fl = valid && t3 == GSL_LM;
                    const unsigned long long fm = __ballot(fl);
                    if (fm) {
                        if (fl) {
                            const uint32_t st0 = cs.y, lb = base & ~GSL_LM, ft = lb >= st0 ? 0u : st0 - lb;
                            s_fl[__popcll(fm & ((1ull << lane) - 1ull))] = make_uint2(slot | (ft << 16), lb);
                        }
                        lds_wave_sync();
                        const uint32_t nf = (uint32_t)__popcll(fm), t = (uint32_t)lane & GSL_LM;
                        for (uint32_t g0 = 0; g0 < nf; g0 += 64u / GSL_LW) {
                            const uint32_t r2 = g0 + ((uint32_t)lane >> GSL_LS);
                            if (r2 < nf) { const uint2 f = s_fl[r2]; if (t >= (f.x >> 16)) A.anc[f.y + t] = s_line[t * pc + (f.x & 0xFFFFu)]; }
                        }
                    }
                    continue;
                }
                const uint32_t st0 = cs.y;
                const uint32_t next = (uint32_t)__builtin_amdgcn_update_dpp(-1, (int)slot, 0x130 , 0xf, 0xf, false);
                const bool last = valid && next != slot;
                const unsigned long long starts = __ballot(valid && !same);
                const unsigned long long upto = starts & (lane == 63 ? ~0ull : ((2ull << lane) - 1ull));
                const uint32_t jj = valid ? (uint32_t)lane - (63u - (uint32_t)__clzll((long long)upto)) : 0u;
                const unsigned long long ends = __ballot(last);
                const uint32_t tail = valid ? (uint32_t)__ffsll((long long)(ends >> lane)) - 1u : 0u;
                const uint32_t d = base + jj, e = d + tail, lastline = e >> GSL_LS;
                if (valid && jj == 0 && (base >> GSL_LS) != lastline && e < A.cap) {
                    const uint32_t f0 = (base & ~GSL_LM) > st0 ? (base & ~GSL_LM) : st0;
                    for (uint32_t t = f0; t < base; t++) A.anc[t] = s_line[(t & GSL_LM) * pc + slot];
                }
                lds_wave_sync();
                if (valid) {
                    if ((d >> GSL_LS) == lastline) s_line[(d & GSL_LM) * pc + slot] = av;
                    else if (e < A.cap) A.anc[d] = av;
                }
                lds_wave_sync();
                if (last) {
                    if (e >= A.cap) atomicOr(A.err, 2u);
                    else if ((e & GSL_LM) == GSL_LM) {
                        const uint32_t f0 = (e & ~GSL_LM) > st0 ? (e & ~GSL_LM) : st0;
                        for (uint32_t t = f0; t <= e; t++) A.anc[t] = s_line[(t & GSL_LM) * pc + slot];
                    }
                    s_cs[slot].x = e + 1u;
                }
                lds_wave_sync();
            }
        }
#undef GSL_FETCH
    }
    }
    }
    lds_wave_sync();
    if (!EMIT) {
#pragma unroll
        for (int o = 32; o > 0; o >>= 1) visited += __shfl_xor(visited, o);
        if (lane == 0 && visited) atomicAdd((unsigned long long*)(A.err + 18), visited);
        for (uint32_t j = lane; j < P; j += 64) {
            const uint32_t c = s_cur[j];
            A.cnt[rec0 + j] = c;
            if (c) atomicAdd(&A.pair_cnt[B.pair_off + j], c);
        }
        for (uint32_t x = lane; x < P * GSL_WORDS; x += 64) { const uint32_t j = x / GSL_WORDS, w = x % GSL_WORDS; A.bm[(size_t)(rec0 + j) * GSL_WORDS + w] = s_bm[w * (pc + 1u) + j]; }
    } else {
        for (uint32_t j = lane; j < P; j += 64) {
            const uint32_t c = s_cs[j].x, st0 = s_cs[j].y;
            if (c > st0 && (c & GSL_LM) && c <= A.cap) {
                const uint32_t f0 = ((c - 1u) & ~GSL_LM) > st0 ? ((c - 1u) & ~GSL_LM) : st0;
                for (uint32_t t = f0; t < c; t++) A.anc[t] = s_line[(t & GSL_LM) * pc + j];
            }
        }
    }
}

constexpr uint32_t GSL_HK = GSL_SEEDS / 64;
__global__ __launch_bounds__(64) void gsl_heads_kernel(GslArgs A) {
    __shared__ unsigned long long s_key[GSL_SEEDS];
    __shared__ uint32_t s_bm[64 * (GSL_WORDS + 1)];
    __shared__ uint32_t s_un[GSL_WORDS];
    const int lane = threadIdx.x;
    const uint32_t e = blockIdx.x;
    const BatchQ B = A.bq[e];
    const uint32_t P = B.rank_hi - B.rank_lo, j = blockIdx.y * 64u + (uint32_t)lane;
    if (blockIdx.y * 64u >= P) return;
    const SketchDesc Q = A.qd[B.q];
    const bool act = j < P;
    const uint32_t nsl = (Q.n + GSL_SEEDS - 1u) / GSL_SEEDS;
    const uint32_t p = B.pair_off + j;
    const uint2 eb = A.ebase[e];
    const bool guard = A.err[5] || *(const unsigned long long*)(A.err + 16) > A.cap;
    uint32_t cursor = act ? A.pstart[p] : 0u;
    const uint32_t pend = act ? A.pstart[p + 1] : 0u;
    const bool live = act && !guard && pend - cursor >= MIN_ANCHORS;
    uint32_t rows = 0; unsigned long long lim1 = live ? 0ull : ~0ull;
    uint32_t* my_bm = s_bm + lane * (GSL_WORDS + 1);
    struct HSlice { uint32_t kp[GSL_HK], kmt[GSL_HK]; uint4 bw[GSL_WORDS / 4]; uint32_t c; };
    HSlice S0, S1;
    auto load_slice = [&](HSlice& X, uint32_t sl) {
        const uint32_t sb = sl * GSL_SEEDS;
#pragma unroll
        for (uint32_t u = 0; u < GSL_HK; u++) { const uint32_t i = sb + u * 64u + (uint32_t)lane; X.kp[u] = 0; X.kmt[u] = 0; if (i < Q.n) { X.kp[u] = Q.pos[i]; X.kmt[u] = Q.meta[i]; } }
        const size_t r = (size_t)eb.x + (size_t)sl * P + j;
        X.c = 0;
#pragma unroll
        for (uint32_t u = 0; u < GSL_WORDS / 4; u++) X.bw[u] = make_uint4(0, 0, 0, 0);
        if (act) {
            X.c = A.cnt[r];
            const uint4* __restrict__ src = (const uint4*)(A.bm + r * GSL_WORDS);
#pragma unroll
            for (uint32_t u = 0; u < GSL_WORDS / 4; u++) X.bw[u] = src[u];
        }
    };
    auto step = [&](HSlice& X, uint32_t sl) {
        const uint32_t sb = sl * GSL_SEEDS, ns = Q.n - sb > GSL_SEEDS ? GSL_SEEDS : Q.n - sb;
        const size_t r = (size_t)eb.x + (size_t)sl * P + j;
        lds_wave_sync();
        if (lane < (int)GSL_WORDS) s_un[lane] = 0;
#pragma unroll
        for (uint32_t u = 0; u < GSL_HK; u++) s_key[u * 64u + lane] = (((unsigned long long)(X.kmt[u] >> 1) << 32) | X.kp[u]) + 1ull;
#pragma unroll
        for (uint32_t u = 0; u < GSL_WORDS / 4; u++) { my_bm[4 * u] = X.bw[u].x; my_bm[4 * u + 1] = X.bw[u].y; my_bm[4 * u + 2] = X.bw[u].z; my_bm[4 * u + 3] = X.bw[u].w; }
        const uint32_t c = X.c;
        if (sl + 2 < nsl) load_slice(X, sl + 2);
        lds_wave_sync();
        if (act) {
            A.rec[r] = make_uint4(cursor, rows, (uint32_t)lim1, (uint32_t)(lim1 >> 32));
            if (live && c) {
                uint32_t from = 0;
                for (;;) {
                    {
                        uint32_t lo = from, hi = ns;
                        while (lo < hi) { const uint32_t mid = (lo + hi) >> 1; if (s_key[mid] > lim1) hi = mid; else lo = mid + 1; }
                        from = lo;
                    }
                    if (from >= ns) break;
                    uint32_t w = from >> 5, x = my_bm[w] & (~0u << (from & 31u));
                    while (!x && ++w < GSL_WORDS) x = my_bm[w];
                    if (!x) break;
                    const uint32_t jl = w * 32u + (uint32_t)__ffs((int)x) - 1u;
                    lim1 = s_key[jl] + FRAGMENT_LENGTH; rows++;
                    atomicOr(&s_un[w], 1u << (jl & 31u));
                    from = jl + 1u;
                }
            }
            cursor += c;
        }
        lds_wave_sync();
        if (lane < (int)GSL_WORDS && s_un[lane]) atomicOr(&A.un[(size_t)(eb.y + sl) * GSL_WORDS + lane], s_un[lane]);
    };
    load_slice(S0, 0);
    if (nsl > 1) load_slice(S1, 1);
    for (uint32_t sl = 0; sl < nsl; sl += 2) {
        step(S0, sl);
        if (sl + 1 < nsl) step(S1, sl + 1);
    }
    if (act) {
        if (live && rows) {
            if (rows - 1u < Q.rows) A.chunks[(size_t)B.row_off + (size_t)j * Q.rows + rows - 1u].y = pend < A.cap ? pend : A.cap; else atomicOr(A.err, 1u);
        }
        A.n_chunks[p] = live ? (rows < Q.rows ? rows : Q.rows) : 0u;
    }
}

__global__ __launch_bounds__(64) void gsl_blocks_kernel(const BatchQ* __restrict__ bq, uint32_t n_entries, const uint8_t* __restrict__ pass, uint32_t n_refs, uint32_t g_blocks,
                                                        const unsigned long long* __restrict__ g_base, uint32_t* __restrict__ blk_tab, uint32_t* __restrict__ blk_cnt, uint32_t blk_cap) {
    static_assert(BSI_BLOG == 8, "four ballots of 64 references = one index block");
    const uint32_t e = blockIdx.x;
    if (e >= n_entries) return;
    const int lane = threadIdx.x;
    const BatchQ B = bq[e];
    const uint8_t* __restrict__ row = pass + (size_t)B.q * n_refs;
    uint32_t* __restrict__ out = blk_tab + (size_t)e * blk_cap * GSL_BT_WORDS;
    uint32_t run = 0, cnt = 0;
    for (uint32_t blk = 0; blk < g_blocks && run < B.rank_hi; blk++) {
        uint8_t f[4];
#pragma unroll
        for (int u = 0; u < 4; u++) { const uint32_t r = (blk * 4u + u) * 64u + (uint32_t)lane; f[u] = r < n_refs ? row[r] : (uint8_t)0; }
        unsigned long long m[4]; uint32_t n_here = 0;
#pragma unroll
        for (int u = 0; u < 4; u++) { m[u] = __ballot(f[u] != 0); n_here += (uint32_t)__popcll(m[u]); }
        if (n_here && run + n_here > B.rank_lo) {
            if (cnt < blk_cap) {
                uint32_t w = 0;
#pragma unroll
                for (int u = 0; u < 4; u++) { if (lane == 2 * u) w = (uint32_t)m[u]; if (lane == 2 * u + 1) w = (uint32_t)(m[u] >> 32); }
                const unsigned long long base = g_base[blk];
                if (lane == 8) w = blk; if (lane == 9) w = run; if (lane == 10) w = (uint32_t)base; if (lane == 11) w = (uint32_t)(base >> 32);
                if (lane < (int)GSL_BT_WORDS) out[(size_t)cnt * GSL_BT_WORDS + lane] = w;
            }
            cnt++;
        }
        run += n_here;
    }
    if (lane == 0) blk_cnt[e] = cnt < blk_cap ? cnt : blk_cap;
}
psk_status gsl_blocks_launch(const BatchQ* bq, uint32_t n_entries, const uint8_t* pass, uint32_t n_refs, uint32_t g_blocks, const unsigned long long* g_base,
                             uint32_t* blk_tab, uint32_t* blk_cnt, uint32_t blk_cap, hipStream_t st) {
    if (!n_entries) return PSK_OK;
    hipLaunchKernelGGL(gsl_blocks_kernel, dim3(n_entries), dim3(64), 0, st, bq, n_entries, pass, n_refs, g_blocks, g_base, blk_tab, blk_cnt, blk_cap);
    PSK_HIP(hipGetLastError());
    return PSK_OK;
}
psk_status gsl_count_launch(const GslArgs& A, hipStream_t st) {
    hipLaunchKernelGGL(gsl_walk_kernel<false>, dim3(A.n_tab), dim3(64), gsl_walk_lds(A, false), st, A);
    PSK_HIP(hipGetLastError());
    return PSK_OK;
}
psk_status gsl_heads_launch(const GslArgs& A, hipStream_t st) {
    PSK_HIP(hipMemsetAsync(A.un, 0, 4 * (size_t)GSL_WORDS * A.n_slices, st));
    hipLaunchKernelGGL(gsl_heads_kernel, dim3(A.n_entries, (A.p_cap + 63u) / 64u), dim3(64), 0, st, A);
    PSK_HIP(hipGetLastError());
    return PSK_OK;
}
psk_status gsl_emit_launch(const GslArgs& A, hipStream_t st) {
    hipLaunchKernelGGL(gsl_walk_kernel<true>, dim3(A.n_tab), dim3(64), gsl_walk_lds(A, true), st, A);
    PSK_HIP(hipGetLastError());
    return PSK_OK;
}
```

rust/ffi.rs:

```rust
use std::os::raw::{c_char, c_int, c_void};

#[repr(C)] pub struct PskCtx { _p: [u8; 0] }
#[repr(C)] pub struct PskSketch { _p: [u8; 0] }
#[repr(C)] pub struct PskDb { _p: [u8; 0] }
#[repr(C)] pub struct PskModel { _p: [u8; 0] }
#[repr(C)] pub struct PskComm { _p: [u8; 0] }
pub const PSK_COMM_ID_BYTES: usize = 128;

#[repr(C)] #[derive(Clone, Copy)]
pub struct PskParams { pub c: i32, pub marker_c: i32, pub k: i32 }

#[repr(C)] #[derive(Clone, Copy)]
pub struct PskQueryOpts {
    pub learned_ani: i32, pub median: i32, pub robust: i32, pub faster_small: i32,
    pub cutoff: f64, pub min_aligned_frac: f64,
    pub model: *const PskModel,
}

#[repr(C)] #[derive(Clone, Copy, Default)]
pub struct PskHit {
    pub ani: f32, pub af_query: f32, pub af_ref: f32, pub ref_index: u32,
    pub n_chunks: u32, pub n_intervals: u32,
    pub n_anchors: u64, pub covered_query: u64, pub covered_ref: u64,
    pub sum_chain_anchors: u64, pub sum_chunk_seeds: u64,
    pub ani_raw: f32, pub ani_std: f32, pub learned: u32, pub reserved: u32,
}
#[repr(C)] #[derive(Clone, Copy)]
pub struct PskHitMin { pub ani: f32, pub af_query: f32, pub af_ref: f32, pub ref_index: u32, pub query: u32 }
#[repr(C)] #[derive(Clone, Copy)]
pub struct PskClusterOpts { pub min_ani: f64, pub min_af: f64, pub af_rule: i32, pub linkage: i32 }
#[repr(C)] #[derive(Clone, Copy)]
pub struct PskSeed { pub kmer: u32, pub pos: u32, pub contig: u32, pub canon: u32 }
#[repr(C)] #[derive(Clone, Copy)]
pub struct PskTreeNode { pub feature: i32, pub threshold: f32, pub left: i32, pub right: i32,
                         pub value: f32, pub missing: i32, pub is_leaf: i32, pub reserved: i32 }

#[link(name = "pyskani_amd")]
extern "C" {
    pub fn psk_last_error() -> *const c_char;
    pub fn psk_version() -> *const c_char;
    pub fn psk_abi_version() -> c_int;
    pub fn psk_free(p: *mut c_void);
    pub fn psk_ctx_create(device: c_int, out: *mut *mut PskCtx) -> c_int;
    pub fn psk_ctx_destroy(ctx: *mut PskCtx);
    pub fn psk_ctx_synchronize(ctx: *mut PskCtx) -> c_int;
    pub fn psk_ctx_set_timing(ctx: *mut PskCtx, on: c_int) -> c_int;
    pub fn psk_ctx_timing(ctx: *mut PskCtx, kernel: *const c_char, total_ms: *mut f64, launches: *mut u64) -> c_int;
    pub fn psk_ctx_clock_probe(ctx: *mut PskCtx, mhz: *mut f64, ms: *mut f64) -> c_int;
    pub fn psk_ctx_work(ctx: *mut PskCtx, pairs: *mut u64, items: *mut u64, anchors: *mut u64, reset: c_int) -> c_int;
    pub fn psk_ctx_join_work(ctx: *mut PskCtx, lookups: *mut u64, visited: *mut u64, candidates: *mut u64, rows: *mut u64, reset: c_int) -> c_int;
    pub fn psk_device_alloc(ctx: *mut PskCtx, bytes: usize, dptr: *mut *mut c_void) -> c_int;
    pub fn psk_device_free(ctx: *mut PskCtx, dptr: *mut c_void) -> c_int;
    pub fn psk_memcpy_h2d(ctx: *mut PskCtx, dst: *mut c_void, src: *const c_void, bytes: usize) -> c_int;
    pub fn psk_sketch_host(ctx: *mut PskCtx, p: *const PskParams, contigs: *const *const u8,
                           lens: *const u64, n_contigs: u32, want_seeds: c_int,
                           out: *mut *mut PskSketch) -> c_int;
    pub fn psk_sketch_many_host(ctx: *mut PskCtx, p: *const PskParams, contigs: *const *const u8, lens: *const u64,
                                genome_first_contig: *const u32, n_genomes: u32, want_seeds: c_int,
                                out: *mut *mut PskSketch) -> c_int;
    pub fn psk_sketch_batch_device(ctx: *mut PskCtx, p: *const PskParams, d_bases: *const u8, contig_off: *const u64,
                                   contig_len: *const u64, genome_first_contig: *const u32, n_genomes: u32,
                                   want_seeds: c_int, out: *mut *mut PskSketch) -> c_int;
    pub fn psk_sketch_free(s: *mut PskSketch);
    pub fn psk_sketch_free_many(sketches: *const *mut PskSketch, n: u32);
    pub fn psk_sketch_info(s: *const PskSketch, p: *mut PskParams, n_seeds: *mut u64, n_markers: *mut u64,
                           total_len: *mut u64, n_contigs: *mut u32) -> c_int;
    pub fn psk_sketch_export(s: *const PskSketch, seeds: *mut PskSeed, markers: *mut u64) -> c_int;
    pub fn psk_sketch_contig_lens(s: *const PskSketch, lens: *mut u32) -> c_int;
    pub fn psk_sketch_import(ctx: *mut PskCtx, p: *const PskParams, contig_lens: *const u32, n_contigs: u32,
                             seeds: *const PskSeed, n_seeds: u64, markers: *const u64, n_markers: u64,
                             has_seeds: c_int, out: *mut *mut PskSketch) -> c_int;
    pub fn psk_sketch_pack_size(s: *const PskSketch, bytes: *mut u64) -> c_int;
    pub fn psk_sketch_pack(s: *const PskSketch, d_dst: *mut c_void, capacity: u64) -> c_int;
    pub fn psk_sketch_unpack(ctx: *mut PskCtx, d_src: *const c_void, capacity: u64, offsets: *const u64, n: u32,
                             out: *mut *mut PskSketch) -> c_int;
    pub fn psk_sketch_pack_many(sketches: *const *const PskSketch, n: u32, d_dst: *mut c_void, offsets: *const u64, capacity: u64) -> c_int;
    pub fn psk_comm_unique_id(id: *mut c_void) -> c_int;
    pub fn psk_comm_create(ctx: *mut PskCtx, rank: c_int, world: c_int, id: *const c_void, out: *mut *mut PskComm) -> c_int;
    pub fn psk_comm_destroy(comm: *mut PskComm);
    pub fn psk_comm_info(comm: *const PskComm, rank: *mut c_int, world: *mut c_int, bytes_sent: *mut u64, collectives: *mut u64) -> c_int;
    pub fn psk_gather_hits(comm: *mut PskComm, local: *const PskHit, n_local: u64, all: *mut *mut PskHit, n_all: *mut u64, counts: *mut u64) -> c_int;
    pub fn psk_gather_hits_min(comm: *mut PskComm, local: *const PskHitMin, n_local: u64, all: *mut *mut PskHitMin, n_all: *mut u64, counts: *mut u64) -> c_int;
    pub fn psk_gather_sketches(comm: *mut PskComm, mine: *const *const PskSketch, n: u32, all: *mut *mut *mut PskSketch, counts: *mut u32) -> c_int;
    pub fn psk_model_create(ctx: *mut PskCtx, nodes: *const PskTreeNode, n_nodes: u64, tree_first_node: *const u32,
                            n_trees: u32, bias: f32, shrinkage: f32, features: *const i32, n_features: u32,
                            out: *mut *mut PskModel) -> c_int;
    pub fn psk_model_load_json(ctx: *mut PskCtx, json: *const c_char, len: usize, out: *mut *mut PskModel) -> c_int;
    pub fn psk_model_load_file(ctx: *mut PskCtx, path: *const c_char, out: *mut *mut PskModel) -> c_int;
    pub fn psk_model_free(m: *mut PskModel);
    pub fn psk_model_info(m: *const PskModel, n_trees: *mut u32, n_nodes: *mut u64, n_features: *mut u32) -> c_int;
    pub fn psk_model_predict(m: *const PskModel, rows: *const f32, n_rows: u32, out: *mut f32) -> c_int;
    pub fn psk_ctx_small_query_stats(ctx: *mut PskCtx, taken: *mut u64, rerun: *mut u64, general: *mut u64) -> c_int;
    pub fn psk_ctx_rerun_stats(ctx: *mut PskCtx, cap: *mut u64, wide: *mut u64, onepass: *mut u64, refit: *mut u64, reset: c_int) -> c_int;
    pub fn psk_ctx_tier_stats(ctx: *mut PskCtx, out: *mut u64, n: c_int, reset: c_int) -> c_int;
    pub fn psk_pack2bit_host(src: *const u8, n: u64, dst: *mut u32, mode: c_int);
    pub fn psk_db_create(ctx: *mut PskCtx, p: *const PskParams, out: *mut *mut PskDb) -> c_int;
    pub fn psk_db_destroy(db: *mut PskDb);
    pub fn psk_db_add(db: *mut PskDb, name: *const c_char, s: *mut PskSketch) -> c_int;
    pub fn psk_db_add_batch(db: *mut PskDb, names: *const *const c_char, sketches: *const *mut PskSketch, n: u32) -> c_int;
    pub fn psk_db_size(db: *const PskDb) -> u32;
    pub fn psk_db_name(db: *const PskDb, index: u32) -> *const c_char;
    pub fn psk_db_sketch(db: *const PskDb, index: u32) -> *const PskSketch;
    pub fn psk_query(db: *mut PskDb, q: *const PskSketch, o: *const PskQueryOpts,
                     hits: *mut *mut PskHit, n_hits: *mut u64) -> c_int;
    pub fn psk_query_host(db: *mut PskDb, contigs: *const *const u8, lens: *const u64, n_contigs: u32, seed: c_int, o: *const PskQueryOpts,
                          hits: *mut *mut PskHit, n_hits: *mut u64) -> c_int;
    pub fn psk_query_many(db: *mut PskDb, qs: *const *const PskSketch, n: u32, o: *const PskQueryOpts,
                          hits: *mut *mut PskHit, offsets: *mut u64) -> c_int;
    pub fn psk_query_many_min(db: *mut PskDb, qs: *const *const PskSketch, n: u32, o: *const PskQueryOpts,
                              hits: *mut *mut PskHitMin, offsets: *mut u64) -> c_int;
    pub fn psk_query_many_tri(db: *mut PskDb, qs: *const *const PskSketch, n: u32, key: *const i64, ref_base: u64, o: *const PskQueryOpts,
                              hits: *mut *mut PskHit, offsets: *mut u64) -> c_int;
    pub fn psk_query_many_tri_min(db: *mut PskDb, qs: *const *const PskSketch, n: u32, key: *const i64, ref_base: u64, o: *const PskQueryOpts,
                                  hits: *mut *mut PskHitMin, offsets: *mut u64) -> c_int;
    pub fn psk_cluster_records(ctx: *mut PskCtx, recs: *const PskHitMin, n_recs: u64, n_genomes: u32, priority: *const u64, opts: *const PskClusterOpts,
                               rep_of: *mut u32, rep_ani: *mut f32, n_reps: *mut u32) -> c_int;
    pub fn psk_ctx_cluster_stats(ctx: *mut PskCtx, edges: *mut u64, rounds: *mut u64, hook_passes: *mut u64) -> c_int;
    pub fn psk_db_locality(db: *mut PskDb, slot_of: *mut u32, n_groups: *mut u32, is_identity: *mut u32) -> c_int;
    pub fn psk_screen(db: *mut PskDb, q: *const PskSketch, screen_val: f64, rescue_small: c_int,
                      pass: *mut u8, shared: *mut u32) -> c_int;
    pub fn psk_chain(ctx: *mut PskCtx, refs: *const *const PskSketch, n: u32, q: *const PskSketch,
                     o: *const PskQueryOpts, out: *mut PskHit) -> c_int;
}

pub fn check(status: c_int) -> pyo3::PyResult<()> {
    use pyo3::exceptions::*;
    if status == 0 { return Ok(()); }
    let msg = unsafe { std::ffi::CStr::from_ptr(psk_last_error()) }.to_string_lossy().into_owned();
    Err(match status {
        1 => PyValueError::new_err(msg),
        2 => PyMemoryError::new_err(msg),
        5 => PyKeyError::new_err(msg),
        6 => PyOverflowError::new_err(msg),
        _ => PyRuntimeError::new_err(msg),
    })
}
```

Before: 209.0 million genome-pairs/s.

## Tag block seed-index values with low k-mer bits to skip key loads

When the bucket table is fine enough that each bucket fixes all but the low 8 k-mer bits, the block seed index stores those 8 bits in the top byte of each value word. The slice-join walk then matches on the tag instead of loading the separate key array, which removes one global load stream from the hot gather loop. In exchange the bucket table grows (more bits), and the new planner enables tagging only when that table stays within a size budget relative to the entry count, or when an env override forces it. A small info API exposes the chosen plan.

```diff
diff --git a/include/pyskani_amd.h b/include/pyskani_amd.h
--- a/include/pyskani_amd.h
+++ b/include/pyskani_amd.h
@@ -158,6 +158,8 @@
 const psk_sketch* psk_db_sketch(const psk_db* db, uint32_t index);
 
 psk_status psk_db_locality(psk_db* db, uint32_t* slot_of, uint32_t* n_groups, uint32_t* is_identity);
+psk_status psk_db_seed_index_info(psk_db* db, int* bits, int* shift, int* tagged);
+void psk_bsi_plan(int k, uint64_t max_block, uint32_t n_blocks, uint64_t n_entries, int mode, int* bits, int* tagged);
 
 psk_status psk_screen(psk_db* db, const psk_sketch* query, double screen_val, int rescue_small,
                       uint8_t* pass, uint32_t* shared);
diff --git a/pyskani_amd/_capi.py b/pyskani_amd/_capi.py
--- a/pyskani_amd/_capi.py
+++ b/pyskani_amd/_capi.py
@@ -54,7 +54,7 @@
     "psk_ctx_synchronize", "psk_pack2bit_host", "psk_ctx_small_query_stats", "psk_ctx_rerun_stats", "psk_ctx_tier_stats", "psk_ctx_set_timing", "psk_ctx_timing", "psk_db_add_batch", "psk_device_alloc", "psk_device_free", "psk_memcpy_h2d",
     "psk_sketch_host", "psk_sketch_many_host", "psk_sketch_batch_device", "psk_sketch_free", "psk_sketch_free_many", "psk_sketch_info",
     "psk_sketch_export", "psk_sketch_contig_lens", "psk_sketch_import", "psk_db_create", "psk_db_destroy", "psk_db_add", "psk_db_size",
-    "psk_db_name", "psk_db_sketch", "psk_db_locality", "psk_screen", "psk_chain", "psk_query", "psk_query_host", "psk_query_many", "psk_query_many_min", "psk_query_many_tri", "psk_query_many_tri_min", "psk_cluster_records", "psk_ctx_cluster_stats", "psk_gather_hits_min",
+    "psk_db_name", "psk_db_sketch", "psk_db_locality", "psk_db_seed_index_info", "psk_bsi_plan", "psk_screen", "psk_chain", "psk_query", "psk_query_host", "psk_query_many", "psk_query_many_min", "psk_query_many_tri", "psk_query_many_tri_min", "psk_cluster_records", "psk_ctx_cluster_stats", "psk_gather_hits_min",
     "psk_sketch_pack_size", "psk_sketch_pack", "psk_sketch_unpack", "psk_sketch_pack_many", "psk_ctx_clock_probe", "psk_ctx_work", "psk_ctx_join_work",
     "psk_comm_unique_id", "psk_comm_create", "psk_comm_destroy", "psk_comm_info", "psk_gather_hits", "psk_gather_sketches",
     "psk_model_create", "psk_model_load_json", "psk_model_load_file", "psk_model_free", "psk_model_info", "psk_model_predict",
@@ -118,6 +118,10 @@
     lib.psk_db_sketch.restype = vp
     lib.psk_screen.argtypes = [vp, vp, C.c_double, C.c_int, vp, vp]
     lib.psk_db_locality.argtypes = [vp, C.POINTER(C.c_uint32), C.POINTER(C.c_uint32), C.POINTER(C.c_uint32)]
+    if hasattr(lib, "psk_db_seed_index_info"):
+        lib.psk_db_seed_index_info.argtypes = [vp, C.POINTER(C.c_int), C.POINTER(C.c_int), C.POINTER(C.c_int)]
+        lib.psk_bsi_plan.argtypes = [C.c_int, u64, u32, u64, C.c_int, C.POINTER(C.c_int), C.POINTER(C.c_int)]
+        lib.psk_bsi_plan.restype = None
     lib.psk_chain.argtypes = [vp, C.POINTER(vp), u32, vp, C.POINTER(QueryOpts), C.POINTER(Hit)]
     lib.psk_query.argtypes = [vp, vp, C.POINTER(QueryOpts), C.POINTER(C.POINTER(Hit)), C.POINTER(u64)]
     lib.psk_query_host.argtypes = [vp, C.POINTER(C.c_char_p), C.POINTER(u64), u32, C.c_int, C.POINTER(QueryOpts), C.POINTER(C.POINTER(Hit)), C.POINTER(u64)]
diff --git a/pyskani_amd/csrc/capi.hip b/pyskani_amd/csrc/capi.hip
--- a/pyskani_amd/csrc/capi.hip
+++ b/pyskani_amd/csrc/capi.hip
@@ -472,6 +472,16 @@
     if (slot_of) for (uint32_t r = 0; r < n; r++) slot_of[r] = db->loc_identity ? r : db->slot_of[r];
     if (n_groups) *n_groups = db->loc_groups;
     if (is_identity) *is_identity = db->loc_identity ? 1u : 0u;
+    return PSK_OK;
+}
+
+psk_status psk_db_seed_index_info(psk_db* db, int* bits, int* shift, int* tagged) {
+    if (!db) { psk_set_error("db_seed_index_info: NULL database"); return PSK_EINVAL; }
+    std::shared_lock<std::shared_mutex> lk(db->rw);
+    const bool built = db->bsi_state == 1;
+    if (bits) *bits = built ? 2 * db->params.k - db->bsi_shift : 0;
+    if (shift) *shift = built ? db->bsi_shift : 0;
+    if (tagged) *tagged = built && db->bsi_tagged ? 1 : 0;
     return PSK_OK;
 }
 
diff --git a/pyskani_amd/csrc/chain.hip b/pyskani_amd/csrc/chain.hip
--- a/pyskani_amd/csrc/chain.hip
+++ b/pyskani_amd/csrc/chain.hip
@@ -200,7 +200,7 @@
         GA.blk_tab = d_btab; GA.blk_cnt = d_bcnt; GA.blk_cap = bcap;
         if (gsl) {
             GL.bq = L.bq; GL.n_entries = L.n_bq; GL.tab = L.gsl_tab; GL.n_tab = L.gsl_n_tab; GL.ebase = L.gsl_ebase; GL.pass = L.d_pass; GL.n_refs = L.n_refs; GL.qd = d_qd;
-            GL.g_key = L.g_key; GL.g_val = L.g_val; GL.g_bucket = L.g_bucket; GL.g_shift = L.g_shift; GL.g_nb1 = L.g_nb1; GL.g_blocks = L.g_blocks; GL.g_base = L.g_base; GL.blk_tab = d_btab; GL.blk_cnt = d_bcnt; GL.blk_cap = bcap; GL.cnt = L.gsl_cnt; GL.rec = L.gsl_rec; GL.bm = L.gsl_bm; GL.un = L.gsl_un; GL.n_slices = L.gsl_n_slices;
+            GL.g_key = L.g_key; GL.g_val = L.g_val; GL.g_bucket = L.g_bucket; GL.g_shift = L.g_shift; GL.tagged = L.g_tagged; GL.g_nb1 = L.g_nb1; GL.g_blocks = L.g_blocks; GL.g_base = L.g_base; GL.blk_tab = d_btab; GL.blk_cnt = d_bcnt; GL.blk_cap = bcap; GL.cnt = L.gsl_cnt; GL.rec = L.gsl_rec; GL.bm = L.gsl_bm; GL.un = L.gsl_un; GL.n_slices = L.gsl_n_slices;
             GL.pair_cnt = L.big_list; GL.pstart = L.pstart; GL.cap = (uint32_t)cap; GL.err = L.misc; GL.p_cap = L.p_cap; GL.chunks = L.chunks; GL.n_chunks = L.nch; GL.row_q0 = L.row_q0;
             PSK_HIP(hipMemsetAsync(L.big_list, 0, 4 * ((size_t)n_pairs + 1), st));
             PSK_TRY(gsl_count_launch(GL, st));
diff --git a/pyskani_amd/csrc/common.h b/pyskani_amd/csrc/common.h
--- a/pyskani_amd/csrc/common.h
+++ b/pyskani_amd/csrc/common.h
@@ -448,6 +448,7 @@
     int bsi_state = 0;
     PoolScratch bsi_key, bsi_val, bsi_bucket, bsi_base;
     uint64_t bsi_n = 0; int bsi_shift = 0; uint32_t bsi_nb1 = 0, bsi_blocks = 0;
+    bool bsi_tagged = false;
     std::atomic<int> small_state{0};
     int loc_state = 0;
     bool loc_identity = true, loc_groups_known = false;
@@ -456,7 +457,7 @@
     PoolScratch d_ref_of, d_slot_of, d_refdesc_slot;
     void stale() {
         tables_dirty = true; inv_dirty = true; desc_dirty = true; small_state = 0; gsi_key.release(); gsi_val.release(); gsi_bucket.release(); gsi_state = 0;
-        bsi_key.release(); bsi_val.release(); bsi_bucket.release(); bsi_base.release(); bsi_state = 0;
+        bsi_key.release(); bsi_val.release(); bsi_bucket.release(); bsi_base.release(); bsi_state = 0; bsi_tagged = false;
         loc_state = 0;
     }
 };
diff --git a/pyskani_amd/csrc/query_many.hip b/pyskani_amd/csrc/query_many.hip
--- a/pyskani_amd/csrc/query_many.hip
+++ b/pyskani_amd/csrc/query_many.hip
@@ -551,7 +551,7 @@
                         if (lrc == PSK_ENOMEM) { J.refit = true; ctx->dev->rr_refit++; return PSK_OK; }
                         PSK_TRY(lrc);
                         L.rows_pair_max = (uint32_t)std::min<uint64_t>(J.rows_pair_max, 0xFFFFFFFFu);
-                        L.g_key = (const uint32_t*)db->bsi_key.p; L.g_val = (const unsigned long long*)db->bsi_val.p; L.g_bucket = (const uint32_t*)db->bsi_bucket.p; L.g_shift = db->bsi_shift; L.g_nb1 = db->bsi_nb1; L.g_blocks = db->bsi_blocks; L.g_base = (const unsigned long long*)db->bsi_base.p;
+                        L.g_key = (const uint32_t*)db->bsi_key.p; L.g_val = (const unsigned long long*)db->bsi_val.p; L.g_bucket = (const uint32_t*)db->bsi_bucket.p; L.g_shift = db->bsi_shift; L.g_nb1 = db->bsi_nb1; L.g_blocks = db->bsi_blocks; L.g_base = (const unsigned long long*)db->bsi_base.p; L.g_tagged = db->bsi_tagged;
                         L.d_pass = d_pass; L.n_refs = n; L.n_bq = (uint32_t)J.bqs.size();
                         uint32_t pm = 1; for (const BatchQ& e : J.bqs) pm = std::max(pm, e.rank_hi - e.rank_lo);
                         L.p_cap = (pm + 15u) & ~15u;
@@ -709,7 +709,7 @@
                 psk_status lrc = chain_layout(ctx, n_pairs, (size_t)items, (size_t)rows, bqs.size(), &L);
                 L.rows_pair_max = (uint32_t)std::min<uint64_t>(rows_pair_max, 0xFFFFFFFFu);
                 if (round_gsi) {
-                    if (round_slice) { L.g_key = (const uint32_t*)db->bsi_key.p; L.g_val = (const unsigned long long*)db->bsi_val.p; L.g_bucket = (const uint32_t*)db->bsi_bucket.p; L.g_shift = db->bsi_shift; L.g_nb1 = db->bsi_nb1; L.g_blocks = db->bsi_blocks; L.g_base = (const unsigned long long*)db->bsi_base.p; }
+                    if (round_slice) { L.g_key = (const uint32_t*)db->bsi_key.p; L.g_val = (const unsigned long long*)db->bsi_val.p; L.g_bucket = (const uint32_t*)db->bsi_bucket.p; L.g_shift = db->bsi_shift; L.g_nb1 = db->bsi_nb1; L.g_blocks = db->bsi_blocks; L.g_base = (const unsigned long long*)db->bsi_base.p; L.g_tagged = db->bsi_tagged; }
                     else {
                         if (db->gsi_state == 1) { L.g_key = (const uint32_t*)db->gsi_key.p; L.g_val = (const unsigned long long*)db->gsi_val.p; L.g_bucket = (const uint32_t*)db->gsi_bucket.p; L.g_shift = db->gsi_shift; }
                         if (round_bsi) { L.b_key = (const uint32_t*)db->bsi_key.p; L.b_val = (const unsigned long long*)db->bsi_val.p; L.b_bucket = (const uint32_t*)db->bsi_bucket.p; L.b_shift = db->bsi_shift; L.b_nb1 = db->bsi_nb1; L.b_blocks = db->bsi_blocks; L.b_base = (const unsigned long long*)db->bsi_base.p; L.b_max = (uint32_t)std::max(1.0, max_blocks_join); }
diff --git a/pyskani_amd/csrc/query_parts.h b/pyskani_amd/csrc/query_parts.h
--- a/pyskani_amd/csrc/query_parts.h
+++ b/pyskani_amd/csrc/query_parts.h
@@ -80,6 +80,7 @@
     unsigned long long* total;
     uint32_t rows_pair_max = 0xFFFFFFFFu;
     const uint32_t* g_key = nullptr; const unsigned long long* g_val = nullptr; const uint32_t* g_bucket = nullptr; int g_shift = 0;
+    bool g_tagged = false;
     uint32_t g_nb1 = 0, g_blocks = 0; const unsigned long long* g_base = nullptr;
     const uint32_t* b_key = nullptr; const unsigned long long* b_val = nullptr; const uint32_t* b_bucket = nullptr; int b_shift = 0; uint32_t b_nb1 = 0, b_blocks = 0, b_max = 0; const unsigned long long* b_base = nullptr;
     const uint8_t* d_pass = nullptr; uint32_t n_refs = 0, n_bq = 0, p_cap = 0;
diff --git a/pyskani_amd/csrc/seed_index.hip b/pyskani_amd/csrc/seed_index.hip
--- a/pyskani_amd/csrc/seed_index.hip
+++ b/pyskani_amd/csrc/seed_index.hip
@@ -3,14 +3,16 @@
 #include <algorithm>
 
 struct GsiSeg { const uint32_t* kmer; const uint64_t* pm; uint32_t n, off; };
+template <bool TAG>
 __global__ __launch_bounds__(256) void gsi_gather_kernel(const GsiSeg* __restrict__ segs, uint32_t* __restrict__ key, unsigned long long* __restrict__ val) {
     const GsiSeg sg = segs[blockIdx.y];
     const unsigned long long ref = (unsigned long long)blockIdx.y << 48;
     for (uint32_t i = blockIdx.x * blockDim.x + threadIdx.x; i < sg.n; i += gridDim.x * blockDim.x) {
         const unsigned long long pm = sg.pm[i];
         const uint32_t meta = (uint32_t)pm;
-        key[sg.off + i] = sg.kmer[i];
-        val[sg.off + i] = ref | ((unsigned long long)(meta >> 1) << 33) | ((pm >> 32) << 1) | (meta & 1u);
+        const uint32_t km = sg.kmer[i];
+        key[sg.off + i] = km;
+        val[sg.off + i] = (TAG ? (unsigned long long)(km & 0xFFu) << 56 : 0ull) | ref | ((unsigned long long)(meta >> 1) << 33) | ((pm >> 32) << 1) | (meta & 1u);
     }
 }
 __global__ __launch_bounds__(256) void gsi_bucket_kernel(const uint32_t* __restrict__ key, uint32_t n, int shift, uint32_t nb, uint32_t* __restrict__ bucket) {
@@ -62,7 +64,7 @@
     };
     hipError_t e = hipMemcpyAsync(T + o_s, segs.data(), sizeof(GsiSeg) * (size_t)n, hipMemcpyHostToDevice, st);
     if (e != hipSuccess) return fail(e, "gsi: upload");
-    hipLaunchKernelGGL(gsi_gather_kernel, dim3(std::max(1u, std::min(64u, (maxn + 4095u) / 4096u)), n), dim3(256), 0, st, (const GsiSeg*)(T + o_s), (uint32_t*)(T + o_k), (unsigned long long*)(T + o_v));
+    hipLaunchKernelGGL(gsi_gather_kernel<false>, dim3(std::max(1u, std::min(64u, (maxn + 4095u) / 4096u)), n), dim3(256), 0, st, (const GsiSeg*)(T + o_s), (uint32_t*)(T + o_k), (unsigned long long*)(T + o_v));
     e = hipcub::DeviceRadixSort::SortPairs(T + o_t, ts, (const uint32_t*)(T + o_k), (uint32_t*)db->gsi_key.p, (const unsigned long long*)(T + o_v), (unsigned long long*)db->gsi_val.p, (int)N, 0, kbits, st);
     if (e != hipSuccess) return fail(e, "gsi: sort");
     hipLaunchKernelGGL(gsi_bucket_kernel, dim3((uint32_t)((N + 255) / 256)), dim3(256), 0, st, (const uint32_t*)db->gsi_key.p, (uint32_t)N, kbits - bits, nb, (uint32_t*)db->gsi_bucket.p);
@@ -81,6 +83,16 @@
     const uint32_t from = i ? (key[i - 1] >> shift) + 1u : 0u;
     for (uint32_t x = from; x <= b; x++) bucket[x] = base + i;
     if (i == n - 1) for (uint32_t x = b + 1; x <= nb; x++) bucket[x] = base + n;
+}
+void psk_bsi_plan(int k, uint64_t max_block, uint32_t n_blocks, uint64_t n_entries, int mode, int* bits, int* tagged) {
+    const int kbits = 2 * k;
+    int bits0 = 4; while (bits0 < 24 && (8ull << bits0) < max_block) bits0++;
+    if (bits0 > kbits) bits0 = kbits;
+    const int bits1 = std::max(bits0, kbits - 8);
+    bool tag = false;
+    if (k >= 1 && k <= 16 && mode != 0) tag = mode == 1 || (uint64_t)n_blocks * ((1ull << bits1) + 1ull) * 4ull <= 4ull * n_entries;
+    if (bits) *bits = tag ? bits1 : bits0;
+    if (tagged) *tagged = tag ? 1 : 0;
 }
 psk_status build_bsi(Lane* ctx, psk_db* db) {
     if (db->bsi_state) return PSK_OK;
@@ -110,8 +122,8 @@
     base[n_blocks] = N;
     if (N == 0) return PSK_OK;
     const int kbits = 2 * db->params.k;
-    int bits = 4; while (bits < 24 && (8ull << bits) < max_block) bits++;
-    if (bits > kbits) bits = kbits;
+    int bits = 0, tagged = 0;
+    psk_bsi_plan(db->params.k, max_block, n_blocks, N, env_val("PSK_BSI_TAG").force(), &bits, &tagged);
     const uint32_t nb = 1u << bits;
     size_t ts = 0;
     PSK_HIP(hipcub::DeviceRadixSort::SortPairs(nullptr, ts, (const uint32_t*)nullptr, (uint32_t*)nullptr, (const unsigned long long*)nullptr, (unsigned long long*)nullptr, (int)max_block, 0, kbits, st));
@@ -138,7 +150,7 @@
         const uint32_t r0 = b << BSI_BLOG, r1 = std::min<uint32_t>(n, (b + 1) << BSI_BLOG);
         const size_t o = (size_t)base[b]; const uint32_t cnt = (uint32_t)(base[b + 1] - base[b]);
         if (cnt) {
-            hipLaunchKernelGGL(gsi_gather_kernel, dim3(std::max(1u, std::min(64u, (maxn + 4095u) / 4096u)), r1 - r0), dim3(256), 0, st, (const GsiSeg*)(T + o_s) + r0, (uint32_t*)(T + o_k), (unsigned long long*)(T + o_v));
+            hipLaunchKernelGGL(gsi_gather_kernel<true>, dim3(std::max(1u, std::min(64u, (maxn + 4095u) / 4096u)), r1 - r0), dim3(256), 0, st, (const GsiSeg*)(T + o_s) + r0, (uint32_t*)(T + o_k), (unsigned long long*)(T + o_v));
             size_t ts_b = ts;
             e = hipcub::DeviceRadixSort::SortPairs(T + o_t, ts_b, (const uint32_t*)(T + o_k), (uint32_t*)db->bsi_key.p + o, (const unsigned long long*)(T + o_v), (unsigned long long*)db->bsi_val.p + o, (int)cnt, 0, kbits, st);
             if (e != hipSuccess) return fail(e, "bsi: sort");
@@ -147,7 +159,7 @@
     }
     e = hipStreamSynchronize(st);
     if (e != hipSuccess) return fail(e, "bsi: build");
-    db->bsi_n = N; db->bsi_shift = kbits - bits; db->bsi_nb1 = nb + 1; db->bsi_blocks = n_blocks;
+    db->bsi_n = N; db->bsi_shift = kbits - bits; db->bsi_nb1 = nb + 1; db->bsi_blocks = n_blocks; db->bsi_tagged = tagged != 0;
     db->bsi_state = 1;
     return PSK_OK;
 }
diff --git a/pyskani_amd/csrc/slice_join.h b/pyskani_amd/csrc/slice_join.h
--- a/pyskani_amd/csrc/slice_join.h
+++ b/pyskani_amd/csrc/slice_join.h
@@ -17,6 +17,7 @@
     uint32_t* un; uint32_t n_slices;
     const uint8_t* pass; uint32_t n_refs; const SketchDesc* qd;
     const uint32_t* g_key; const unsigned long long* g_val; const uint32_t* g_bucket; int g_shift;
+    bool tagged;
     const unsigned long long* g_base;
     uint32_t g_nb1, g_blocks;
     uint32_t* blk_tab; uint32_t* blk_cnt; uint32_t blk_cap;
diff --git a/pyskani_amd/csrc/slice_join.hip b/pyskani_amd/csrc/slice_join.hip
--- a/pyskani_amd/csrc/slice_join.hip
+++ b/pyskani_amd/csrc/slice_join.hip
@@ -27,7 +27,10 @@
     return (emit ? (8 * GSL_LW + 8 + 8) * (size_t)A.p_cap + 8 * 64 : 0) + 64 + 4 * (size_t)A.p_cap + (emit ? 0 : 4 * (size_t)GSL_WORDS * (A.p_cap + 1));
 }
 
-template <bool EMIT>
+__device__ __forceinline__ uint32_t gsl_ref_word(unsigned long long v) { return (uint32_t)(v >> 53) & 7u; }
+__device__ __forceinline__ uint32_t gsl_ref_bit(unsigned long long v) { return (uint32_t)(v >> 48) & 31u; }
+__device__ __forceinline__ uint32_t gsl_tag(unsigned long long v) { return (uint32_t)(v >> 56); }
+template <bool EMIT, bool TAGGED>
 __global__ __launch_bounds__(64) void gsl_walk_kernel(GslArgs A) {
     extern __shared__ uint4 s_gsl[];
     const int lane = threadIdx.x;
@@ -107,7 +110,7 @@
                 ns[u] = 63u - (uint32_t)__clzll((long long)own); \
                 nx[u] = (uint32_t)__builtin_amdgcn_readlane((int)lo, (int)ns[u]) + 64u * ((t) - (uint32_t)__builtin_amdgcn_readlane((int)pre, (int)ns[u])); \
                 nh[u] = (uint32_t)__builtin_amdgcn_readlane((int)hi, (int)ns[u]); \
-                if (nx[u] + (uint32_t)lane < nh[u]) { nk[u] = x_key[nx[u] + lane]; nv[u] = x_val[nx[u] + lane]; } \
+                if (nx[u] + (uint32_t)lane < nh[u]) { if (!TAGGED) nk[u] = x_key[nx[u] + lane]; nv[u] = x_val[nx[u] + lane]; } \
             } } while (0)
 #pragma unroll
         for (uint32_t u = 0; u < GSL_AHEAD; u++) GSL_FETCH(u, u);
@@ -119,12 +122,13 @@
             for (uint32_t u = 0; u < GSL_AHEAD; u++) GSL_FETCH(t0 + GSL_AHEAD + u, u);
             uint32_t slots[GSL_AHEAD]; uint2 bps[GSL_AHEAD];
 #pragma unroll
-            for (uint32_t u = 0; u < GSL_AHEAD; u++) bps[u] = s_bp[(uint32_t)(cv[u] >> 53) & 7u];
+            for (uint32_t u = 0; u < GSL_AHEAD; u++) bps[u] = s_bp[gsl_ref_word(cv[u])];
 #pragma unroll
             for (uint32_t u = 0; u < GSL_AHEAD; u++) {
                 const uint32_t skm = (uint32_t)__builtin_amdgcn_readlane((int)km, (int)cs[u]);
-                const uint32_t b = (uint32_t)(cv[u] >> 48) & 31u, rk = bps[u].y + (uint32_t)__popc(bps[u].x & ~(~0u << b)) - B.rank_lo;
-                const bool ok = cx[u] + (uint32_t)lane < ch[u] && ck[u] == skm && ((bps[u].x >> b) & 1u) && rk < P;
+                const uint32_t b = gsl_ref_bit(cv[u]), rk = bps[u].y + (uint32_t)__popc(bps[u].x & ~(~0u << b)) - B.rank_lo;
+                const bool hit = TAGGED ? gsl_tag(cv[u]) == (skm & 0xFFu) : ck[u] == skm;
+                const bool ok = cx[u] + (uint32_t)lane < ch[u] && hit && ((bps[u].x >> b) & 1u) && rk < P;
                 slots[u] = ok ? rk : 0xFFFFFFFFu;
             }
 #pragma unroll
@@ -369,7 +373,8 @@
     return PSK_OK;
 }
 psk_status gsl_count_launch(const GslArgs& A, hipStream_t st) {
-    hipLaunchKernelGGL(gsl_walk_kernel<false>, dim3(A.n_tab), dim3(64), gsl_walk_lds(A, false), st, A);
+    auto* const walk = A.tagged ? gsl_walk_kernel<false, true> : gsl_walk_kernel<false, false>;
+    hipLaunchKernelGGL(walk, dim3(A.n_tab), dim3(64), gsl_walk_lds(A, false), st, A);
     PSK_HIP(hipGetLastError());
     return PSK_OK;
 }
@@ -380,7 +385,8 @@
     return PSK_OK;
 }
 psk_status gsl_emit_launch(const GslArgs& A, hipStream_t st) {
-    hipLaunchKernelGGL(gsl_walk_kernel<true>, dim3(A.n_tab), dim3(64), gsl_walk_lds(A, true), st, A);
+    auto* const walk = A.tagged ? gsl_walk_kernel<true, true> : gsl_walk_kernel<true, false>;
+    hipLaunchKernelGGL(walk, dim3(A.n_tab), dim3(64), gsl_walk_lds(A, true), st, A);
     PSK_HIP(hipGetLastError());
     return PSK_OK;
 }
diff --git a/rust/ffi.rs b/rust/ffi.rs
--- a/rust/ffi.rs
+++ b/rust/ffi.rs
@@ -117,6 +117,8 @@
                                rep_of: *mut u32, rep_ani: *mut f32, n_reps: *mut u32) -> c_int;
     pub fn psk_ctx_cluster_stats(ctx: *mut PskCtx, edges: *mut u64, rounds: *mut u64, hook_passes: *mut u64) -> c_int;
     pub fn psk_db_locality(db: *mut PskDb, slot_of: *mut u32, n_groups: *mut u32, is_identity: *mut u32) -> c_int;
+    pub fn psk_db_seed_index_info(db: *mut PskDb, bits: *mut c_int, shift: *mut c_int, tagged: *mut c_int) -> c_int;
+    pub fn psk_bsi_plan(k: c_int, max_block: u64, n_blocks: u32, n_entries: u64, mode: c_int, bits: *mut c_int, tagged: *mut c_int);
     pub fn psk_screen(db: *mut PskDb, q: *const PskSketch, screen_val: f64, rescue_small: c_int,
                       pass: *mut u8, shared: *mut u32) -> c_int;
     pub fn psk_chain(ctx: *mut PskCtx, refs: *const *const PskSketch, n: u32, q: *const PskSketch,
```

Result: faster. 220.2 million genome-pairs/s (median of 6 runs) (+5.3%).
